# jiaxi98/cnf_ot

Hardware: NVIDIA B200
Metric: flow train-step samples/s (fwd+inv+logdet+loss+grad) (higher is better)
Workload: dtype f32

## Files before the change

cnf_ot_b200/csrc/api.cu:

```cuda
#include <cuda_runtime.h>
#include <math.h>
#include <stdarg.h>
#include <stdio.h>
#include <stdlib.h>
#include <string.h>

#include <mutex>
#include <vector>

#include "../../include/cnfot.h"
#include "device_common.cuh"
#include "dense_tc.h"
#include "dispatch.h"
#include "flow_kernels.cuh"
#include "step_host.h"
#include "wide.h"

namespace cnfot {

cudaError_t rqs_eval_dispatch(int K, bool inverse, cudaStream_t s, const float* v,
                              const float* params, int64_t rows, const SplineConsts<float>& sc,
                              float* out, float* ld, int32_t* bin, int num_sms, bool* known);
cudaError_t rqs_vjp_dispatch(int K, bool inverse, cudaStream_t s, const float* v,
                             const float* params, const float* go, const float* gl, int64_t rows,
                             const SplineConsts<float>& sc, float* gi, float* gp, int num_sms,
                             bool* known);

static thread_local char g_err[512] = "";

static int fail(int code, const char* fmt, ...) {
  va_list ap;
  va_start(ap, fmt);
  vsnprintf(g_err, sizeof(g_err), fmt, ap);
  va_end(ap);
  return code;
}

static int cuda_fail(cudaError_t e, const char* what) {
  return fail(CNFOT_ERR_CUDA, "%s: %s", what, cudaGetErrorString(e));
}

struct DeviceInfo {
  int device = -1;
  int num_sms = 0;
  int max_smem_optin = 0;
};

static int device_info(DeviceInfo* out) {
  static DeviceInfo cache[64];
  int dev = 0;
  cudaError_t e = cudaGetDevice(&dev);
  if (e != cudaSuccess) return cuda_fail(e, "cudaGetDevice (no CUDA device? libcnfot has no CPU path)");
  if (dev < 0 || dev >= 64) return fail(CNFOT_ERR_CUDA, "device id %d out of range", dev);
  if (cache[dev].device != dev) {
    DeviceInfo d;
    d.device = dev;
    e = cudaDeviceGetAttribute(&d.num_sms, cudaDevAttrMultiProcessorCount, dev);
    if (e != cudaSuccess) return cuda_fail(e, "cudaDeviceGetAttribute");
    e = cudaDeviceGetAttribute(&d.max_smem_optin, cudaDevAttrMaxSharedMemoryPerBlockOptin, dev);
    if (e != cudaSuccess) return cuda_fail(e, "cudaDeviceGetAttribute");
    cache[dev] = d;
  }
  *out = cache[dev];
  return 0;
}

constexpr int kMaxGrid = 148 * 8;
constexpr int64_t kCounterBytes = 256;

static int check_flow(const cnfot_flow_desc* f, FlowLayout* lay) {
  if (!f) return fail(CNFOT_ERR_ARG, "flow descriptor is NULL");
  if (f->dim < 1 || f->num_layers < 1 || f->mlp_layers < 1 || f->hidden < 1 || f->num_bins < 1)
    return fail(CNFOT_ERR_ARG, "flow descriptor has non-positive sizes");
  if (f->hidden % 4 != 0) return fail(CNFOT_ERR_ARG, "hidden size %d must be a multiple of 4", f->hidden);
  if (!(f->range_max > f->range_min) || f->num_bins * f->min_bin_size > f->range_max - f->range_min)
    return fail(CNFOT_ERR_ARG, "min_bin_size too large for the spline range");
  if (!(f->min_knot_slope < 1.f)) return fail(CNFOT_ERR_ARG, "min_knot_slope must be < 1");
  *lay = make_layout(f->dim, f->num_layers, f->mlp_layers, f->hidden, f->num_bins);
  return 0;
}

static bool reference_spline_consts(const cnfot_flow_desc* f) {
  const SplineConsts<float> c = make_spline_consts<float>(f->num_bins, f->range_min, f->range_max, f->min_bin_size,
                                                          f->min_knot_slope);
  return c.lo == -10.f && c.hi == 10.f && c.min_bin == 1e-4f && c.min_slope == 1e-4f &&
         fabsf(c.slope_offset - 0.5411666523385311f) <= 1e-7f;
}

static int check_fused(const cnfot_flow_desc* f, const FlowLayout& lay) {
  if (!reference_spline_consts(f))
    return fail(CNFOT_ERR_ARG, "the fused flow kernels are compiled for the reference's spline constants (range -10..10, "
                               "min_bin_size = min_knot_slope = 1e-4; cnf_ot/models/flows.py:124-132)");
  if (f->dim > kMaxDim) return fail(CNFOT_ERR_ARG, "fused kernels support dim <= %d (got %d)", kMaxDim, f->dim);
  if ((f->num_layers + 1) * f->dim > kMaxStateFloats)
    return fail(CNFOT_ERR_ARG, "fused kernels need (num_layers+1)*dim <= %d (got %d)", kMaxStateFloats,
                (f->num_layers + 1) * f->dim);
  if (!find_flow_eval_kernel(lay))
    return fail(CNFOT_ERR_ARG,
                "no fused kernel instantiated for hidden=%d num_bins=%d mlp_layers=%d "
                "(see CNFOT_NET_LIST in cnf_ot_b200/csrc/dispatch.h)",
                f->hidden, f->num_bins, f->mlp_layers);
  return 0;
}

static bool fused_ok(const cnfot_flow_desc* f, const FlowLayout& lay) {
  if (!(f->dim <= kMaxDim && (f->num_layers + 1) * f->dim <= kMaxStateFloats && find_flow_eval_kernel(lay) != nullptr))
    return false;
  if (!reference_spline_consts(f)) return false;
  if (tc_available(lay)) return true;
  DeviceInfo di;
  if (device_info(&di)) return true;
  return (int64_t)plan_smem(lay, true, false).floats * 4 <= di.max_smem_optin;
}
static bool use_wide(const cnfot_flow_desc* f, const FlowLayout& lay) {
  if (!wide_supported(lay, nullptr)) return false;
  if (!fused_ok(f, lay)) return true;
  const char* e = getenv("CNFOT_ENGINE");
  return e && !strcmp(e, "wide");
}

static SplineConsts<float> spline_consts(const cnfot_flow_desc* f) {
  return make_spline_consts<float>(f->num_bins, f->range_min, f->range_max, f->min_bin_size,
                                   f->min_knot_slope);
}

struct LaunchCfg {
  int grid;
  size_t smem;
};
static thread_local int g_last_launch[4] = {0, 0, 0, 0};

static int engine_override() {
  const char* e = getenv("CNFOT_ENGINE");
  if (!e) {
    const char* t = getenv("CNFOT_TC");
    return (t && t[0] == '1') ? kEngTc : -1;
  }
  if (!strcmp(e, "cuda")) return kEngCuda;
  if (!strcmp(e, "tc")) return kEngTc;
  if (!strcmp(e, "mma")) return kEngMma;
  return -1;
}

static int make_plan(const FlowLayout& lay, bool with_grad, SmemPlan* sp, int* engine, bool has_ws = true) {
  DeviceInfo di;
  if (int rc = device_info(&di)) return rc;
  const int want = engine_override();
  *engine = kEngCuda;
  if (want == kEngTc && tc_available(lay)) {
    SmemPlan t = plan_smem(lay, with_grad, true, true);
    if ((int64_t)t.floats * 4 * 2 <= di.max_smem_optin) {
      *sp = t;
      *engine = kEngTc;
      return 0;
    }
  }
  if ((want == kEngMma || want < 0) && tc_available(lay)) {
    SmemPlan m = plan_smem_mma(lay, with_grad);
    if ((int64_t)m.floats * 4 * 2 <= di.max_smem_optin) {
      *sp = m;
      *engine = kEngMma;
      return 0;
    }
    if (has_ws) {
      *sp = plan_smem_mma(lay, with_grad, false);
      *engine = kEngMmaStream;
      return 0;
    }
  }
  SmemPlan p = plan_smem(lay, with_grad, true);
  if ((int64_t)p.floats * 4 * 2 > di.max_smem_optin) p = plan_smem(lay, with_grad, false);
  *sp = p;
  return 0;
}

static int configure(const void* kernel, const SmemPlan& sp, int64_t tiles, LaunchCfg* cfg) {
  DeviceInfo di;
  if (int rc = device_info(&di)) return rc;
  size_t smem = (size_t)sp.floats * sizeof(float);
  if ((int64_t)smem > di.max_smem_optin)
    return fail(CNFOT_ERR_ARG, "network too large for the fused kernels: needs %zu B of shared memory, device allows %d",
                smem, di.max_smem_optin);
  cudaError_t e = cudaFuncSetAttribute(kernel, cudaFuncAttributeMaxDynamicSharedMemorySize, (int)smem);
  if (e != cudaSuccess) return cuda_fail(e, "cudaFuncSetAttribute");
  int occ = 0;
  e = cudaOccupancyMaxActiveBlocksPerMultiprocessor(&occ, kernel, kTile, smem);
  if (e != cudaSuccess) return cuda_fail(e, "cudaOccupancyMaxActiveBlocksPerMultiprocessor");
  if (sp.off_wmma >= 0) {
    cudaFuncAttributes fa;
    e = cudaFuncGetAttributes(&fa, kernel);
    if (e != cudaSuccess) return cuda_fail(e, "cudaFuncGetAttributes");
    int smem_sm = 0, regs_sm = 0;
    cudaDeviceGetAttribute(&smem_sm, cudaDevAttrMaxSharedMemoryPerMultiprocessor, di.device);
    cudaDeviceGetAttribute(&regs_sm, cudaDevAttrMaxRegistersPerMultiprocessor, di.device);
    int by_smem = (int)(smem_sm / (smem + fa.sharedSizeBytes + 1024));
    int by_regs = regs_sm / (fa.numRegs * kTile > 0 ? fa.numRegs * kTile : 1);
    int by_tmem = 512 / 32;
    occ = by_smem < by_regs ? by_smem : by_regs;
    if (occ > by_tmem) occ = by_tmem;
  }
  if (getenv("CNFOT_DEBUG")) {
    cudaFuncAttributes fa;
    cudaFuncGetAttributes(&fa, kernel);
    int o0 = 0, o1 = 0;
    cudaOccupancyMaxActiveBlocksPerMultiprocessor(&o0, kernel, kTile, 0);
    cudaOccupancyMaxActiveBlocksPerMultiprocessor(&o1, kernel, kTile, 60000);
    fprintf(stderr, "[cnfot] occ=%d (smem %zu) occ@0=%d occ@60000=%d regs=%d static_smem=%zu local=%zu maxdyn=%d carveout=%d\n",
            occ, smem, o0, o1, fa.numRegs, fa.sharedSizeBytes, fa.localSizeBytes, fa.maxDynamicSharedSizeBytes,
            fa.preferredShmemCarveout);
  }
  if (occ < 1) return fail(CNFOT_ERR_CUDA, "kernel does not fit on an SM");
  int64_t cap = (int64_t)di.num_sms * occ;
  if (cap > kMaxGrid) cap = kMaxGrid;
  int64_t g = tiles < cap ? tiles : cap;
  cfg->grid = (int)(g > 0 ? g : 1);
  cfg->smem = smem;
  g_last_launch[0] = cfg->grid;
  g_last_launch[1] = (int)smem;
  g_last_launch[2] = occ;
  g_last_launch[3] = sp.off_wmma >= 0 ? kEngTc : (sp.off_frag >= 0 ? kEngMma : kEngCuda);
  return 0;
}

static int64_t frag_bytes(const FlowLayout& lay) {
  if (!tc_available(lay)) return 0;
  return (int64_t)lay.L * (lay.D - 1) * lay.M * kFragFloats * sizeof(float);
}
static int64_t partial_bytes(const FlowLayout& lay) {
  int64_t loss = (int64_t)kMaxGrid * kNumSlots * sizeof(double);
  int64_t grad = ((int64_t)kMaxGrid * lay.total * sizeof(float) + 255) / 256 * 256;
  return kCounterBytes + loss + grad + frag_bytes(lay);
}
static int64_t stash_cta_floats(const FlowLayout& lay) {
  if (!tc_available(lay)) return 0;
  const int64_t per_cta = (int64_t)lay.L * (lay.D - 1) * (4 * lay.M + (2 * lay.K + 10 + 3) / 4) * kTile * 4;
  if (per_cta * (int64_t)sizeof(float) > 64 * 1024) return 0;
  if (const char* e = getenv("CNFOT_STEP_STASH")) {
    if (e[0] == '0') return 0;
  }
  return per_cta;
}
constexpr int kStashMaxGrid = 6 * 148;
static int64_t stash_bytes(const FlowLayout& lay) { return stash_cta_floats(lay) * (int64_t)sizeof(float) * kStashMaxGrid; }
static int64_t step_bytes(const FlowLayout& lay) { return partial_bytes(lay) + stash_bytes(lay); }
static float* carve_frags(void* ws, const FlowLayout& lay) {
  return (float*)((char*)ws + partial_bytes(lay) - frag_bytes(lay));
}
static int launch_build_frags(cudaStream_t s, const FlowLayout& lay, const float* weights, float* frags) {
  const int n_mat = lay.L * (lay.D - 1) * lay.M;
  const int blocks = (n_mat * 256 + 255) / 256;
  build_frags_kernel<<<blocks < 1184 ? blocks : 1184, 256, 0, s>>>(weights, frags, lay.D, lay.M, n_mat);
  cudaError_t e = cudaGetLastError();
  if (e != cudaSuccess) return cuda_fail(e, "build_frags_kernel launch");
  return 0;
}

static PartialBuf carve_partials(void* ws, unsigned long long** counter) {
  char* p = (char*)ws;
  *counter = (unsigned long long*)p;
  PartialBuf pb;
  pb.loss = (double*)(p + kCounterBytes);
  pb.grad = (float*)(p + kCounterBytes + (int64_t)kMaxGrid * kNumSlots * sizeof(double));
  return pb;
}

constexpr int kFinWarps = 32;
__device__ __forceinline__ double column_partial(const float* __restrict__ pgrad, int n_cta, int total, int i,
                                                 int warp) {
  double a0 = 0.0, a1 = 0.0, a2 = 0.0, a3 = 0.0;
  int c = warp;
  for (; c + 3 * kFinWarps < n_cta; c += 4 * kFinWarps) {
    const float v0 = __ldcg(pgrad + (int64_t)c * total + i);
    const float v1 = __ldcg(pgrad + (int64_t)(c + kFinWarps) * total + i);
    const float v2 = __ldcg(pgrad + (int64_t)(c + 2 * kFinWarps) * total + i);
    const float v3 = __ldcg(pgrad + (int64_t)(c + 3 * kFinWarps) * total + i);
    a0 += (double)v0; a1 += (double)v1; a2 += (double)v2; a3 += (double)v3;
  }
  for (; c < n_cta; c += kFinWarps) a0 += (double)__ldcg(pgrad + (int64_t)c * total + i);
  return (a0 + a1) + (a2 + a3);
}

__global__ void __launch_bounds__(32 * kFinWarps)
finalize_kernel(const float* __restrict__ pgrad, const double* __restrict__ ploss, int n_cta,
                int total, float* __restrict__ out_grad, float* __restrict__ out_slots,
                int accumulate) {
  __shared__ double part[kFinWarps][32];
  const int lane = threadIdx.x & 31, warp = threadIdx.x >> 5;
  const int i = blockIdx.x * 32 + lane;
  double acc = 0.0;
  if (i < total) acc = column_partial(pgrad, n_cta, total, i, warp);
  part[warp][lane] = acc;
  __syncthreads();
  if (warp == 0 && i < total) {
    double t = 0.0;
#pragma unroll
    for (int w = 0; w < kFinWarps; ++w) t += part[w][lane];
    out_grad[i] = accumulate ? out_grad[i] + (float)t : (float)t;
  }
  if (out_slots && blockIdx.x == gridDim.x - 1) {
    __syncthreads();
    const int sl = lane & 7, sub = lane >> 3;
    double v = 0.0;
    for (int c = warp * 4 + sub; c < n_cta; c += 4 * kFinWarps) v += ploss[(int64_t)c * kNumSlots + sl];
    v += __shfl_xor_sync(0xffffffffu, v, 8);
    v += __shfl_xor_sync(0xffffffffu, v, 16);
    part[warp][lane] = v;
    __syncthreads();
    if (warp == 0) {
      double t = 0.0;
      if (lane < kNumSlots)
        for (int w = 0; w < kFinWarps; ++w) t += part[w][lane];
      double tot = t;
      tot += __shfl_xor_sync(0xffffffffu, tot, 1);
      tot += __shfl_xor_sync(0xffffffffu, tot, 2);
      if (lane == 0) out_slots[0] = accumulate ? out_slots[0] + (float)tot : (float)tot;
      if (lane < 4) out_slots[1 + lane] = accumulate ? out_slots[1 + lane] + (float)t : (float)t;
      if (lane >= 5 && lane < kNumSlots) out_slots[lane] = 0.f;
    }
  }
}

static int launch_finalize(cudaStream_t s, const PartialBuf& pb, int n_cta, int total, float* out_grad,
                           float* out_slots, bool accumulate = false) {
  int blocks = (total + 31) / 32;
  finalize_kernel<<<blocks, 32 * kFinWarps, 0, s>>>(pb.grad, pb.loss, n_cta, total, out_grad, out_slots,
                                                   accumulate ? 1 : 0);
  cudaError_t e = cudaGetLastError();
  if (e != cudaSuccess) return cuda_fail(e, "finalize_kernel launch");
  return 0;
}

__global__ void energy_finalize_kernel(const double* __restrict__ ploss, int n_cta, double* __restrict__ out) {
  double v = 0.0;
  for (int c = threadIdx.x; c < n_cta; c += 32) v += ploss[(int64_t)c * kNumSlots + kSlotKinetic];
#pragma unroll
  for (int o = 16; o > 0; o >>= 1) v += __shfl_xor_sync(0xffffffffu, v, o);
  if (threadIdx.x == 0) out[0] = v;
}

__global__ void adam_kernel(float* __restrict__ p, const float* __restrict__ g, float* __restrict__ m,
                            float* __restrict__ v, int64_t n, float lr, float b1, float b2, float eps,
                            float c1, float c2) {
  for (int64_t i = blockIdx.x * (int64_t)blockDim.x + threadIdx.x; i < n; i += (int64_t)gridDim.x * blockDim.x) {
    float gi = g[i];
    float mi = b1 * m[i] + (1.f - b1) * gi;
    float vi = b2 * v[i] + (1.f - b2) * gi * gi;
    m[i] = mi;
    v[i] = vi;
    p[i] -= lr * (mi / c1) / (sqrtf(vi / c2) + eps);
  }
}

__global__ void __launch_bounds__(256)
recon_head_kernel(const float* __restrict__ x, const float* __restrict__ xr, int64_t count, float weight,
                  float* __restrict__ g_xr, double* __restrict__ loss) {
  double acc = 0.0;
  for (int64_t e = blockIdx.x * (int64_t)blockDim.x + threadIdx.x; e < count; e += (int64_t)gridDim.x * blockDim.x) {
    const float dlt = x[e] - xr[e];
    acc += (double)dlt * (double)dlt;
    g_xr[e] = -2.f * weight * dlt;
  }
#pragma unroll
  for (int o = 16; o > 0; o >>= 1) acc += __shfl_xor_sync(0xffffffffu, acc, o);
  if ((threadIdx.x & 31) == 0 && acc != 0.0) atomicAdd(loss, acc * (double)weight);
}
__global__ void __launch_bounds__(256)
mask_tail_kernel(float* __restrict__ y, int64_t rows, int dim, int sub_dim) {
  const int64_t count = rows * dim;
  for (int64_t e = blockIdx.x * (int64_t)blockDim.x + threadIdx.x; e < count; e += (int64_t)gridDim.x * blockDim.x)
    if ((int)(e % dim) >= sub_dim) y[e] = 0.f;
}

}

using namespace cnfot;

extern "C" {

int cnfot_abi_version(void) { return CNFOT_ABI_VERSION; }
static unsigned long long* g_step_timeline = nullptr;
void cnfot_debug_step_timeline(void* device_words) { g_step_timeline = (unsigned long long*)device_words; }

void cnfot_last_launch_info(int32_t* grid, int32_t* smem_bytes, int32_t* ctas_per_sm, int32_t* tensor_cores) {
  if (grid) *grid = g_last_launch[0];
  if (smem_bytes) *smem_bytes = g_last_launch[1];
  if (ctas_per_sm) *ctas_per_sm = g_last_launch[2];
  if (tensor_cores) *tensor_cores = g_last_launch[3];
}
const char* cnfot_last_error(void) { return g_err; }

int64_t cnfot_param_count(const cnfot_flow_desc* flow) {
  FlowLayout lay;
  if (check_flow(flow, &lay)) return -1;
  return lay.total;
}

int64_t cnfot_spline_param_stride(const cnfot_flow_desc* flow) {
  FlowLayout lay;
  if (check_flow(flow, &lay)) return -1;
  return lay.Pp;
}

int64_t cnfot_offset_first(const cnfot_flow_desc* flow) {
  FlowLayout lay;
  if (check_flow(flow, &lay)) return -1;
  return 0;
}

int64_t cnfot_offset_linear(const cnfot_flow_desc* flow, int32_t layer, int32_t d, int32_t m, int32_t bias) {
  FlowLayout lay;
  if (check_flow(flow, &lay)) return -1;
  if (layer < 0 || layer >= lay.L || d < 1 || d >= lay.D || m < 0 || m > lay.M) {
    fail(CNFOT_ERR_ARG, "offset_linear: index out of range");
    return -1;
  }
  const int H = lay.H;
  int64_t off = lay.Pp + (int64_t)layer * lay.layer_stride + (int64_t)(d - 1) * lay.mlp_const +
                (int64_t)H * ((d - 1) * (d + 2) / 2);
  const int n_in = d + 1;
  if (m == 0) return off + (bias ? n_in * H : 0);
  off += n_in * H + H + (int64_t)(m - 1) * (H * H + H);
  if (m < lay.M) return off + (bias ? H * H : 0);
  return off + (bias ? H * lay.Pp : 0);
}

int cnfot_flow_supported(const cnfot_flow_desc* flow) {
  FlowLayout lay;
  if (int rc = check_flow(flow, &lay)) return rc;
  if (use_wide(flow, lay)) return 0;
  return check_fused(flow, lay);
}

static int rqs_call(bool inverse, void* stream, const float* v, const float* params, int64_t rows,
                    int32_t K, float lo, float hi, float min_bin, float min_slope, float* out,
                    float* ld, int32_t* bin) {
  if (rows < 0) return fail(CNFOT_ERR_ARG, "rows < 0");
  if (rows == 0) return 0;
  if (!v || !params || !out || !ld) return fail(CNFOT_ERR_ARG, "NULL buffer");
  if (K < 1 || !(hi > lo) || K * min_bin > hi - lo || !(min_slope < 1.f))
    return fail(CNFOT_ERR_ARG, "bad spline constants");
  DeviceInfo di;
  if (int rc = device_info(&di)) return rc;
  bool known = false;
  cudaError_t e = rqs_eval_dispatch(K, inverse, (cudaStream_t)stream, v, params, rows,
                                    make_spline_consts<float>(K, lo, hi, min_bin, min_slope), out, ld,
                                    bin, di.num_sms, &known);
  if (!known) return fail(CNFOT_ERR_ARG, "num_bins=%d not instantiated (see CNFOT_BINS_LIST)", K);
  if (e != cudaSuccess) return cuda_fail(e, "rqs kernel launch");
  return 0;
}

static int rqs_vjp_call(bool inverse, void* stream, const float* v, const float* params,
                        const float* go, const float* gl, int64_t rows, int32_t K, float lo, float hi,
                        float min_bin, float min_slope, float* gi, float* gp) {
  if (rows < 0) return fail(CNFOT_ERR_ARG, "rows < 0");
  if (rows == 0) return 0;
  if (!v || !params || !go || !gl || !gi || !gp) return fail(CNFOT_ERR_ARG, "NULL buffer");
  if (K < 1 || !(hi > lo) || K * min_bin > hi - lo || !(min_slope < 1.f))
    return fail(CNFOT_ERR_ARG, "bad spline constants");
  DeviceInfo di;
  if (int rc = device_info(&di)) return rc;
  bool known = false;
  cudaError_t e = rqs_vjp_dispatch(K, inverse, (cudaStream_t)stream, v, params, go, gl, rows,
                                   make_spline_consts<float>(K, lo, hi, min_bin, min_slope), gi, gp,
                                   di.num_sms, &known);
  if (!known) return fail(CNFOT_ERR_ARG, "num_bins=%d not instantiated (see CNFOT_BINS_LIST)", K);
  if (e != cudaSuccess) return cuda_fail(e, "rqs vjp kernel launch");
  return 0;
}

int cnfot_rqs_forward(void* stream, const float* x, const float* params, int64_t rows, int32_t num_bins,
                      float range_min, float range_max, float min_bin_size, float min_knot_slope,
                      float* y, float* logdet, int32_t* bin_idx) {
  return rqs_call(false, stream, x, params, rows, num_bins, range_min, range_max, min_bin_size,
                  min_knot_slope, y, logdet, bin_idx);
}
int cnfot_rqs_inverse(void* stream, const float* y, const float* params, int64_t rows, int32_t num_bins,
                      float range_min, float range_max, float min_bin_size, float min_knot_slope,
                      float* x, float* logdet, int32_t* bin_idx) {
  return rqs_call(true, stream, y, params, rows, num_bins, range_min, range_max, min_bin_size,
                  min_knot_slope, x, logdet, bin_idx);
}
int cnfot_rqs_forward_vjp(void* stream, const float* x, const float* params, const float* g_y,
                          const float* g_logdet, int64_t rows, int32_t num_bins, float range_min,
                          float range_max, float min_bin_size, float min_knot_slope, float* g_x,
                          float* g_params) {
  return rqs_vjp_call(false, stream, x, params, g_y, g_logdet, rows, num_bins, range_min, range_max,
                      min_bin_size, min_knot_slope, g_x, g_params);
}
int cnfot_rqs_inverse_vjp(void* stream, const float* y, const float* params, const float* g_x,
                          const float* g_logdet, int64_t rows, int32_t num_bins, float range_min,
                          float range_max, float min_bin_size, float min_knot_slope, float* g_y,
                          float* g_params) {
  return rqs_vjp_call(true, stream, y, params, g_x, g_logdet, rows, num_bins, range_min, range_max,
                      min_bin_size, min_knot_slope, g_y, g_params);
}

static int flow_eval_call(int dir, void* stream, const cnfot_flow_desc* flow, const float* weights,
                          const float* in, const float* cond, int64_t cond_stride, int64_t rows,
                          float* out, float* logdet, int32_t add_base, void* workspace = nullptr,
                          int64_t workspace_bytes = 0) {
  FlowLayout lay;
  if (int rc = check_flow(flow, &lay)) return rc;
  if (use_wide(flow, lay)) {
    if (rows < 0) return fail(CNFOT_ERR_ARG, "rows < 0");
    if (cond_stride != 0 && cond_stride != 1) return fail(CNFOT_ERR_ARG, "cond_stride must be 0 or 1");
    if (rows == 0) return 0;
    if (!weights || !in || !cond || !out) return fail(CNFOT_ERR_ARG, "NULL buffer");
    const int64_t need = wide_flow_workspace_bytes(lay, rows, false);
    if (!workspace)
      return fail(CNFOT_ERR_WORKSPACE, "this flow runs on the wide-conditioner engine, which needs a workspace: "
                                       "call cnfot_flow_forward_ws / cnfot_flow_inverse_ws");
    if (workspace_bytes < need) return fail(CNFOT_ERR_WORKSPACE, "workspace too small: %lld < %lld",
                                            (long long)workspace_bytes, (long long)need);
    const char* what = "";
    cudaError_t e = wide_flow_eval((cudaStream_t)stream, lay, spline_consts(flow), weights, dir, in, cond, cond_stride,
                                   rows, out, logdet, add_base, workspace, &what);
    if (e != cudaSuccess) return cuda_fail(e, what);
    g_last_launch[0] = 0; g_last_launch[1] = 0; g_last_launch[2] = 0; g_last_launch[3] = kEngWide;
    return 0;
  }
  if (int rc = check_fused(flow, lay)) return rc;
  if (rows < 0) return fail(CNFOT_ERR_ARG, "rows < 0");
  if (cond_stride != 0 && cond_stride != 1) return fail(CNFOT_ERR_ARG, "cond_stride must be 0 or 1");
  if (rows == 0) return 0;
  if (!weights || !in || !cond || !out) return fail(CNFOT_ERR_ARG, "NULL buffer");
  SmemPlan sp;
  int engine;
  if (int rc = make_plan(lay, false, &sp, &engine, false)) return rc;
  const void* kernel = find_flow_eval_kernel(lay, engine);
  LaunchCfg cfg;
  if (int rc = configure(kernel, sp, (rows + kTile - 1) / kTile, &cfg)) return rc;
  EvalArgs a;
  a.W = weights; a.frags = nullptr; a.in = in; a.cond = cond; a.cond_stride = cond_stride; a.rows = rows;
  a.out = out; a.logdet = logdet; a.dir = dir; a.add_base = add_base;
  a.D = lay.D; a.L = lay.L; a.plan = sp;
  void* args[] = {&a};
  cudaError_t e = cudaLaunchKernel(kernel, dim3(cfg.grid), dim3(kTile), args, cfg.smem, (cudaStream_t)stream);
  if (e != cudaSuccess) return cuda_fail(e, "flow_eval_kernel launch");
  return 0;
}

int cnfot_flow_forward(void* stream, const cnfot_flow_desc* flow, const float* weights, const float* in,
                       const float* cond, int64_t cond_stride, int64_t rows, float* out, float* logdet,
                       int32_t add_base) {
  return flow_eval_call(0, stream, flow, weights, in, cond, cond_stride, rows, out, logdet, add_base);
}
int cnfot_flow_inverse(void* stream, const cnfot_flow_desc* flow, const float* weights, const float* in,
                       const float* cond, int64_t cond_stride, int64_t rows, float* out, float* logdet,
                       int32_t add_base) {
  return flow_eval_call(1, stream, flow, weights, in, cond, cond_stride, rows, out, logdet, add_base);
}

int64_t cnfot_flow_workspace_bytes(const cnfot_flow_desc* flow, int64_t rows) {
  FlowLayout lay;
  if (check_flow(flow, &lay)) return -1;
  return use_wide(flow, lay) ? wide_flow_workspace_bytes(lay, rows, false) : 0;
}
int cnfot_flow_forward_ws(void* stream, const cnfot_flow_desc* flow, const float* weights, const float* in,
                          const float* cond, int64_t cond_stride, int64_t rows, float* out, float* logdet,
                          int32_t add_base, void* workspace, int64_t workspace_bytes) {
  return flow_eval_call(0, stream, flow, weights, in, cond, cond_stride, rows, out, logdet, add_base, workspace,
                        workspace_bytes);
}
int cnfot_flow_inverse_ws(void* stream, const cnfot_flow_desc* flow, const float* weights, const float* in,
                          const float* cond, int64_t cond_stride, int64_t rows, float* out, float* logdet,
                          int32_t add_base, void* workspace, int64_t workspace_bytes) {
  return flow_eval_call(1, stream, flow, weights, in, cond, cond_stride, rows, out, logdet, add_base, workspace,
                        workspace_bytes);
}

int64_t cnfot_flow_vjp_workspace_bytes(const cnfot_flow_desc* flow, int64_t rows) {
  FlowLayout lay;
  if (check_flow(flow, &lay)) return -1;
  if (use_wide(flow, lay)) return wide_flow_workspace_bytes(lay, rows, true);
  return step_bytes(lay);
}

static int flow_vjp_call(int dir, void* stream, const cnfot_flow_desc* flow, const float* weights,
                         const float* in, const float* cond, int64_t cond_stride, int64_t rows,
                         const float* g_out, const float* g_logdet, int32_t add_base, float* g_in,
                         float* g_weights, void* workspace, int64_t workspace_bytes) {
  FlowLayout lay;
  if (int rc = check_flow(flow, &lay)) return rc;
  if (use_wide(flow, lay)) {
    if (rows < 0) return fail(CNFOT_ERR_ARG, "rows < 0");
    if (cond_stride != 0 && cond_stride != 1) return fail(CNFOT_ERR_ARG, "cond_stride must be 0 or 1");
    if (!weights || !g_weights || !workspace) return fail(CNFOT_ERR_ARG, "NULL buffer");
    if (rows > 0 && (!in || !cond || !g_out)) return fail(CNFOT_ERR_ARG, "NULL buffer");
    const int64_t need = wide_flow_workspace_bytes(lay, rows, true);
    if (workspace_bytes < need) return fail(CNFOT_ERR_WORKSPACE, "workspace too small: %lld < %lld",
                                            (long long)workspace_bytes, (long long)need);
    const char* what = "";
    cudaError_t e = wide_flow_vjp((cudaStream_t)stream, lay, spline_consts(flow), weights, dir, in, cond, cond_stride,
                                  rows, g_out, g_logdet, add_base, g_in, g_weights, workspace, &what);
    if (e != cudaSuccess) return cuda_fail(e, what);
    g_last_launch[0] = 0; g_last_launch[1] = 0; g_last_launch[2] = 0; g_last_launch[3] = kEngWide;
    return 0;
  }
  if (int rc = check_fused(flow, lay)) return rc;
  if (rows < 0) return fail(CNFOT_ERR_ARG, "rows < 0");
  if (cond_stride != 0 && cond_stride != 1) return fail(CNFOT_ERR_ARG, "cond_stride must be 0 or 1");
  if (!weights || !g_weights || !workspace) return fail(CNFOT_ERR_ARG, "NULL buffer");
  if (workspace_bytes < partial_bytes(lay)) return fail(CNFOT_ERR_WORKSPACE, "workspace too small: %lld < %lld",
                                                        (long long)workspace_bytes, (long long)partial_bytes(lay));
  cudaStream_t s = (cudaStream_t)stream;
  if (rows == 0) {
    cudaError_t e = cudaMemsetAsync(g_weights, 0, (size_t)lay.total * sizeof(float), s);
    if (e != cudaSuccess) return cuda_fail(e, "cudaMemsetAsync");
    return 0;
  }
  if (!in || !cond || !g_out) return fail(CNFOT_ERR_ARG, "NULL buffer");
  SmemPlan sp;
  int engine;
  if (int rc = make_plan(lay, true, &sp, &engine)) return rc;
  const void* kernel = find_flow_vjp_kernel(lay, engine);
  LaunchCfg cfg;
  if (int rc = configure(kernel, sp, (rows + kTile - 1) / kTile, &cfg)) return rc;
  unsigned long long* counter;
  VjpArgs a;
  a.W = weights; a.frags = nullptr; a.in = in; a.cond = cond; a.cond_stride = cond_stride; a.rows = rows;
  if (engine == kEngMmaStream) {
    float* fr = carve_frags(workspace, lay);
    if (int rc = launch_build_frags(s, lay, weights, fr)) return rc;
    a.frags = fr;
  }
  a.g_out = g_out; a.g_logdet = g_logdet; a.g_in = g_in; a.dir = dir; a.add_base = add_base;
  a.D = lay.D; a.L = lay.L; a.plan = sp;
  a.pb = carve_partials(workspace, &counter);
  a.stash = nullptr;
  a.stash_cta_floats = (engine == kEngMma || engine == kEngMmaStream) && cfg.grid <= kStashMaxGrid &&
                               workspace_bytes >= step_bytes(lay)
                           ? stash_cta_floats(lay) : 0;
  if (a.stash_cta_floats > 0) a.stash = (float*)((char*)workspace + partial_bytes(lay));
  void* args[] = {&a};
  cudaError_t e = cudaLaunchKernel(kernel, dim3(cfg.grid), dim3(kTile), args, cfg.smem, s);
  if (e != cudaSuccess) return cuda_fail(e, "flow_vjp_kernel launch");
  return launch_finalize(s, a.pb, cfg.grid, lay.total, g_weights, nullptr);
}

int cnfot_flow_forward_vjp(void* stream, const cnfot_flow_desc* flow, const float* weights,
                           const float* in, const float* cond, int64_t cond_stride, int64_t rows,
                           const float* g_out, const float* g_logdet, int32_t add_base, float* g_in,
                           float* g_weights, void* workspace, int64_t workspace_bytes) {
  return flow_vjp_call(0, stream, flow, weights, in, cond, cond_stride, rows, g_out, g_logdet, add_base,
                       g_in, g_weights, workspace, workspace_bytes);
}
int cnfot_flow_inverse_vjp(void* stream, const cnfot_flow_desc* flow, const float* weights,
                           const float* in, const float* cond, int64_t cond_stride, int64_t rows,
                           const float* g_out, const float* g_logdet, int32_t add_base, float* g_in,
                           float* g_weights, void* workspace, int64_t workspace_bytes) {
  return flow_vjp_call(1, stream, flow, weights, in, cond, cond_stride, rows, g_out, g_logdet, add_base,
                       g_in, g_weights, workspace, workspace_bytes);
}

static std::mutex g_ws_mu;
static std::vector<std::pair<void*, int64_t>> g_ws_registered;
static bool ws_registered(const void* ws) {
  std::lock_guard<std::mutex> lk(g_ws_mu);
  for (const auto& e : g_ws_registered)
    if (e.first == ws) return true;
  return false;
}
int cnfot_workspace_release(void* workspace) {
  std::lock_guard<std::mutex> lk(g_ws_mu);
  for (size_t i = 0; i < g_ws_registered.size(); ++i)
    if (g_ws_registered[i].first == workspace) {
      g_ws_registered.erase(g_ws_registered.begin() + i);
      return 0;
    }
  return 0;
}

static bool pdl_enabled() {
  static int on = -1;
  if (on < 0) {
    const char* e = getenv("CNFOT_PDL");
    on = (e && e[0] == '0') ? 0 : 1;
  }
  return on != 0;
}
static cudaError_t launch_step_kernel(const void* kernel, int grid, void** args, size_t smem, cudaStream_t s) {
  if (!pdl_enabled()) return cudaLaunchKernel(kernel, dim3(grid), dim3(kTile), args, smem, s);
  cudaLaunchConfig_t lc = {};
  lc.gridDim = dim3(grid); lc.blockDim = dim3(kTile); lc.dynamicSmemBytes = smem; lc.stream = s;
  cudaLaunchAttribute at[1];
  at[0].id = cudaLaunchAttributeProgrammaticStreamSerialization;
  at[0].val.programmaticStreamSerializationAllowed = 1;
  lc.attrs = at; lc.numAttrs = 1;
  return cudaLaunchKernelExC(&lc, kernel, args);
}

static int64_t step_ws_bytes(const cnfot_flow_desc* flow, const FlowLayout& lay, int64_t rows_B, int64_t rows_b) {
  return use_wide(flow, lay) ? wide_step_workspace_bytes(lay, rows_B, rows_b) : step_bytes(lay);
}

int64_t cnfot_mfc_step_workspace_bytes(const cnfot_flow_desc* flow, int64_t rows_B, int64_t rows_b,
                                       int32_t n_t) {
  (void)n_t;
  FlowLayout lay;
  if (check_flow(flow, &lay)) return -1;
  return step_ws_bytes(flow, lay, rows_B, rows_b);
}

static int mfc_step_wide(void* stream, const cnfot_flow_desc* flow, const FlowLayout& lay,
                         const cnfot_problem_desc* problem, const float* weights, const float* latent, const float* latent_sub,
                         const float* src, const float* tgt, const float* t_batch_host, int32_t n_t, int64_t rows_B,
                         int64_t rows_b, int64_t global_B, int64_t global_b, float lambda, float* out, void* workspace,
                         int64_t workspace_bytes, bool accumulate, const cnfot_peer_desc* peers) {
  if (!problem) return fail(CNFOT_ERR_ARG, "problem descriptor is NULL");
  if (peers)
    return fail(CNFOT_ERR_ARG, "the wide-conditioner engine has no fused all-reduce (its gradient is hundreds of MB): "
                               "call cnfot_mfc_step and all-reduce `out` with NCCL");
  if (accumulate) return fail(CNFOT_ERR_ARG, "the wide-conditioner engine does not take chunked host input");
  if (rows_B < 0 || rows_b < 0 || global_B < 1 || global_b < 1 || rows_B > global_B || rows_b > global_b)
    return fail(CNFOT_ERR_ARG, "bad row counts");
  if (n_t < 1) return fail(CNFOT_ERR_ARG, "t_batch_size must be >= 1");
  if (!weights || !out || !workspace || !t_batch_host) return fail(CNFOT_ERR_ARG, "NULL buffer");
  if (problem->type == CNFOT_OT) {
    if (rows_B > 0 && (!src || !tgt)) return fail(CNFOT_ERR_ARG, "ot needs src and tgt batches");
  } else if (rows_B > 0 && !latent) {
    return fail(CNFOT_ERR_ARG, "latent is NULL");
  }
  if (rows_b > 0 && !latent_sub) return fail(CNFOT_ERR_ARG, "latent_sub is NULL");
  const int64_t need = wide_step_workspace_bytes(lay, rows_B, rows_b);
  if (workspace_bytes < need) return fail(CNFOT_ERR_WORKSPACE, "workspace too small: %lld < %lld",
                                          (long long)workspace_bytes, (long long)need);
  StepConsts<float> pc;
  const char* err = nullptr;
  if (make_step_consts<float>(*problem, lay.D, (double)lambda, global_B, global_b, n_t, &pc, &err))
    return fail(CNFOT_ERR_ARG, "%s", err);
  const char* what = "";
  cudaError_t e = wide_mfc_step((cudaStream_t)stream, lay, spline_consts(flow), pc, weights, latent, latent_sub, src, tgt,
                                t_batch_host, n_t, rows_B, rows_b, out, workspace, &what);
  if (e != cudaSuccess) return cuda_fail(e, what);
  g_last_launch[0] = 0; g_last_launch[1] = 0; g_last_launch[2] = 0; g_last_launch[3] = kEngWide;
  return 0;
}

struct StepIo {
  const float* latent = nullptr;
  const float* latent_sub = nullptr;
  const float* src = nullptr;
  const float* tgt = nullptr;
  const float* t_batch_host = nullptr;
  bool rng = false;
  uint64_t key = 0;
  uint32_t step = 0;
  int64_t row0_B = 0, row0_b = 0;
  float* out = nullptr;
  bool accumulate = false;
  const cnfot_peer_desc* peers = nullptr;
  bool stateful = false;
  float* weights_rw = nullptr;
  float* adam_m = nullptr;
  float* adam_v = nullptr;
  float lr = 0.f, b1 = 0.9f, b2 = 0.999f, eps = 1e-8f;
  float* loss_hist = nullptr;
  int64_t loss_hist_len = 0;
};

static unsigned long long dp_timeout_ns() {
  unsigned long long ms = 20000ULL;
  if (const char* e = getenv("CNFOT_DP_TIMEOUT_MS")) {
    const long long v = atoll(e);
    if (v > 0) ms = (unsigned long long)v;
  }
  return ms * 1000000ULL;
}

static int mfc_step_impl(void* stream, const cnfot_flow_desc* flow, const cnfot_problem_desc* problem,
                         const float* weights, const StepIo& io, int32_t n_t,
                         int64_t rows_B, int64_t rows_b, int64_t global_B, int64_t global_b, float lambda,
                         void* workspace, int64_t workspace_bytes) {
  FlowLayout lay;
  if (int rc = check_flow(flow, &lay)) return rc;
  if (use_wide(flow, lay)) {
    cnfot_workspace_release(workspace);
    if (io.rng || io.stateful)
      return fail(CNFOT_ERR_ARG, "the wide-conditioner engine takes explicit row arrays: fill them with cnfot_philox_rows "
                                 "and call cnfot_mfc_step (+ cnfot_adam_update)");
    return mfc_step_wide(stream, flow, lay, problem, weights, io.latent, io.latent_sub, io.src, io.tgt, io.t_batch_host, n_t,
                         rows_B, rows_b, global_B, global_b, lambda, io.out, workspace, workspace_bytes, io.accumulate, io.peers);
  }
  if (int rc = check_fused(flow, lay)) return rc;
  if (!problem) return fail(CNFOT_ERR_ARG, "problem descriptor is NULL");
  StepArgs a;
  memset(&a.tail, 0, sizeof(a.tail));
  PeerArgs& pa = a.tail.pa;
  const cnfot_peer_desc* peers = io.peers;
  if (peers) {
    if (peers->world < 1 || peers->world > 8 || peers->rank < 0 || peers->rank >= peers->world)
      return fail(CNFOT_ERR_ARG, "peer descriptor: need 1 <= world <= 8 and 0 <= rank < world");
    if (peers->epoch == 0 && !io.stateful) return fail(CNFOT_ERR_ARG, "peer descriptor: epoch starts at 1");
    pa.rank = peers->rank; pa.world = peers->world; pa.epoch = peers->epoch;
    pa.stride = (int)cnfot_dp_exchange_stride(flow);
    pa.timeout_ns = dp_timeout_ns();
    for (int k = 0; k < peers->world; ++k) {
      if (!peers->xbuf[k] || !peers->flags[k]) return fail(CNFOT_ERR_ARG, "peer descriptor: NULL peer buffer");
      if ((uintptr_t)peers->xbuf[k] & 7) return fail(CNFOT_ERR_ARG, "peer descriptor: exchange buffers must be 8-byte aligned");
      pa.xbuf[k] = (unsigned long long*)peers->xbuf[k]; pa.flags[k] = peers->flags[k];
    }
  }
  if (rows_B < 0 || rows_b < 0 || global_B < 1 || global_b < 1 || rows_B > global_B || rows_b > global_b)
    return fail(CNFOT_ERR_ARG, "bad row counts");
  if (n_t < 1 || n_t > kMaxSegments - 4) return fail(CNFOT_ERR_ARG, "t_batch_size must be in [1, %d]", kMaxSegments - 4);
  if (!weights || !workspace) return fail(CNFOT_ERR_ARG, "NULL buffer");
  if (!io.out && !io.stateful) return fail(CNFOT_ERR_ARG, "out is NULL");
  if (!io.rng && !io.t_batch_host) return fail(CNFOT_ERR_ARG, "t_batch is NULL");
  if (workspace_bytes < step_bytes(lay)) return fail(CNFOT_ERR_WORKSPACE, "workspace too small: %lld < %lld",
                                                     (long long)workspace_bytes, (long long)step_bytes(lay));
  const char* err = nullptr;
  if (make_step_consts<float>(*problem, lay.D, (double)lambda, global_B, global_b, n_t, &a.pc, &err))
    return fail(CNFOT_ERR_ARG, "%s", err);
  if (!io.rng) {
    if (problem->type == CNFOT_OT) {
      if (rows_B > 0 && (!io.src || !io.tgt)) return fail(CNFOT_ERR_ARG, "ot needs src and tgt batches");
    } else {
      if (rows_B > 0 && !io.latent) return fail(CNFOT_ERR_ARG, "latent is NULL");
    }
    if (rows_b > 0 && !io.latent_sub) return fail(CNFOT_ERR_ARG, "latent_sub is NULL");
  } else if (io.row0_B < 0 || io.row0_b < 0 || io.row0_B + rows_B > global_B || io.row0_b + rows_b > global_b) {
    return fail(CNFOT_ERR_ARG, "shard [row0, row0 + rows) outside the global batch");
  }
  cudaStream_t s = (cudaStream_t)stream;
  if (rows_B == 0 && rows_b == 0 && !peers && !io.stateful) {
    if (io.accumulate) return 0;
    cudaError_t e = cudaMemsetAsync(io.out, 0, (size_t)(lay.total + CNFOT_NUM_LOSS_SLOTS) * sizeof(float), s);
    if (e != cudaSuccess) return cuda_fail(e, "cudaMemsetAsync");
    return 0;
  }
  SmemPlan sp;
  int engine;
  if (int rc = make_plan(lay, true, &sp, &engine)) return rc;
  const int unit = kTile;

  int ns = 0;
  int64_t tiles = 0;
  auto add = [&](int kind, int slot, int do_fit, int do_pot, float t, int t_index, const float* rows, int source,
                 int64_t row0, int64_t n, int group) {
    if (n <= 0) return;
    Segment& sg = a.seg[ns++];
    sg.kind = kind; sg.slot = slot; sg.do_fit = do_fit; sg.do_pot = do_pot; sg.t = t; sg.t_index = t_index;
    sg.rows = rows; sg.source = io.rng ? source : (int)kRowsMemory; sg.row0 = row0;
    sg.n = n; sg.first_tile = tiles; sg.group = group;
    tiles += (n * group + unit - 1) / unit;
  };
  int group = 1;
  {
    const bool with_score = problem->type != CNFOT_OT;
    const bool need_r3 = with_score || a.pc.potential == kPotObstacle;
    int g = with_score ? 4 : (need_r3 ? 4 : 2);
    while (with_score && g < 2 * lay.D) g <<= 1;
    const int64_t fit_tiles = (problem->type == CNFOT_FP ? 1 : 2) * ((rows_B + unit - 1) / unit);
    const int64_t serial_tiles = fit_tiles + (int64_t)n_t * ((rows_b + unit - 1) / unit);
    bool split = g <= 32 && serial_tiles <= kMaxGrid;
    if (const char* e = getenv("CNFOT_KINETIC_SPLIT")) split = g <= 32 && e[0] != '0';
    if (split) group = g;
  }
  bool latency = false;
  {
    const int64_t fit_tiles = (problem->type == CNFOT_FP ? 1 : 2) * ((rows_B + unit - 1) / unit);
    latency = fit_tiles + (int64_t)n_t * ((rows_b + unit - 1) / unit) < 8 * 4 * 148;
    if (const char* e = getenv("CNFOT_STEP_LATENCY")) latency = e[0] != '0';
  }
  const void* kernel = find_mfc_step_kernel(lay, engine, group > 1, latency);
  for (int i = 0; i < n_t; ++i)
    add(group > 1 ? kSegKineticSplit : kSegKinetic, kSlotKinetic, 0, 0, io.rng ? 0.f : io.t_batch_host[i], io.rng ? i : -1,
        io.latent_sub, kRowsNormal, io.row0_b, rows_b, group);
  if (problem->type == CNFOT_OT) {
    add(kSegNll, kSlotFit0, 1, 0, 0.f, -1, io.src, kRowsOtSource, io.row0_B, rows_B, 1);
    add(kSegNll, kSlotFitT, 1, 0, (float)a.pc.horizon, -1, io.tgt, kRowsNormal, io.row0_B, rows_B, 1);
  } else {
    add(kSegSample, kSlotFit0, 1, 0, 0.f, -1, io.latent, kRowsNormal, io.row0_B, rows_B, 1);
    if (problem->type == CNFOT_RWPO) add(kSegSample, kSlotFit0, 0, 1, (float)a.pc.horizon, -1, io.latent, kRowsNormal, io.row0_B, rows_B, 1);
  }
  a.n_seg = ns;
  a.n_tiles = tiles;
  a.key = io.key;
  a.step = io.step;
  a.timeline = g_step_timeline;
  a.salt_B = philox_salt(kDrawNormal, (uint64_t)global_B);
  a.salt_Bc = philox_salt(kDrawCategorical, (uint64_t)global_B);
  a.salt_b = philox_salt(kDrawNormal, (uint64_t)global_b);
  a.salt_t = philox_salt(kDrawUniform, (uint64_t)n_t);
  LaunchCfg cfg;
  if (int rc = configure(kernel, sp, (tiles * unit + kTile - 1) / kTile, &cfg)) return rc;
  a.W = weights;
  a.frags = nullptr;
  if (engine == kEngMmaStream) {
    float* fr = carve_frags(workspace, lay);
    if (int rc = launch_build_frags(s, lay, weights, fr)) return rc;
    a.frags = fr;
  }
  a.D = lay.D; a.L = lay.L; a.plan = sp;
  a.stash = nullptr;
  a.stash_cta_floats = (engine == kEngMma || engine == kEngMmaStream) && cfg.grid <= kStashMaxGrid ? stash_cta_floats(lay) : 0;
  if (a.stash_cta_floats > 0) a.stash = (float*)((char*)workspace + partial_bytes(lay));
  TailArgs& t = a.tail;
  char* wsb = (char*)workspace;
  t.sync = (uint32_t*)wsb;
  t.loss_row = (double*)(wsb) + kLossRowOffset;
  t.grad_rows = (float*)(wsb + kCounterBytes);
  const bool persistent = io.stateful || ws_registered(workspace);
  t.n_rows = cfg.grid < kStepRows ? cfg.grid : kStepRows;
  if (const char* e = getenv("CNFOT_STEP_ROWS")) {
    const int v = atoi(e);
    if (v >= 1 && v <= (persistent ? kStepRows : kMaxGrid)) t.n_rows = v < cfg.grid ? v : cfg.grid;
  }
  int n_tail = (lay.total + kNumSlots + kTile / 4 - 1) / (kTile / 4);
  if (n_tail > cfg.grid) n_tail = cfg.grid;
  if (cfg.grid > 148 && n_tail > cfg.grid / 2) n_tail = cfg.grid / 2;
  if (n_tail > 2 * 148) n_tail = 2 * 148;
  if (n_tail < 1) n_tail = 1;
  t.n_tail = n_tail;
  t.total = lay.total;
  t.n_tiles = tiles;
  t.accumulate = io.accumulate ? 1 : 0;
  t.out = io.out;
  if (io.stateful) {
    t.self_clean = 1;
    t.state = (unsigned long long*)wsb + kStateWordOffset;
    t.weights = io.weights_rw; t.adam_m = io.adam_m; t.adam_v = io.adam_v;
    t.lr = io.lr; t.b1 = io.b1; t.b2 = io.b2; t.eps = io.eps;
    t.loss_hist = io.loss_hist; t.loss_hist_len = io.loss_hist_len;
  } else if (persistent) {
    t.self_clean = 1;
  } else {
    cudaError_t e = cudaMemsetAsync(wsb, 0, (size_t)kCounterBytes + (size_t)t.n_rows * lay.total * sizeof(float), s);
    if (e != cudaSuccess) return cuda_fail(e, "cudaMemsetAsync");
  }
  void* args[] = {&a};
  cudaError_t e = launch_step_kernel(kernel, cfg.grid, args, cfg.smem, s);
  if (e != cudaSuccess) return cuda_fail(e, "mfc_step_kernel launch");
  return 0;
}

int64_t cnfot_dp_exchange_stride(const cnfot_flow_desc* flow) {
  FlowLayout lay;
  if (check_flow(flow, &lay)) return -1;
  return (lay.total + kNumSlots + 31) / 32 * 32;
}
int64_t cnfot_dp_exchange_floats(const cnfot_flow_desc* flow, int32_t world) {
  const int64_t st = cnfot_dp_exchange_stride(flow);
  return st < 0 ? -1 : 2 * 2 * (int64_t)world * st;
}
int64_t cnfot_dp_flag_count(const cnfot_flow_desc* flow, int32_t world) {
  FlowLayout lay;
  if (check_flow(flow, &lay)) return -1;
  (void)world;
  return 32;
}

int cnfot_mfc_step_dp(void* stream, const cnfot_flow_desc* flow, const cnfot_problem_desc* problem,
                      const float* weights, const float* latent, const float* latent_sub, const float* src,
                      const float* tgt, const float* t_batch_host, int32_t n_t, int64_t rows_B,
                      int64_t rows_b, int64_t global_B, int64_t global_b, float lambda, float* out,
                      void* workspace, int64_t workspace_bytes, const cnfot_peer_desc* peers) {
  if (!peers) return fail(CNFOT_ERR_ARG, "peer descriptor is NULL");
  StepIo io;
  io.latent = latent; io.latent_sub = latent_sub; io.src = src; io.tgt = tgt; io.t_batch_host = t_batch_host;
  io.out = out; io.peers = peers;
  return mfc_step_impl(stream, flow, problem, weights, io, n_t, rows_B, rows_b, global_B, global_b, lambda, workspace,
                       workspace_bytes);
}

int cnfot_workspace_register(void* stream, const cnfot_flow_desc* flow, void* workspace, int64_t workspace_bytes) {
  FlowLayout lay;
  if (int rc = check_flow(flow, &lay)) return rc;
  if (use_wide(flow, lay)) return fail(CNFOT_ERR_ARG, "persistent workspaces serve the fused per-row step kernel, not the wide-conditioner engine");
  if (!workspace) return fail(CNFOT_ERR_ARG, "NULL buffer");
  if (workspace_bytes < step_bytes(lay)) return fail(CNFOT_ERR_WORKSPACE, "workspace too small: %lld < %lld",
                                                     (long long)workspace_bytes, (long long)step_bytes(lay));
  cudaError_t e = cudaMemsetAsync(workspace, 0, (size_t)kCounterBytes + (size_t)kStepRows * lay.total * sizeof(float),
                                  (cudaStream_t)stream);
  if (e != cudaSuccess) return cuda_fail(e, "cudaMemsetAsync");
  cnfot_workspace_release(workspace);
  std::lock_guard<std::mutex> lk(g_ws_mu);
  g_ws_registered.emplace_back(workspace, workspace_bytes);
  return 0;
}

int cnfot_mfc_step(void* stream, const cnfot_flow_desc* flow, const cnfot_problem_desc* problem,
                   const float* weights, const float* latent, const float* latent_sub, const float* src,
                   const float* tgt, const float* t_batch_host, int32_t n_t, int64_t rows_B,
                   int64_t rows_b, int64_t global_B, int64_t global_b, float lambda, float* out,
                   void* workspace, int64_t workspace_bytes) {
  StepIo io;
  io.latent = latent; io.latent_sub = latent_sub; io.src = src; io.tgt = tgt; io.t_batch_host = t_batch_host;
  io.out = out;
  return mfc_step_impl(stream, flow, problem, weights, io, n_t, rows_B, rows_b, global_B, global_b, lambda, workspace,
                       workspace_bytes);
}

__global__ void __launch_bounds__(256)
philox_rows_kernel(unsigned long long key_n, unsigned long long key_c, uint32_t step, int source, int64_t row0, int64_t rows,
                   int dim, float* __restrict__ out) {
  for (int64_t r = blockIdx.x * (int64_t)blockDim.x + threadIdx.x; r < rows; r += (int64_t)gridDim.x * blockDim.x) {
    float row[kMaxDim];
    philox_row(key_n, key_c, step, source, (uint64_t)(row0 + r), dim, row);
    for (int i = 0; i < dim; ++i) out[r * dim + i] = row[i];
  }
}

int cnfot_philox_rows(void* stream, uint64_t key, uint32_t step, int32_t source, int64_t global_rows, int64_t row0,
                      int64_t rows, int32_t dim, float* out) {
  if (rows < 0 || row0 < 0 || row0 + rows > global_rows || dim < 1 || dim > kMaxDim)
    return fail(CNFOT_ERR_ARG, "philox_rows: need 0 <= row0, row0 + rows <= global_rows, 1 <= dim <= %d", kMaxDim);
  if (source != CNFOT_ROWS_NORMAL && source != CNFOT_ROWS_OT_SOURCE) return fail(CNFOT_ERR_ARG, "philox_rows: unknown row source");
  if (rows == 0) return 0;
  if (!out) return fail(CNFOT_ERR_ARG, "NULL buffer");
  int64_t blocks = (rows + 255) / 256;
  if (blocks > 148 * 8) blocks = 148 * 8;
  philox_rows_kernel<<<(int)blocks, 256, 0, (cudaStream_t)stream>>>(
      key ^ philox_salt(kDrawNormal, (uint64_t)global_rows), key ^ philox_salt(kDrawCategorical, (uint64_t)global_rows), step,
      source, row0, rows, dim, out);
  cudaError_t e = cudaGetLastError();
  if (e != cudaSuccess) return cuda_fail(e, "philox_rows_kernel launch");
  return 0;
}

int cnfot_philox_times_host(uint64_t key, uint32_t step, int32_t n_t, float horizon, float* t_host) {
  if (n_t < 0 || (n_t > 0 && !t_host)) return fail(CNFOT_ERR_ARG, "philox_times: bad arguments");
  const uint64_t kt = key ^ philox_salt(kDrawUniform, (uint64_t)n_t);
  for (int i = 0; i < n_t; ++i) t_host[i] = philox_time(kt, step, i, horizon);
  return 0;
}

int cnfot_mfc_step_rng(void* stream, const cnfot_flow_desc* flow, const cnfot_problem_desc* problem, const float* weights,
                       uint64_t key, uint32_t step, int32_t n_t, int64_t row0_B, int64_t rows_B, int64_t row0_b,
                       int64_t rows_b, int64_t global_B, int64_t global_b, float lambda, float* out, void* workspace,
                       int64_t workspace_bytes, const cnfot_peer_desc* peers) {
  StepIo io;
  io.rng = true; io.key = key; io.step = step; io.row0_B = row0_B; io.row0_b = row0_b;
  io.out = out; io.peers = peers;
  return mfc_step_impl(stream, flow, problem, weights, io, n_t, rows_B, rows_b, global_B, global_b, lambda, workspace,
                       workspace_bytes);
}

int64_t cnfot_train_state_bytes(const cnfot_flow_desc* flow) {
  FlowLayout lay;
  if (check_flow(flow, &lay)) return -1;
  if (use_wide(flow, lay)) { fail(CNFOT_ERR_ARG, "no device-resident update for the wide-conditioner engine"); return -1; }
  return step_bytes(lay);
}

int cnfot_train_state_init(void* stream, const cnfot_flow_desc* flow, void* state, int64_t state_bytes, uint64_t key,
                           uint64_t step, uint32_t epoch) {
  const int64_t need = cnfot_train_state_bytes(flow);
  if (need < 0) return CNFOT_ERR_ARG;
  if (!state) return fail(CNFOT_ERR_ARG, "NULL buffer");
  if (state_bytes < need) return fail(CNFOT_ERR_WORKSPACE, "train state too small: %lld < %lld", (long long)state_bytes, (long long)need);
  FlowLayout lay;
  check_flow(flow, &lay);
  cudaStream_t s = (cudaStream_t)stream;
  cudaError_t e = cudaMemsetAsync(state, 0, (size_t)kCounterBytes + (size_t)kStepRows * lay.total * sizeof(float), s);
  if (e != cudaSuccess) return cuda_fail(e, "cudaMemsetAsync");
  const unsigned long long words[3] = {key, step, (unsigned long long)epoch};
  e = cudaMemcpyAsync((unsigned long long*)state + kStateWordOffset, words, sizeof(words), cudaMemcpyHostToDevice, s);
  if (e != cudaSuccess) return cuda_fail(e, "H2D train state");
  e = cudaStreamSynchronize(s);
  if (e != cudaSuccess) return cuda_fail(e, "cudaStreamSynchronize");
  return 0;
}

int cnfot_mfc_update(void* stream, const cnfot_flow_desc* flow, const cnfot_problem_desc* problem, void* state,
                     int64_t state_bytes, float* weights, float* adam_m, float* adam_v, const cnfot_adam_desc* adam,
                     int32_t n_t, int64_t row0_B, int64_t rows_B, int64_t row0_b, int64_t rows_b, int64_t global_B,
                     int64_t global_b, float lambda, float* out, float* loss_hist, int64_t loss_hist_len,
                     const cnfot_peer_desc* peers) {
  if (!state || !weights || !adam_m || !adam_v || !adam) return fail(CNFOT_ERR_ARG, "NULL buffer");
  if (loss_hist_len < 0 || (loss_hist_len > 0 && !loss_hist)) return fail(CNFOT_ERR_ARG, "bad loss history buffer");
  StepIo io;
  io.rng = true; io.row0_B = row0_B; io.row0_b = row0_b;
  io.out = out; io.peers = peers;
  io.stateful = true;
  io.weights_rw = weights; io.adam_m = adam_m; io.adam_v = adam_v;
  io.lr = adam->lr; io.b1 = adam->b1; io.b2 = adam->b2; io.eps = adam->eps;
  io.loss_hist = loss_hist; io.loss_hist_len = loss_hist_len;
  return mfc_step_impl(stream, flow, problem, weights, io, n_t, rows_B, rows_b, global_B, global_b, lambda, state,
                       state_bytes);
}

static int64_t align256(int64_t v) { return (v + 255) / 256 * 256; }

struct HostPipe {
  bool ready_ = false;
  cudaStream_t copy;
  cudaEvent_t start;
  cudaEvent_t ready[4];
};
static int host_pipe(HostPipe** out) {
  static HostPipe pipes[64];
  DeviceInfo di;
  if (int rc = device_info(&di)) return rc;
  HostPipe& p = pipes[di.device];
  if (!p.ready_) {
    cudaError_t e = cudaStreamCreateWithFlags(&p.copy, cudaStreamNonBlocking);
    if (e != cudaSuccess) return cuda_fail(e, "cudaStreamCreateWithFlags");
    if ((e = cudaEventCreateWithFlags(&p.start, cudaEventDisableTiming)) != cudaSuccess) return cuda_fail(e, "cudaEventCreate");
    for (int k = 0; k < 4; ++k)
      if ((e = cudaEventCreateWithFlags(&p.ready[k], cudaEventDisableTiming)) != cudaSuccess) return cuda_fail(e, "cudaEventCreate");
    p.ready_ = true;
  }
  *out = &p;
  return 0;
}

int64_t cnfot_mfc_step_host_workspace_bytes(const cnfot_flow_desc* flow, int64_t rows_B, int64_t rows_b,
                                            int32_t n_t) {
  FlowLayout lay;
  if (check_flow(flow, &lay)) return -1;
  (void)n_t;
  int64_t rowsB = align256(rows_B * lay.D * (int64_t)sizeof(float));
  int64_t rowsb = align256(rows_b * lay.D * (int64_t)sizeof(float));
  int64_t w = align256((int64_t)lay.total * sizeof(float));
  int64_t o = align256((int64_t)(lay.total + CNFOT_NUM_LOSS_SLOTS) * sizeof(float));
  return align256(step_ws_bytes(flow, lay, rows_B, rows_b)) + w + o + 3 * rowsB + rowsb;
}

int cnfot_mfc_step_host(void* stream, const cnfot_flow_desc* flow, const cnfot_problem_desc* problem,
                        const float* weights_host, const float* latent_host,
                        const float* latent_sub_host, const float* src_host, const float* tgt_host,
                        const float* t_batch_host, int32_t n_t, int64_t rows_B, int64_t rows_b,
                        int64_t global_B, int64_t global_b, float lambda, float* out_host,
                        void* workspace, int64_t workspace_bytes) {
  FlowLayout lay;
  if (int rc = check_flow(flow, &lay)) return rc;
  if (!weights_host || !out_host || !workspace) return fail(CNFOT_ERR_ARG, "NULL buffer");
  if (rows_B < 0 || rows_b < 0) return fail(CNFOT_ERR_ARG, "bad row counts");
  int64_t need = cnfot_mfc_step_host_workspace_bytes(flow, rows_B, rows_b, n_t);
  if (workspace_bytes < need) return fail(CNFOT_ERR_WORKSPACE, "workspace too small: %lld < %lld",
                                          (long long)workspace_bytes, (long long)need);
  cudaStream_t s = (cudaStream_t)stream;
  char* p = (char*)workspace;
  const int64_t ws_bytes = align256(step_ws_bytes(flow, lay, rows_B, rows_b));
  void* ws = p; p += ws_bytes;
  float* dW = (float*)p; p += align256((int64_t)lay.total * sizeof(float));
  float* dOut = (float*)p; p += align256((int64_t)(lay.total + CNFOT_NUM_LOSS_SLOTS) * sizeof(float));
  const int64_t bytesB = rows_B * lay.D * (int64_t)sizeof(float);
  float* dLat = (float*)p; p += align256(bytesB);
  float* dSrc = (float*)p; p += align256(bytesB);
  float* dTgt = (float*)p; p += align256(bytesB);
  float* dSub = (float*)p;
  cudaError_t e;
  bool zero_copy = true;
  if (const char* ev = getenv("CNFOT_HOST_ZEROCOPY")) zero_copy = ev[0] != '0';
  const float* mapped[4] = {nullptr, nullptr, nullptr, nullptr};
  const float* hostp[4] = {latent_host, latent_sub_host, src_host, tgt_host};
  for (int k = 0; k < 4 && zero_copy; ++k) {
    if (!hostp[k]) continue;
    cudaPointerAttributes at;
    e = cudaPointerGetAttributes(&at, hostp[k]);
    if (e != cudaSuccess || at.type != cudaMemoryTypeHost || !at.devicePointer) {
      cudaGetLastError();
      zero_copy = false;
      break;
    }
    mapped[k] = (const float*)at.devicePointer;
  }
  if ((e = cudaMemcpyAsync(dW, weights_host, (size_t)lay.total * sizeof(float), cudaMemcpyHostToDevice, s)) != cudaSuccess)
    return cuda_fail(e, "H2D weights");
  if (zero_copy) {
    StepIo io;
    io.latent = mapped[0]; io.latent_sub = mapped[1]; io.src = mapped[2]; io.tgt = mapped[3]; io.t_batch_host = t_batch_host;
    io.out = dOut;
    int rc = mfc_step_impl(stream, flow, problem, dW, io, n_t, rows_B, rows_b, global_B, global_b, lambda, ws, ws_bytes);
    if (rc) return rc;
  } else {
    HostPipe* hp = nullptr;
    if (int rc = host_pipe(&hp)) return rc;
    int nchunk = 1;
    if (const char* ev = getenv("CNFOT_HOST_CHUNKS")) {
      const int v = atoi(ev);
      if (v >= 1 && v <= 4) nchunk = v;
    }
    if ((e = cudaEventRecord(hp->start, s)) != cudaSuccess) return cuda_fail(e, "cudaEventRecord");
    if ((e = cudaStreamWaitEvent(hp->copy, hp->start, 0)) != cudaSuccess) return cuda_fail(e, "cudaStreamWaitEvent");
    auto h2d = [&](cudaStream_t st, float* dst, const float* src, int64_t off_rows, int64_t n_rows) -> cudaError_t {
      if (!src || n_rows == 0) return cudaSuccess;
      return cudaMemcpyAsync(dst + off_rows * lay.D, src + off_rows * lay.D, (size_t)(n_rows * lay.D) * sizeof(float),
                             cudaMemcpyHostToDevice, st);
    };
    if ((e = h2d(s, dSub, latent_sub_host, 0, rows_b)) != cudaSuccess) return cuda_fail(e, "H2D latent_sub");
    for (int k = 0; k < nchunk; ++k) {
      const int64_t lo = rows_B * k / nchunk, hi = rows_B * (k + 1) / nchunk;
      if ((e = h2d(hp->copy, dLat, latent_host, lo, hi - lo)) != cudaSuccess) return cuda_fail(e, "H2D latent");
      if ((e = h2d(hp->copy, dSrc, src_host, lo, hi - lo)) != cudaSuccess) return cuda_fail(e, "H2D src");
      if ((e = h2d(hp->copy, dTgt, tgt_host, lo, hi - lo)) != cudaSuccess) return cuda_fail(e, "H2D tgt");
      if ((e = cudaEventRecord(hp->ready[k], hp->copy)) != cudaSuccess) return cuda_fail(e, "cudaEventRecord");
    }
    for (int k = 0; k < nchunk; ++k) {
      const int64_t lo = rows_B * k / nchunk, hi = rows_B * (k + 1) / nchunk;
      if ((e = cudaStreamWaitEvent(s, hp->ready[k], 0)) != cudaSuccess) return cuda_fail(e, "cudaStreamWaitEvent");
      StepIo io;
      io.latent = latent_host ? dLat + lo * lay.D : nullptr;
      io.latent_sub = latent_sub_host ? dSub : nullptr;
      io.src = src_host ? dSrc + lo * lay.D : nullptr;
      io.tgt = tgt_host ? dTgt + lo * lay.D : nullptr;
      io.t_batch_host = t_batch_host;
      io.out = dOut;
      io.accumulate = k > 0;
      int rc = mfc_step_impl(stream, flow, problem, dW, io, n_t, hi - lo, k == 0 ? rows_b : 0, global_B, global_b, lambda, ws,
                             ws_bytes);
      if (rc) return rc;
    }
  }
  e = cudaMemcpyAsync(out_host, dOut, (size_t)(lay.total + CNFOT_NUM_LOSS_SLOTS) * sizeof(float),
                      cudaMemcpyDeviceToHost, s);
  if (e != cudaSuccess) return cuda_fail(e, "D2H out");
  e = cudaStreamSynchronize(s);
  if (e != cudaSuccess) return cuda_fail(e, "cudaStreamSynchronize");
  return 0;
}

int64_t cnfot_mfc_step_rng_host_workspace_bytes(const cnfot_flow_desc* flow) {
  FlowLayout lay;
  if (check_flow(flow, &lay)) return -1;
  if (use_wide(flow, lay)) { fail(CNFOT_ERR_ARG, "on-chip draws are not available on the wide-conditioner engine"); return -1; }
  return align256(step_bytes(lay)) + align256((int64_t)lay.total * sizeof(float)) +
         align256((int64_t)(lay.total + CNFOT_NUM_LOSS_SLOTS) * sizeof(float));
}

int cnfot_mfc_step_rng_host(void* stream, const cnfot_flow_desc* flow, const cnfot_problem_desc* problem,
                            const float* weights_host, uint64_t key, uint32_t step, int32_t n_t, int64_t row0_B,
                            int64_t rows_B, int64_t row0_b, int64_t rows_b, int64_t global_B, int64_t global_b,
                            float lambda, float* out_host, void* workspace, int64_t workspace_bytes) {
  FlowLayout lay;
  if (int rc = check_flow(flow, &lay)) return rc;
  if (!weights_host || !out_host || !workspace) return fail(CNFOT_ERR_ARG, "NULL buffer");
  const int64_t need = cnfot_mfc_step_rng_host_workspace_bytes(flow);
  if (need < 0) return CNFOT_ERR_ARG;
  if (workspace_bytes < need) return fail(CNFOT_ERR_WORKSPACE, "workspace too small: %lld < %lld",
                                          (long long)workspace_bytes, (long long)need);
  cudaStream_t s = (cudaStream_t)stream;
  char* p = (char*)workspace;
  const int64_t ws_bytes = align256(step_bytes(lay));
  void* ws = p; p += ws_bytes;
  float* dW = (float*)p; p += align256((int64_t)lay.total * sizeof(float));
  float* dOut = (float*)p;
  cudaError_t e = cudaMemcpyAsync(dW, weights_host, (size_t)lay.total * sizeof(float), cudaMemcpyHostToDevice, s);
  if (e != cudaSuccess) return cuda_fail(e, "H2D weights");
  StepIo io;
  io.rng = true; io.key = key; io.step = step; io.row0_B = row0_B; io.row0_b = row0_b;
  float* out_mapped = nullptr;
  {
    cudaPointerAttributes at;
    if (cudaPointerGetAttributes(&at, out_host) == cudaSuccess && at.type == cudaMemoryTypeHost && at.devicePointer)
      out_mapped = (float*)at.devicePointer;
    else
      cudaGetLastError();
  }
  io.out = out_mapped ? out_mapped : dOut;
  if (int rc = mfc_step_impl(stream, flow, problem, dW, io, n_t, rows_B, rows_b, global_B, global_b, lambda, ws, ws_bytes))
    return rc;
  if (!out_mapped) {
    e = cudaMemcpyAsync(out_host, dOut, (size_t)(lay.total + CNFOT_NUM_LOSS_SLOTS) * sizeof(float), cudaMemcpyDeviceToHost, s);
    if (e != cudaSuccess) return cuda_fail(e, "D2H out");
  }
  e = cudaStreamSynchronize(s);
  if (e != cudaSuccess) return cuda_fail(e, "cudaStreamSynchronize");
  return 0;
}

int64_t cnfot_kinetic_energy_workspace_bytes(const cnfot_flow_desc* flow, int32_t n_t) {
  FlowLayout lay;
  if (check_flow(flow, &lay)) return -1;
  if (use_wide(flow, lay)) return wide_energy_workspace_bytes(lay);
  return partial_bytes(lay) + ((int64_t)(n_t > 0 ? n_t : 0) * (int64_t)sizeof(float) + 255) / 256 * 256;
}

int cnfot_kinetic_energy(void* stream, const cnfot_flow_desc* flow, const float* weights, const float* latent,
                         int64_t batch, int32_t latent_blocks, const float* t_host, int32_t n_t, float dt,
                         int32_t with_score, float kappa, float dx, double* out, void* workspace,
                         int64_t workspace_bytes) {
  FlowLayout lay;
  if (int rc = check_flow(flow, &lay)) return rc;
  if (!use_wide(flow, lay))
    if (int rc = check_fused(flow, lay)) return rc;
  if (batch < 1 || n_t < 1 || latent_blocks < 1) return fail(CNFOT_ERR_ARG, "batch, n_t and latent_blocks must be >= 1");
  if (!weights || !latent || !t_host || !out || !workspace) return fail(CNFOT_ERR_ARG, "NULL buffer");
  if (!(dt > 0.f) || (with_score && !(dx > 0.f))) return fail(CNFOT_ERR_ARG, "dt and dx must be positive");
  const int64_t need = cnfot_kinetic_energy_workspace_bytes(flow, n_t);
  if (workspace_bytes < need) return fail(CNFOT_ERR_WORKSPACE, "workspace too small: %lld < %lld",
                                          (long long)workspace_bytes, (long long)need);
  if (use_wide(flow, lay)) {
    const char* what = "";
    cudaError_t we = wide_kinetic_energy((cudaStream_t)stream, lay, spline_consts(flow), weights, latent, batch,
                                         latent_blocks, t_host, n_t, dt, with_score, kappa, dx, out, workspace, &what);
    if (we != cudaSuccess) return cuda_fail(we, what);
    g_last_launch[0] = 0; g_last_launch[1] = 0; g_last_launch[2] = 0; g_last_launch[3] = kEngWide;
    return 0;
  }
  cudaStream_t s = (cudaStream_t)stream;
  EnergyArgs a;
  float* t_dev = (float*)((char*)workspace + partial_bytes(lay));
  cudaError_t e = cudaMemcpyAsync(t_dev, t_host, (size_t)n_t * sizeof(float), cudaMemcpyHostToDevice, s);
  if (e != cudaSuccess) return cuda_fail(e, "H2D times");
  SmemPlan sp;
  int engine;
  if (int rc = make_plan(lay, false, &sp, &engine)) return rc;
  const void* kernel = find_energy_kernel(lay, engine);
  if (!kernel) return fail(CNFOT_ERR_ARG, "no energy kernel for this network shape");
  a.tiles_per_t = (batch + kTile - 1) / kTile;
  a.n_tiles = a.tiles_per_t * n_t;
  LaunchCfg cfg;
  if (int rc = configure(kernel, sp, a.n_tiles, &cfg)) return rc;
  a.W = weights;
  a.frags = nullptr;
  if (engine == kEngMmaStream) {
    float* fr = carve_frags(workspace, lay);
    if (int rc = launch_build_frags(s, lay, weights, fr)) return rc;
    a.frags = fr;
  }
  a.D = lay.D; a.L = lay.L; a.plan = sp;
  a.latent = latent; a.batch = batch; a.latent_blocks = latent_blocks;
  a.t_dev = t_dev; a.n_t = n_t; a.with_score = with_score;
  a.dt = dt; a.dx = dx; a.kappa = kappa;
  a.weight = 1.0 / (2.0 * (double)batch * (double)n_t);
  a.pb = carve_partials(workspace, &a.tile_counter);
  e = cudaMemsetAsync(a.tile_counter, 0, sizeof(unsigned long long), s);
  if (e != cudaSuccess) return cuda_fail(e, "cudaMemsetAsync");
  void* args[] = {&a};
  e = cudaLaunchKernel(kernel, dim3(cfg.grid), dim3(kTile), args, cfg.smem, s);
  if (e != cudaSuccess) return cuda_fail(e, "energy_kernel launch");
  energy_finalize_kernel<<<1, 32, 0, s>>>(a.pb.loss, cfg.grid, out);
  e = cudaGetLastError();
  if (e != cudaSuccess) return cuda_fail(e, "energy_finalize_kernel launch");
  return 0;
}

int64_t cnfot_density_workspace_bytes(const cnfot_flow_desc* flow, int32_t n_t) {
  FlowLayout lay;
  if (check_flow(flow, &lay)) return -1;
  if (use_wide(flow, lay)) { fail(CNFOT_ERR_ARG, "density evaluation runs on the fused kernels only"); return -1; }
  return partial_bytes(lay) + ((int64_t)(n_t > 0 ? n_t : 0) * (int64_t)sizeof(float) + 255) / 256 * 256 + 256;
}

static int density_call(void* stream, const cnfot_flow_desc* flow, const float* weights, DensityArgs& a, const float* t_host,
                        int32_t n_t, double* sq_err, void* workspace, int64_t workspace_bytes) {
  FlowLayout lay;
  if (int rc = check_flow(flow, &lay)) return rc;
  if (use_wide(flow, lay)) return fail(CNFOT_ERR_ARG, "density evaluation runs on the fused kernels only");
  if (int rc = check_fused(flow, lay)) return rc;
  if (!weights || !workspace) return fail(CNFOT_ERR_ARG, "NULL buffer");
  if (a.with_ref && (!sq_err || !(a.var0 > 0.f) || !(a.var1 > 0.f))) return fail(CNFOT_ERR_ARG, "reference density: need sq_err and positive variances");
  const int64_t need = cnfot_density_workspace_bytes(flow, n_t);
  if (workspace_bytes < need) return fail(CNFOT_ERR_WORKSPACE, "workspace too small: %lld < %lld", (long long)workspace_bytes, (long long)need);
  cudaStream_t s = (cudaStream_t)stream;
  if (a.n == 0) {
    if (sq_err) { cudaError_t e = cudaMemsetAsync(sq_err, 0, sizeof(double), s); if (e != cudaSuccess) return cuda_fail(e, "cudaMemsetAsync"); }
    return 0;
  }
  float* t_dev = (float*)((char*)workspace + partial_bytes(lay));
  if (n_t > 0) {
    cudaError_t e = cudaMemcpyAsync(t_dev, t_host, (size_t)n_t * sizeof(float), cudaMemcpyHostToDevice, s);
    if (e != cudaSuccess) return cuda_fail(e, "H2D times");
  }
  SmemPlan sp;
  int engine;
  if (int rc = make_plan(lay, false, &sp, &engine)) return rc;
  const void* kernel = find_density_kernel(lay, engine);
  if (!kernel) return fail(CNFOT_ERR_ARG, "no density kernel for this network shape");
  LaunchCfg cfg;
  if (int rc = configure(kernel, sp, (a.n + kTile - 1) / kTile, &cfg)) return rc;
  a.W = weights;
  a.frags = nullptr;
  if (engine == kEngMmaStream) {
    float* fr = carve_frags(workspace, lay);
    if (int rc = launch_build_frags(s, lay, weights, fr)) return rc;
    a.frags = fr;
  }
  a.D = lay.D; a.L = lay.L; a.plan = sp;
  a.t_dev = t_dev;
  unsigned long long* counter;
  a.pb = carve_partials(workspace, &counter);
  void* args[] = {&a};
  cudaError_t e = cudaLaunchKernel(kernel, dim3(cfg.grid), dim3(kTile), args, cfg.smem, s);
  if (e != cudaSuccess) return cuda_fail(e, "density_kernel launch");
  if (sq_err) {
    energy_finalize_kernel<<<1, 32, 0, s>>>(a.pb.loss, cfg.grid, sq_err);
    e = cudaGetLastError();
    if (e != cudaSuccess) return cuda_fail(e, "energy_finalize_kernel launch");
  }
  return 0;
}

int cnfot_density_grid(void* stream, const cnfot_flow_desc* flow, const float* weights, const float* t_host, int32_t n_t,
                       double x_min, double x_max, double y_min, double y_max, int32_t nx, int32_t ny, float* density,
                       int32_t with_ref, float mix, float var0, float var1, double* sq_err, void* workspace,
                       int64_t workspace_bytes) {
  if (!flow || flow->dim != 2) return fail(CNFOT_ERR_ARG, "density grids are two-dimensional (the reference's are): dim must be 2");
  if (n_t < 1 || nx < 2 || ny < 2 || !t_host) return fail(CNFOT_ERR_ARG, "density_grid: need n_t >= 1, nx, ny >= 2");
  if (!density && !with_ref) return fail(CNFOT_ERR_ARG, "density_grid: nothing to compute");
  DensityArgs a;
  memset(&a, 0, sizeof(a));
  a.mode = 0; a.nx = nx; a.ny = ny; a.n_t = n_t;
  a.x_min = x_min; a.x_step = (x_max - x_min) / (nx - 1);
  a.y_min = y_min; a.y_step = (y_max - y_min) / (ny - 1);
  a.n = (int64_t)nx * ny * n_t;
  a.density = density;
  a.with_ref = with_ref; a.mix = mix; a.var0 = var0; a.var1 = var1;
  return density_call(stream, flow, weights, a, t_host, n_t, with_ref ? sq_err : nullptr, workspace, workspace_bytes);
}

int cnfot_density_mc(void* stream, const cnfot_flow_desc* flow, const float* weights, float cond, uint64_t key, uint32_t step,
                     int64_t n, float* samples, float* density, int32_t with_ref, float mix, float var0, float var1,
                     double* sq_err, void* workspace, int64_t workspace_bytes) {
  if (n < 0) return fail(CNFOT_ERR_ARG, "density_mc: n < 0");
  if (!density && !with_ref && !samples) return fail(CNFOT_ERR_ARG, "density_mc: nothing to compute");
  DensityArgs a;
  memset(&a, 0, sizeof(a));
  a.mode = 1; a.n = n; a.cond = cond;
  a.key_n = key ^ philox_salt(kDrawNormal, (uint64_t)n);
  a.step = step;
  a.samples = samples; a.density = density;
  a.with_ref = with_ref; a.mix = mix; a.var0 = var0; a.var1 = var1;
  return density_call(stream, flow, weights, a, nullptr, 0, with_ref ? sq_err : nullptr, workspace, workspace_bytes);
}

int64_t cnfot_dense_prepared_floats(int32_t K, int32_t N) {
  if (K < 16 || N < 16 || K % 16 || N % 16) return -1;
  return 2 * (int64_t)K * N;
}

int cnfot_dense_prepare(void* stream, const float* W, int32_t K, int32_t N, int32_t ldw, int32_t transpose,
                        float* prepared) {
  if (!W || !prepared) return fail(CNFOT_ERR_ARG, "NULL buffer");
  if (cnfot_dense_prepared_floats(K, N) < 0) return fail(CNFOT_ERR_ARG, "dense layers need K and N to be multiples of 16");
  cudaError_t e = dense_prep((cudaStream_t)stream, W, K, N, ldw, transpose != 0, prepared);
  if (e != cudaSuccess) return cuda_fail(e, "dense_prep_kernel launch");
  return 0;
}

int cnfot_dense_forward(void* stream, const float* X, int64_t rows, int32_t K, int32_t ldx, const float* prepared,
                        int32_t N, const float* bias, const float* mask_src, int32_t ldm, int32_t epilogue,
                        float* Y, int32_t ldy) {
  if (rows < 0) return fail(CNFOT_ERR_ARG, "rows < 0");
  if (rows == 0) return 0;
  if (!X || !prepared || !Y) return fail(CNFOT_ERR_ARG, "NULL buffer");
  if (cnfot_dense_prepared_floats(K, N) < 0) return fail(CNFOT_ERR_ARG, "dense layers need K and N to be multiples of 16");
  if (epilogue < 0 || epilogue > 4) return fail(CNFOT_ERR_ARG, "unknown epilogue");
  if ((epilogue == 0 || epilogue == 1) && !bias) return fail(CNFOT_ERR_ARG, "bias is NULL");
  if (epilogue == 2 && !mask_src) return fail(CNFOT_ERR_ARG, "mask_src is NULL");
  if (ldx % 4 || ldy % 4 || (epilogue == 2 && ldm % 4)) return fail(CNFOT_ERR_ARG, "row strides must be multiples of 4 floats");
  bool ok = false;
  cudaError_t e = dense_forward((cudaStream_t)stream, X, rows, K, ldx, prepared, N, bias, mask_src, ldm, epilogue,
                                Y, ldy, &ok);
  if (!ok) return fail(CNFOT_ERR_ARG, "no dense kernel for N = %d", N);
  if (e != cudaSuccess) return cuda_fail(e, "dense_tc_kernel launch");
  return 0;
}

int cnfot_dense_wgrad(void* stream, const float* A, int32_t lda, const float* G, int32_t ldg, int64_t rows,
                      int32_t Ka, int32_t Nb, float* dW, int32_t ldw, float* db) {
  if (rows < 0) return fail(CNFOT_ERR_ARG, "rows < 0");
  if (rows == 0) return 0;
  if (!A || !G || !dW) return fail(CNFOT_ERR_ARG, "NULL buffer");
  if (Ka < 1 || Nb < 4 || Nb % 4 || ldw % 4 || ((uintptr_t)dW & 15))
    return fail(CNFOT_ERR_ARG, "dense_wgrad: Nb and ldw must be multiples of 4 and dW 16-byte aligned");
  cudaError_t e = dense_wgrad((cudaStream_t)stream, A, lda, G, ldg, rows, Ka, Nb, dW, ldw, db);
  if (e != cudaSuccess) return cuda_fail(e, "dense_wgrad_kernel launch");
  return 0;
}

int cnfot_recon_head(void* stream, const float* x, const float* xr, int64_t rows, int32_t dim, float weight,
                     float* g_xr, double* loss) {
  if (rows < 0 || dim < 1) return fail(CNFOT_ERR_ARG, "bad sizes");
  if (rows == 0) return 0;
  if (!x || !xr || !g_xr || !loss) return fail(CNFOT_ERR_ARG, "NULL buffer");
  const int64_t count = rows * dim;
  int64_t blocks = (count + 255) / 256;
  if (blocks > 148 * 8) blocks = 148 * 8;
  recon_head_kernel<<<(int)blocks, 256, 0, (cudaStream_t)stream>>>(x, xr, count, weight, g_xr, loss);
  cudaError_t e = cudaGetLastError();
  if (e != cudaSuccess) return cuda_fail(e, "recon_head_kernel launch");
  return 0;
}

int cnfot_mask_tail(void* stream, float* y, int64_t rows, int32_t dim, int32_t sub_dim) {
  if (rows < 0 || dim < 1 || sub_dim < 0 || sub_dim > dim) return fail(CNFOT_ERR_ARG, "bad sizes");
  if (rows == 0 || sub_dim == dim) return 0;
  if (!y) return fail(CNFOT_ERR_ARG, "NULL buffer");
  int64_t blocks = (rows * dim + 255) / 256;
  if (blocks > 148 * 8) blocks = 148 * 8;
  mask_tail_kernel<<<(int)blocks, 256, 0, (cudaStream_t)stream>>>(y, rows, dim, sub_dim);
  cudaError_t e = cudaGetLastError();
  if (e != cudaSuccess) return cuda_fail(e, "mask_tail_kernel launch");
  return 0;
}

int cnfot_adam_update(void* stream, float* params, const float* grads, float* m, float* v, int64_t count,
                      float lr, float b1, float b2, float eps, int64_t step) {
  if (count < 0 || step < 1) return fail(CNFOT_ERR_ARG, "bad count/step");
  if (count == 0) return 0;
  if (!params || !grads || !m || !v) return fail(CNFOT_ERR_ARG, "NULL buffer");
  DeviceInfo di;
  if (int rc = device_info(&di)) return rc;
  float c1 = (float)(1.0 - pow((double)b1, (double)step)), c2 = (float)(1.0 - pow((double)b2, (double)step));
  int threads = 256;
  int64_t blocks = (count + threads - 1) / threads;
  if (blocks > (int64_t)di.num_sms * 8) blocks = (int64_t)di.num_sms * 8;
  adam_kernel<<<(int)blocks, threads, 0, (cudaStream_t)stream>>>(params, grads, m, v, count, lr, b1, b2, eps, c1, c2);
  cudaError_t e = cudaGetLastError();
  if (e != cudaSuccess) return cuda_fail(e, "adam_kernel launch");
  return 0;
}

}
```

cnf_ot_b200/csrc/device_common.cuh:

```cuda
#pragma once

#include <cuda_runtime.h>
#include <stdint.h>

#include "flow_math.cuh"

namespace cnfot {

constexpr int kTile = 128;
constexpr int kWarps = kTile / 32;

__host__ __device__ inline bool tile_uses_swizzle(int n) {
  const int c = (n + 3) / 4;
  return c == 2 || c == 4 || (c >= 8 && c % 8 == 0);
}
__host__ __device__ inline int staged_stride(int n) {
  int q = (n + 3) / 4;
  if ((q & 1) == 0 && !tile_uses_swizzle(n)) q += 1;
  return q * 4;
}
__host__ __device__ inline int tile_swizzle(int n, int row) {
  if (!tile_uses_swizzle(n)) return 0;
  const int c = (n + 3) / 4;
  if (c == 2) return (row >> 2) & 1;
  if (c == 4) return (row >> 1) & 3;
  return row & 7;
}

struct SmemPlan {
  int total;
  int w_in_smem;
  int off_w;
  int w_stage;
  int off_acc;
  int off_in, ld_in;
  int off_hid, ld_h;
  int off_gh;
  int off_gth, ld_p;
  int off_lo;
  int off_wmma;
  int off_frag;
  int off_wt, wt_stride;
  int off_fk;
  int floats;
};

constexpr int kFirstKnotFloats = 128;
constexpr int kTileAlign = 128;
inline int align_up(int v, int a) { return (v + a - 1) / a * a; }

inline SmemPlan plan_smem(const FlowLayout& f, bool with_grad, bool w_in_smem = true,
                          bool tensor_cores = false) {
  SmemPlan p;
  p.total = f.total;
  p.w_in_smem = w_in_smem ? 1 : 0;
  const int tot4 = (f.total + 3) / 4 * 4;
  p.ld_in = staged_stride((f.D + 3) / 4 * 4);
  p.ld_h = staged_stride(f.H);
  p.ld_p = staged_stride(f.Pp);
  p.off_w = 0;
  p.w_stage = w_in_smem ? 0 : (f.D * f.H + f.mlp_const + 3) / 4 * 4;
  int o = w_in_smem ? tot4 : f.Pp + p.w_stage;
  p.off_acc = with_grad ? o : -1;
  if (with_grad) o += tot4;
  o = align_up(o, kTileAlign);
  p.off_in = o; o += kTile * p.ld_in;
  o = align_up(o, kTileAlign);
  p.off_hid = o; o += f.M * kTile * p.ld_h;
  p.off_gh = with_grad ? o : -1;
  if (with_grad) o += f.M * kTile * p.ld_h;
  p.off_gth = with_grad ? o : -1;
  if (with_grad) o += kTile * p.ld_p;
  p.off_lo = -1;
  p.off_wmma = -1;
  p.off_frag = -1;
  p.off_wt = -1;
  p.wt_stride = 0;
  if (tensor_cores) {
    o = align_up(o, kTileAlign);
    p.off_lo = o; o += kTile * 16;
    p.off_wmma = o; o += f.L * (f.D - 1) * f.M * 4 * 256;
  }
  o = align_up(o, 4);
  p.off_fk = o; o += kFirstKnotFloats;
  p.floats = o;
  return p;
}

__device__ inline void load_weights(float* sW, const float* __restrict__ gW, int total) {
  const int n4 = total >> 2;
  const float4* src = reinterpret_cast<const float4*>(gW);
  float4* dst = reinterpret_cast<float4*>(sW);
  for (int i = threadIdx.x; i < n4; i += blockDim.x) dst[i] = __ldg(src + i);
  for (int i = (n4 << 2) + threadIdx.x; i < total; i += blockDim.x) sW[i] = __ldg(gW + i);
}

template <int K, class SC>
__device__ __forceinline__ void first_knots_build_warp(const float* theta, const SC& c, FirstKnots<float, K>& fk) {
  static_assert(K + 1 <= 32, "one lane per knot");
  constexpr unsigned kAll = 0xffffffffu;
  const int k = threadIdx.x & 31;
  const bool bin = k < K;
  float pos[2], prob[2];
#pragma unroll
  for (int axis = 0; axis < 2; ++axis) {
    const float u = bin ? theta[axis * K + k] : -INFINITY;
    float m = u;
#pragma unroll
    for (int o = 16; o > 0; o >>= 1) m = fmaxf(m, __shfl_xor_sync(kAll, m, o));
    const float e = bin ? m_exp_shifted(u, m_exp_shift_prep(m)) : 0.f;
    float sum = e;
#pragma unroll
    for (int o = 16; o > 0; o >>= 1) sum += __shfl_xor_sync(kAll, sum, o);
    const float inv = m_rcp(sum);
    const float size = bin ? e * (inv * c.bin_scale) + c.min_bin : 0.f;
    prob[axis] = e * inv;
    float acc = size;
#pragma unroll
    for (int o = 1; o < 32; o <<= 1) {
      const float v = __shfl_up_sync(kAll, acc, o);
      if (k >= o) acc += v;
    }
    pos[axis] = c.lo + acc;
  }
  if (bin) {
    fk.pw[k] = prob[0];
    fk.ph[k] = prob[1];
    if (k + 1 <= K - 1) { fk.xp[k + 1] = pos[0]; fk.yp[k + 1] = pos[1]; }
  }
  if (k == 0) { fk.xp[0] = c.lo; fk.yp[0] = c.lo; fk.xp[K] = c.hi; fk.yp[K] = c.hi; }
  if (k <= K) {
    const float u = theta[2 * K + k] + c.slope_offset;
    fk.dk[k] = softplus(u) + c.min_slope;
    fk.sg[k] = sigmoid(u);
  }
}

template <class Net>
__device__ inline void build_first_knots(const float* first_smem, float* fk_smem) {
  static_assert(sizeof(FirstKnots<float, Net::kK>) <= kFirstKnotFloats * sizeof(float), "FirstKnots does not fit its slot");
  if (threadIdx.x < 32)
    first_knots_build_warp<Net::kK>(first_smem, FixedSplineConsts<float, Net::kK>(),
                                    *reinterpret_cast<FirstKnots<float, Net::kK>*>(fk_smem));
}

template <class Net>
__device__ inline RowTiles<float, Net> make_row_tiles(float* smem, const SmemPlan& p) {
  RowTiles<float, Net> tl;
  const int r = threadIdx.x;
  tl.in = smem + p.off_in + r * p.ld_in;
#pragma unroll
  for (int m = 0; m < Net::kM; ++m) {
    tl.hid[m] = smem + p.off_hid + (m * kTile + r) * p.ld_h;
    tl.gh[m] = p.off_gh >= 0 ? smem + p.off_gh + (m * kTile + r) * p.ld_h : nullptr;
  }
  tl.gth = p.off_gth >= 0 ? smem + p.off_gth + r * p.ld_p : nullptr;
  tl.sw_h = tile_swizzle(Net::kH, r);
  tl.sw_p = tile_swizzle(Net::kPp, r);
  return tl;
}

template <class Net>
struct DeviceCtx {
  using NetT = Net;
  static constexpr bool kWarpMlp = false;
  static constexpr bool kAccInGlobal = false;
  __device__ __forceinline__ void bind_partials(float*, bool = true) {}
  __device__ __forceinline__ void bind_frags(const float*) {}
  __device__ __forceinline__ void bind_stash(float*) {}
  __device__ __forceinline__ bool stash_on() const { return false; }
  static constexpr int H = Net::kH, M = Net::kM, Pp = Net::kPp;
  float* smem;
  const float* gW;
  SmemPlan p;

  __device__ __forceinline__ int row_in_tile() const { return threadIdx.x; }
  __device__ __forceinline__ void setup(int, int, uint64_t*, uint32_t*) { load(); }
  __device__ __forceinline__ void teardown() {}

  __device__ __forceinline__ void load() {
    if (p.w_in_smem) load_weights(smem + p.off_w, gW, p.total);
    else load_weights(smem + p.off_w, gW, Pp);
    if (p.off_acc >= 0)
      for (int i = threadIdx.x; i < p.total; i += blockDim.x) smem[p.off_acc + i] = 0.f;
    __syncthreads();
    build_first_knots<Net>(smem + p.off_w, smem + p.off_fk);
    __syncthreads();
  }

  __device__ __forceinline__ const float* first_params() const { return smem + p.off_w; }
  __device__ __forceinline__ const FirstKnots<float, Net::kK>& first_knots() const {
    return *reinterpret_cast<const FirstKnots<float, Net::kK>*>(smem + p.off_fk);
  }

  __device__ __forceinline__ const float* weights(int w_off, int count) {
    if (p.w_in_smem) return smem + p.off_w + w_off;
    __syncthreads();
    float* dst = smem + p.off_w + Pp;
    const float4* src = reinterpret_cast<const float4*>(gW + w_off);
    for (int i = threadIdx.x; i < (count >> 2); i += blockDim.x)
      reinterpret_cast<float4*>(dst)[i] = __ldg(src + i);
    __syncthreads();
    return dst;
  }

  __device__ __forceinline__ void begin() { __syncthreads(); }

  template <int K, int N>
  __device__ __forceinline__ void dense_fwd(const float* xt, int sw, const float*, const float* Wm, int, float* y) {
    dense_fwd_from_tile<float, K, N>(xt, sw, Wm, y);
  }
  template <int K, int N>
  __device__ __forceinline__ void dense_bwd(const float*, int, const float* g, const float* Wm, int, float* y) {
    dense_bwd_from_regs<float, K, N>(g, Wm, y);
  }

  __device__ __forceinline__ void block_accumulate(const float* pa, int lda, const float* pg,
                                                   int ldg, float* c) {
#pragma unroll 4
    for (int k = 0; k < kTile / 8; ++k) {
      const float4 g4 = *reinterpret_cast<const float4*>(pg + k * 8 * ldg);
      const float4 a4 = *reinterpret_cast<const float4*>(pa + k * 8 * lda);
      c[0] += a4.x * g4.x; c[1] += a4.x * g4.y; c[2] += a4.x * g4.z; c[3] += a4.x * g4.w;
      c[4] += a4.y * g4.x; c[5] += a4.y * g4.y; c[6] += a4.y * g4.z; c[7] += a4.y * g4.w;
      c[8] += a4.z * g4.x; c[9] += a4.z * g4.y; c[10] += a4.z * g4.z; c[11] += a4.z * g4.w;
      c[12] += a4.w * g4.x; c[13] += a4.w * g4.y; c[14] += a4.w * g4.z; c[15] += a4.w * g4.w;
    }
  }

  __device__ __noinline__ void reduce(int w_off, int n_in) {
    const int lane = threadIdx.x & 31, warp = threadIdx.x >> 5;
    const int rg = lane & 7, slot = lane >> 3;
    constexpr int CH = H / 4, CP = Pp / 4;
    const int nb0 = ((n_in + 3) >> 2) * CH;
    constexpr int nbm = CH * CH;
    constexpr int nbo = CH * CP;
    const int total = nb0 + (M - 1) * nbm + nbo;
    float* acc = smem + p.off_acc + w_off;
    const float* t_in = smem + p.off_in;
    const float* t_hid = smem + p.off_hid;
    const float* t_gh = smem + p.off_gh;
    const float* t_gth = smem + p.off_gth;
    const int off_hidden0 = n_in * H + H;
    for (int base = warp * 4; base < total; base += 4 * kWarps) {
      const int b = base + slot;
      const bool valid = b < total;
      const float *pa = t_in, *pg = t_gh;
      int lda = p.ld_in, ldg = p.ld_h, Na = n_in, ncol = H, rb = 0, cb = 0;
      float* dst = acc;
      if (valid) {
        if (b < nb0) {
          rb = b / CH; cb = b - rb * CH;
        } else if (b < nb0 + (M - 1) * nbm) {
          const int q = b - nb0;
          const int m = 1 + q / nbm;
          const int r = q - (m - 1) * nbm;
          rb = r / CH; cb = r - rb * CH;
          pa = t_hid + (m - 1) * kTile * p.ld_h; lda = p.ld_h; Na = H;
          pg = t_gh + m * kTile * p.ld_h;
          dst = acc + off_hidden0 + (m - 1) * (H * H + H);
        } else {
          const int r = b - nb0 - (M - 1) * nbm;
          rb = r / CP; cb = r - rb * CP;
          pa = t_hid + (M - 1) * kTile * p.ld_h; lda = p.ld_h; Na = H;
          pg = t_gth; ldg = p.ld_p; ncol = Pp;
          dst = acc + off_hidden0 + (M - 1) * (H * H + H);
        }
      }
      float c[16];
#pragma unroll
      for (int e = 0; e < 16; ++e) c[e] = 0.f;
      if (valid) {
        const int sa = pa == t_in ? 0 : tile_swizzle(H, rg);
        const int sg = ncol == H ? tile_swizzle(H, rg) : tile_swizzle(Pp, rg);
        block_accumulate(pa + rg * lda + ((rb ^ sa) << 2), lda, pg + rg * ldg + ((cb ^ sg) << 2), ldg, c);
      }
      const bool b2 = lane & 4, b1 = lane & 2, b0 = lane & 1;
      float v8[8], v4[4], v2[2];
#pragma unroll
      for (int q = 0; q < 8; ++q) {
        const float keep = b2 ? c[8 + q] : c[q], send = b2 ? c[q] : c[8 + q];
        v8[q] = keep + __shfl_xor_sync(0xffffffffu, send, 4);
      }
#pragma unroll
      for (int q = 0; q < 4; ++q) {
        const float keep = b1 ? v8[4 + q] : v8[q], send = b1 ? v8[q] : v8[4 + q];
        v4[q] = keep + __shfl_xor_sync(0xffffffffu, send, 2);
      }
#pragma unroll
      for (int q = 0; q < 2; ++q) {
        const float keep = b0 ? v4[2 + q] : v4[q], send = b0 ? v4[q] : v4[2 + q];
        v2[q] = keep + __shfl_xor_sync(0xffffffffu, send, 1);
      }
      const int row = rb * 4 + (b2 ? 2 : 0) + (b1 ? 1 : 0);
      if (valid && row < Na) {
        float2* q = reinterpret_cast<float2*>(dst + row * ncol + cb * 4 + (b0 ? 2 : 0));
        float2 cur = *q;
        cur.x += v2[0];
        cur.y += v2[1];
        *q = cur;
      }
    }
    constexpr int tasks = M * CH + CP;
    for (int task = warp; task < tasks; task += kWarps) {
      const float* pg;
      int ldg, cb;
      float* dst;
      if (task < M * CH) {
        const int m = task / CH;
        cb = task - m * CH;
        pg = t_gh + m * kTile * p.ld_h; ldg = p.ld_h;
        dst = m == 0 ? acc + n_in * H : acc + off_hidden0 + (m - 1) * (H * H + H) + H * H;
      } else {
        cb = task - M * CH;
        pg = t_gth; ldg = p.ld_p;
        dst = acc + off_hidden0 + (M - 1) * (H * H + H) + H * Pp;
      }
      float4 s = make_float4(0.f, 0.f, 0.f, 0.f);
      const int sg = task < M * CH ? tile_swizzle(H, lane) : tile_swizzle(Pp, lane);
#pragma unroll
      for (int k = 0; k < kTile / 32; ++k) {
        const float4 g4 = *reinterpret_cast<const float4*>(pg + (k * 32 + lane) * ldg + ((cb ^ sg) << 2));
        s.x += g4.x; s.y += g4.y; s.z += g4.z; s.w += g4.w;
      }
#pragma unroll
      for (int o = 16; o > 0; o >>= 1) {
        s.x += __shfl_xor_sync(0xffffffffu, s.x, o);
        s.y += __shfl_xor_sync(0xffffffffu, s.y, o);
        s.z += __shfl_xor_sync(0xffffffffu, s.z, o);
        s.w += __shfl_xor_sync(0xffffffffu, s.w, o);
      }
      if (lane == 0) {
        float4* q = reinterpret_cast<float4*>(dst + cb * 4);
        float4 cur = *q;
        cur.x += s.x; cur.y += s.y; cur.z += s.z; cur.w += s.w;
        *q = cur;
      }
    }
  }

  __device__ __forceinline__ void commit(int w_off, int n_in, const RowTiles<float, Net>&) {
    __syncthreads();
    reduce(w_off, n_in);
  }

  __device__ __forceinline__ void flush_first(const float* gfirst, const RowTiles<float, Net>& tl) {
    __syncthreads();
#pragma unroll
    for (int j = 0; j < Pp; j += 4)
      *reinterpret_cast<float4*>(tl.gth + chunk_at(j, tl.sw_p)) =
          make_float4(gfirst[j], gfirst[j + 1], gfirst[j + 2], gfirst[j + 3]);
    __syncthreads();
    const int lane = threadIdx.x & 31, warp = threadIdx.x >> 5;
    const float* pg = smem + p.off_gth;
    for (int cb = warp; cb < Pp / 4; cb += kWarps) {
      float4 s = make_float4(0.f, 0.f, 0.f, 0.f);
      const int sg = tile_swizzle(Pp, lane);
#pragma unroll
      for (int k = 0; k < kTile / 32; ++k) {
        const float4 g4 = *reinterpret_cast<const float4*>(pg + (k * 32 + lane) * p.ld_p + ((cb ^ sg) << 2));
        s.x += g4.x; s.y += g4.y; s.z += g4.z; s.w += g4.w;
      }
#pragma unroll
      for (int o = 16; o > 0; o >>= 1) {
        s.x += __shfl_xor_sync(0xffffffffu, s.x, o);
        s.y += __shfl_xor_sync(0xffffffffu, s.y, o);
        s.z += __shfl_xor_sync(0xffffffffu, s.z, o);
        s.w += __shfl_xor_sync(0xffffffffu, s.w, o);
      }
      if (lane == 0) {
        float4* q = reinterpret_cast<float4*>(smem + p.off_acc + cb * 4);
        float4 cur = *q;
        cur.x += s.x; cur.y += s.y; cur.z += s.z; cur.w += s.w;
        *q = cur;
      }
    }
    __syncthreads();
  }
};

__device__ inline double block_sum(double v, double* scratch ) {
#pragma unroll
  for (int o = 16; o > 0; o >>= 1) v += __shfl_xor_sync(0xffffffffu, v, o);
  __syncthreads();
  if ((threadIdx.x & 31) == 0) scratch[threadIdx.x >> 5] = v;
  __syncthreads();
  double t = 0.0;
  if (threadIdx.x == 0)
    for (int w = 0; w < kWarps; ++w) t += scratch[w];
  return t;
}

}
```

cnf_ot_b200/csrc/dispatch.h:

```cpp
#pragma once

#include "flow_math.cuh"

namespace cnfot {

const void* find_flow_eval_kernel(const FlowLayout& f, int engine = 0);
const void* find_flow_vjp_kernel(const FlowLayout& f, int engine = 0);
const void* find_mfc_step_kernel(const FlowLayout& f, int engine = 0, bool split = false, bool latency = false);
const void* find_energy_kernel(const FlowLayout& f, int engine = 0);
const void* find_density_kernel(const FlowLayout& f, int engine = 0);
inline bool tc_available(const FlowLayout& f) { return f.H == 16 && f.K == 5 && f.D >= 2 && f.M <= 3; }

#define CNFOT_NET_LIST(X) \
  X(16, 5, 2)             \
  X(16, 5, 1)             \
  X(16, 5, 3)             \
  X(32, 8, 2)             \
  X(32, 5, 2)             \
  X(64, 5, 2)             \
  X(8, 3, 1)

}
```

cnf_ot_b200/csrc/flow_eval.cu:

```cuda
#include "dispatch.h"
#include "flow_kernels.cuh"

namespace cnfot {

#define EVAL_CASE(H_, K_, M_)                                                            \
  if (f.H == H_ && f.K == K_ && f.M == M_)                                               \
    return (const void*)&flow_eval_kernel<NetCfg<H_, K_, M_>, Dims<0, 0>, kEngCuda>;
#define VJP_CASE(H_, K_, M_)                                                             \
  if (f.H == H_ && f.K == K_ && f.M == M_)                                               \
    return (const void*)&flow_vjp_kernel<NetCfg<H_, K_, M_>, Dims<0, 0>, kEngCuda>;
#define EVAL_ENG_CASE(M_, E_)                                                            \
  if (f.M == M_) return (const void*)&flow_eval_kernel<NetCfg<16, 5, M_>, Dims<0, 0>, E_>;
#define VJP_ENG_CASE(M_, E_)                                                             \
  if (f.M == M_) return (const void*)&flow_vjp_kernel<NetCfg<16, 5, M_>, Dims<0, 0>, E_>;

const void* find_flow_eval_kernel(const FlowLayout& f, int engine) {
  if (engine == kEngTc && tc_available(f)) {
    EVAL_ENG_CASE(1, kEngTc) EVAL_ENG_CASE(2, kEngTc) EVAL_ENG_CASE(3, kEngTc)
    return nullptr;
  }
  if (engine == kEngMma && tc_available(f)) {
    if (f.M == 2 && f.D == 2 && f.L == 2)
      return (const void*)&flow_eval_kernel<NetCfg<16, 5, 2>, Dims<2, 2>, kEngMma>;
    EVAL_ENG_CASE(1, kEngMma) EVAL_ENG_CASE(2, kEngMma) EVAL_ENG_CASE(3, kEngMma)
    return nullptr;
  }
  if (engine == kEngMmaStream && tc_available(f)) {
    EVAL_ENG_CASE(1, kEngMmaStream) EVAL_ENG_CASE(2, kEngMmaStream) EVAL_ENG_CASE(3, kEngMmaStream)
    return nullptr;
  }
  if (f.H == 16 && f.K == 5 && f.M == 2 && f.D == 2 && f.L == 2)
    return (const void*)&flow_eval_kernel<NetCfg<16, 5, 2>, Dims<2, 2>, kEngCuda>;
  CNFOT_NET_LIST(EVAL_CASE)
  return nullptr;
}

const void* find_flow_vjp_kernel(const FlowLayout& f, int engine) {
  if (engine == kEngTc && tc_available(f)) {
    VJP_ENG_CASE(1, kEngTc) VJP_ENG_CASE(2, kEngTc) VJP_ENG_CASE(3, kEngTc)
    return nullptr;
  }
  if (engine == kEngMma && tc_available(f)) {
    if (f.M == 2 && f.D == 2 && f.L == 2)
      return (const void*)&flow_vjp_kernel<NetCfg<16, 5, 2>, Dims<2, 2>, kEngMma>;
    VJP_ENG_CASE(1, kEngMma) VJP_ENG_CASE(2, kEngMma) VJP_ENG_CASE(3, kEngMma)
    return nullptr;
  }
  if (engine == kEngMmaStream && tc_available(f)) {
    VJP_ENG_CASE(1, kEngMmaStream) VJP_ENG_CASE(2, kEngMmaStream) VJP_ENG_CASE(3, kEngMmaStream)
    return nullptr;
  }
  if (f.H == 16 && f.K == 5 && f.M == 2 && f.D == 2 && f.L == 2)
    return (const void*)&flow_vjp_kernel<NetCfg<16, 5, 2>, Dims<2, 2>, kEngCuda>;
  CNFOT_NET_LIST(VJP_CASE)
  return nullptr;
}

#define ENERGY_CASE(H_, K_, M_)                                                          \
  if (f.H == H_ && f.K == K_ && f.M == M_)                                               \
    return (const void*)&energy_kernel<NetCfg<H_, K_, M_>, Dims<0, 0>, kEngCuda>;
#define ENERGY_ENG_CASE(M_, E_)                                                          \
  if (f.M == M_) return (const void*)&energy_kernel<NetCfg<16, 5, M_>, Dims<0, 0>, E_>;

const void* find_energy_kernel(const FlowLayout& f, int engine) {
  if (engine == kEngMma && tc_available(f)) {
    if (f.M == 2 && f.D == 2 && f.L == 2)
      return (const void*)&energy_kernel<NetCfg<16, 5, 2>, Dims<2, 2>, kEngMma>;
    ENERGY_ENG_CASE(1, kEngMma) ENERGY_ENG_CASE(2, kEngMma) ENERGY_ENG_CASE(3, kEngMma)
    return nullptr;
  }
  if (engine == kEngMmaStream && tc_available(f)) {
    ENERGY_ENG_CASE(1, kEngMmaStream) ENERGY_ENG_CASE(2, kEngMmaStream) ENERGY_ENG_CASE(3, kEngMmaStream)
    return nullptr;
  }
  CNFOT_NET_LIST(ENERGY_CASE)
  return nullptr;
}

#define DENSITY_CASE(H_, K_, M_)                                                         \
  if (f.H == H_ && f.K == K_ && f.M == M_)                                               \
    return (const void*)&density_kernel<NetCfg<H_, K_, M_>, Dims<0, 0>, kEngCuda>;
#define DENSITY_ENG_CASE(M_, E_)                                                         \
  if (f.M == M_) return (const void*)&density_kernel<NetCfg<16, 5, M_>, Dims<0, 0>, E_>;

const void* find_density_kernel(const FlowLayout& f, int engine) {
  if (engine == kEngMma && tc_available(f)) {
    if (f.M == 2 && f.D == 2 && f.L == 2)
      return (const void*)&density_kernel<NetCfg<16, 5, 2>, Dims<2, 2>, kEngMma>;
    DENSITY_ENG_CASE(1, kEngMma) DENSITY_ENG_CASE(2, kEngMma) DENSITY_ENG_CASE(3, kEngMma)
    return nullptr;
  }
  if (engine == kEngMmaStream && tc_available(f)) {
    DENSITY_ENG_CASE(1, kEngMmaStream) DENSITY_ENG_CASE(2, kEngMmaStream) DENSITY_ENG_CASE(3, kEngMmaStream)
    return nullptr;
  }
  CNFOT_NET_LIST(DENSITY_CASE)
  return nullptr;
}

}
```

cnf_ot_b200/csrc/flow_kernels.cuh:

```cuda
#pragma once

#include <type_traits>

#include "device_common.cuh"
#include "philox.cuh"
#include "step_math.cuh"
#include "tc_engine.cuh"
#include "warp_mlp.cuh"

namespace cnfot {

enum Engine { kEngCuda = 0, kEngTc = 1, kEngMma = 2, kEngMmaStream = 3, kEngWide = 4 };
#ifndef CNFOT_MMA_MIN_CTAS
#define CNFOT_MMA_MIN_CTAS 4
#endif
constexpr int kMmaMinCtas = CNFOT_MMA_MIN_CTAS;
#ifndef CNFOT_STEP_MIN_CTAS
#define CNFOT_STEP_MIN_CTAS 3
#endif
constexpr int kStepMinCtas = CNFOT_STEP_MIN_CTAS;
constexpr int kStepMinCtasStream = 4;
constexpr int kStepMinCtasStreamLatency = 2;
template <class Net, int ENG, int DC = 0, int LC = 0>
struct CtxSelect { using type = DeviceCtx<Net>; };
template <class Net, int DC, int LC>
struct CtxSelect<Net, kEngTc, DC, LC> { using type = DeviceCtxTC<Net>; };
template <class Net, int DC, int LC>
struct CtxSelect<Net, kEngMma, DC, LC> { using type = DeviceCtxMma<Net, true, DC, LC>; };
template <class Net, int DC, int LC>
struct CtxSelect<Net, kEngMmaStream, DC, LC> { using type = DeviceCtxMma<Net, false>; };

template <class Ctx>
__device__ __forceinline__ void ctx_setup(Ctx& ctx, int D, int L, uint64_t* mbar, uint32_t* slot) {
  ctx.setup(D, L, mbar, slot);
}
template <class Ctx>
__device__ __forceinline__ void ctx_teardown(Ctx& ctx) { ctx.teardown(); }

struct EvalArgs {
  const float* W;
  const float* frags;
  const float* in;
  const float* cond;
  int64_t cond_stride;
  int64_t rows;
  float* out;
  float* logdet;
  int dir;
  int add_base;
  int D, L;
  SmemPlan plan;
};

template <class Net, class DimsT, int ENG>
__global__ void __launch_bounds__(kTile, ENG >= kEngMma ? kMmaMinCtas : 1) flow_eval_kernel(EvalArgs a) {
  extern __shared__ __align__(1024) float smem[];
  __shared__ __align__(8) uint64_t tc_mbar;
  __shared__ uint32_t tc_slot;
  using Ctx = typename CtxSelect<Net, ENG>::type;
  Ctx ctx;
  ctx.smem = smem; ctx.gW = a.W; ctx.p = a.plan;
  ctx.bind_partials(nullptr);
  ctx.bind_frags(a.frags);
  ctx_setup(ctx, a.D, a.L, &tc_mbar, &tc_slot);
  const RowTiles<float, Net> tl = make_row_tiles<Net>(smem, a.plan);
  const DimsT dm{a.D, a.L};
  const int D = dm.D(), L = dm.L();
  for (int64_t tile = blockIdx.x; tile * kTile < a.rows; tile += gridDim.x) {
    const int64_t r = tile * kTile + ctx.row_in_tile();
    const bool live = r < a.rows;
    float st[kMaxStateFloats];
    for (int i = 0; i < D; ++i) st[i] = live ? a.in[r * D + i] : 0.f;
    const float t = live ? a.cond[r * a.cond_stride] : 0.f;
    float ld = a.dir == 0 ? flow_pass<0, float, Net, DimsT, Ctx>(dm, FixedSplineConsts<float, Net::kK>(), t, st, tl, ctx)
                          : flow_pass<1, float, Net, DimsT, Ctx>(dm, FixedSplineConsts<float, Net::kK>(), t, st, tl, ctx);
    if (!live) continue;
    for (int i = 0; i < D; ++i) a.out[r * D + i] = st[L * D + i];
    if (a.logdet) {
      if (a.add_base)
        ld = a.dir == 0 ? base_log_prob<float>(st, D) - ld
                        : base_log_prob<float>(st + L * D, D) + ld;
      a.logdet[r] = ld;
    }
  }
  ctx_teardown(ctx);
}

struct PartialBuf {
  float* grad;
  double* loss;
};

__device__ inline void flush_partials(const PartialBuf& pb, const float* sAcc, int total,
                                      const double* loss ,
                                      double* scratch) {
  __syncthreads();
  float* dst = pb.grad + (int64_t)blockIdx.x * total;
  if (sAcc)
    for (int i = threadIdx.x; i < total; i += blockDim.x) dst[i] = sAcc[i];
  for (int s = 0; s < kNumSlots; ++s) {
    double v = block_sum(loss[s], scratch);
    if (threadIdx.x == 0) pb.loss[(int64_t)blockIdx.x * kNumSlots + s] = v;
  }
}

struct VjpArgs {
  const float* W;
  const float* frags;
  const float* in;
  const float* cond;
  int64_t cond_stride;
  int64_t rows;
  const float* g_out;
  const float* g_logdet;
  float* g_in;
  int dir;
  int add_base;
  int D, L;
  SmemPlan plan;
  PartialBuf pb;
  float* stash;
  long long stash_cta_floats;
};

template <class Net, class DimsT, int ENG>
__global__ void __launch_bounds__(kTile, ENG >= kEngMma ? kMmaMinCtas : 1) flow_vjp_kernel(VjpArgs a) {
  extern __shared__ __align__(1024) float smem[];
  __shared__ double scratch[kWarps];
  __shared__ __align__(8) uint64_t tc_mbar;
  __shared__ uint32_t tc_slot;
  using Ctx = typename CtxSelect<Net, ENG>::type;
  float* sAcc = Ctx::kAccInGlobal ? nullptr : smem + a.plan.off_acc;
  Ctx ctx;
  ctx.smem = smem; ctx.gW = a.W; ctx.p = a.plan;
  ctx.bind_partials(a.pb.grad + (int64_t)blockIdx.x * a.plan.total);
  ctx.bind_frags(a.frags);
  ctx.bind_stash(a.stash ? a.stash + (size_t)blockIdx.x * a.stash_cta_floats : nullptr);
  ctx_setup(ctx, a.D, a.L, &tc_mbar, &tc_slot);
  const RowTiles<float, Net> tl = make_row_tiles<Net>(smem, a.plan);
  const DimsT dm{a.D, a.L};
  const int D = dm.D(), L = dm.L();
  FirstGrad<float, Net::kK> gfirst;
#pragma unroll
  for (int j = 0; j <= Net::kK; ++j) { gfirst.gx[j] = 0.f; gfirst.gy[j] = 0.f; gfirst.gd[j] = 0.f; }
  for (int64_t tile = blockIdx.x; tile * kTile < a.rows; tile += gridDim.x) {
    const int64_t r = tile * kTile + ctx.row_in_tile();
    const bool live = r < a.rows;
    float st[kMaxStateFloats], g[kMaxDim];
    for (int i = 0; i < D; ++i) st[i] = live ? a.in[r * D + i] : 0.f;
    const float t = live ? a.cond[r * a.cond_stride] : 0.f;
    const bool stash = ctx.stash_on();
    if (a.dir == 0) flow_pass<0, float, Net, DimsT, Ctx>(dm, FixedSplineConsts<float, Net::kK>(), t, st, tl, ctx, stash);
    else flow_pass<1, float, Net, DimsT, Ctx>(dm, FixedSplineConsts<float, Net::kK>(), t, st, tl, ctx, stash);
    const float gl = (live && a.g_logdet) ? a.g_logdet[r] : 0.f;
    for (int i = 0; i < D; ++i) g[i] = live ? a.g_out[r * D + i] : 0.f;
    float gl_pass = gl;
    if (a.add_base) {
      if (a.dir == 0) gl_pass = -gl;
      else
        for (int i = 0; i < D; ++i) g[i] -= gl * st[L * D + i];
    }
    if (a.dir == 0)
      flow_pass_bwd<0, float, Net, DimsT, Ctx>(dm, FixedSplineConsts<float, Net::kK>(), t, st, g, gl_pass, gfirst, tl, ctx, stash);
    else
      flow_pass_bwd<1, float, Net, DimsT, Ctx>(dm, FixedSplineConsts<float, Net::kK>(), t, st, g, gl_pass, gfirst, tl, ctx, stash);
    if (a.add_base && a.dir == 0)
      for (int i = 0; i < D; ++i) g[i] -= gl * st[i];
    if (live && a.g_in)
      for (int i = 0; i < D; ++i) a.g_in[r * D + i] = g[i];
  }
  {
    float graw[Net::kPp];
#pragma unroll
    for (int j = 0; j < Net::kPp; ++j) graw[j] = 0.f;
    first_grad_to_raw<float, Net::kK>(gfirst, ctx.first_knots(), FixedSplineConsts<float, Net::kK>(), graw);
    ctx.flush_first(graw, tl);
  }
  double zero[kNumSlots];
  for (int s = 0; s < kNumSlots; ++s) zero[s] = 0.0;
  flush_partials(a.pb, sAcc, a.plan.total, zero, scratch);
  ctx_teardown(ctx);
}

struct EnergyArgs {
  const float* W;
  const float* frags;
  int D, L;
  SmemPlan plan;
  const float* latent;
  int64_t batch;
  int latent_blocks;
  const float* t_dev;
  int n_t;
  int with_score;
  float dt, dx, kappa;
  double weight;
  int64_t tiles_per_t, n_tiles;
  unsigned long long* tile_counter;
  PartialBuf pb;
};

template <class Net, class DimsT, int ENG>
__global__ void __launch_bounds__(kTile, ENG >= kEngMma ? kMmaMinCtas : 1) energy_kernel(const __grid_constant__ EnergyArgs a) {
  extern __shared__ __align__(1024) float smem[];
  __shared__ double scratch[kWarps];
  __shared__ long long s_tile;
  __shared__ __align__(8) uint64_t tc_mbar;
  __shared__ uint32_t tc_slot;
  using Ctx = typename CtxSelect<Net, ENG>::type;
  Ctx ctx;
  ctx.smem = smem; ctx.gW = a.W; ctx.p = a.plan;
  ctx.bind_partials(nullptr);
  ctx.bind_frags(a.frags);
  ctx_setup(ctx, a.D, a.L, &tc_mbar, &tc_slot);
  const RowTiles<float, Net> tl = make_row_tiles<Net>(smem, a.plan);
  const DimsT dm{a.D, a.L};
  const int D = dm.D();
  double loss[kNumSlots];
#pragma unroll
  for (int s = 0; s < kNumSlots; ++s) loss[s] = 0.0;
  while (true) {
    __syncthreads();
    if (threadIdx.x == 0) s_tile = (long long)atomicAdd(a.tile_counter, 1ULL);
    __syncthreads();
    const long long tile = s_tile;
    if (tile >= a.n_tiles) break;
    const int ti = (int)(tile / a.tiles_per_t);
    const int64_t r = (tile - (long long)ti * a.tiles_per_t) * kTile + ctx.row_in_tile();
    const bool live = r < a.batch;
    const float* src = a.latent + ((int64_t)(ti % a.latent_blocks) * a.batch + r) * D;
    float row[kMaxDim];
    for (int i = 0; i < D; ++i) row[i] = live ? src[i] : 0.f;
    const float v2 = row_kinetic_value<float, Net, DimsT, Ctx>(dm, FixedSplineConsts<float, Net::kK>(), a.t_dev[ti], row, a.dt, a.with_score != 0,
                                                               a.kappa, a.dx, tl, ctx);
    if (live) loss[kSlotKinetic] += (double)v2 * a.weight;
  }
  flush_partials(a.pb, nullptr, 0, loss, scratch);
  ctx_teardown(ctx);
}

struct DensityArgs {
  const float* W;
  const float* frags;
  int D, L;
  SmemPlan plan;
  int mode;
  int nx, ny, n_t;
  double x_min, x_step, y_min, y_step;
  const float* t_dev;
  unsigned long long key_n;
  uint32_t step;
  float cond;
  int64_t n;
  float* density;
  float* samples;
  int with_ref;
  float mix, var0, var1;
  PartialBuf pb;
};

template <class Net, class DimsT, int ENG>
__global__ void __launch_bounds__(kTile, ENG >= kEngMma ? kMmaMinCtas : 1) density_kernel(const __grid_constant__ DensityArgs a) {
  extern __shared__ __align__(1024) float smem[];
  __shared__ double scratch[kWarps];
  __shared__ __align__(8) uint64_t tc_mbar;
  __shared__ uint32_t tc_slot;
  using Ctx = typename CtxSelect<Net, ENG>::type;
  Ctx ctx;
  ctx.smem = smem; ctx.gW = a.W; ctx.p = a.plan;
  ctx.bind_partials(nullptr);
  ctx.bind_frags(a.frags);
  ctx_setup(ctx, a.D, a.L, &tc_mbar, &tc_slot);
  const RowTiles<float, Net> tl = make_row_tiles<Net>(smem, a.plan);
  const DimsT dm{a.D, a.L};
  const int D = dm.D(), L = dm.L();
  const FixedSplineConsts<float, Net::kK> sc;
  double loss[kNumSlots];
#pragma unroll
  for (int s = 0; s < kNumSlots; ++s) loss[s] = 0.0;
  const float half_log_2pi = 0.91893853320467274178f;
  for (int64_t tile = blockIdx.x; tile * kTile < a.n; tile += gridDim.x) {
    const int64_t r = tile * kTile + ctx.row_in_tile();
    const bool live = r < a.n;
    float st[kMaxStateFloats];
    for (int i = 0; i < D; ++i) st[i] = 0.f;
    float t = a.cond, lp;
    const float* y;
    if (a.mode == 0) {
      const int64_t per_t = (int64_t)a.nx * a.ny;
      const int ti = live ? (int)(r / per_t) : 0;
      const int64_t q = live ? r - (int64_t)ti * per_t : 0;
      const int iy = (int)(q / a.nx), ix = (int)(q - (int64_t)iy * a.nx);
      st[0] = (float)(a.x_min + (double)ix * a.x_step);
      st[1] = (float)(a.y_min + (double)iy * a.y_step);
      t = a.t_dev[ti];
      const float ld = flow_pass<1, float, Net, DimsT, Ctx>(dm, sc, t, st, tl, ctx);
      lp = base_log_prob<float>(st + L * D, D) + ld;
      y = st;
    } else {
      if (live) philox_row(a.key_n, a.key_n, a.step, kRowsNormal, (uint64_t)r, D, st);
      const float fldj = flow_pass<0, float, Net, DimsT, Ctx>(dm, sc, t, st, tl, ctx);
      lp = base_log_prob<float>(st, D) - fldj;
      y = st + L * D;
      if (live && a.samples)
        for (int i = 0; i < D; ++i) a.samples[r * D + i] = y[i];
    }
    if (!live) continue;
    const float p = m_exp(lp);
    if (a.density) a.density[r] = p;
    if (a.with_ref) {
      float r2 = 0.f;
      for (int i = 0; i < D; ++i) r2 += y[i] * y[i];
      const float p0 = m_exp(-0.5f * r2 / a.var0 - (float)D * (half_log_2pi + 0.5f * m_log(a.var0)));
      const float p1 = m_exp(-0.5f * r2 / a.var1 - (float)D * (half_log_2pi + 0.5f * m_log(a.var1)));
      const float e = p - (p0 * (1.f - a.mix) + p1 * a.mix);
      loss[kSlotKinetic] += (double)e * (double)e;
    }
  }
  flush_partials(a.pb, nullptr, 0, loss, scratch);
  ctx_teardown(ctx);
}

enum SegmentKind { kSegNll = 0, kSegSample = 1, kSegKinetic = 2, kSegKineticSplit = 3  };

struct Segment {
  int kind;
  int slot;
  int do_fit, do_pot;
  int source;
  int t_index;
  float t;
  const float* rows;
  int64_t row0;
  int64_t n;
  int64_t first_tile;
  int group;
};

constexpr int kMaxSegments = 36;

enum SyncWord { kSyncTile = 0 , kSyncDone = 2, kSyncStatus = 4, kSyncDoneBase = 5, kSyncSeq = 6,
                kSyncTileBase = 8  };
constexpr int kStateWordOffset = 16;
constexpr int kLossRowOffset = 24;
constexpr int kStepRows = 32;

struct PeerArgs {
  int rank, world;
  uint32_t epoch;
  int stride;
  unsigned long long timeout_ns;
  unsigned long long* xbuf[8];
  uint32_t* flags[8];
};

struct TailArgs {
  int n_rows;
  int n_tail;
  int total;
  int accumulate;
  int self_clean;
  long long n_tiles;
  uint32_t* sync;
  double* loss_row;
  float* grad_rows;
  float* out;
  float* weights;
  float* adam_m;
  float* adam_v;
  float lr, b1, b2, eps;
  unsigned long long* state;
  float* loss_hist;
  long long loss_hist_len;
  PeerArgs pa;
};

struct StepArgs {
  const float* W;
  const float* frags;
  int D, L;
  SmemPlan plan;
  StepConsts<float> pc;
  int n_seg;
  int64_t n_tiles;
  float* stash;
  long long stash_cta_floats;
  unsigned long long key;
  unsigned long long salt_B, salt_Bc, salt_b, salt_t;
  uint32_t step;
  unsigned long long* timeline;
  Segment seg[kMaxSegments];
  TailArgs tail;
};

__device__ __forceinline__ uint32_t ld_acquire_gpu(const uint32_t* p) {
  uint32_t v;
  asm volatile("ld.acquire.gpu.global.u32 %0, [%1];" : "=r"(v) : "l"(p) : "memory");
  return v;
}
__device__ __forceinline__ uint32_t ld_acquire_sys(const uint32_t* p) {
  uint32_t v;
  asm volatile("ld.acquire.sys.global.u32 %0, [%1];" : "=r"(v) : "l"(p) : "memory");
  return v;
}
__device__ __forceinline__ void st_release_sys(uint32_t* p, uint32_t v) {
  asm volatile("st.release.sys.global.u32 [%0], %1;" ::"l"(p), "r"(v) : "memory");
}
__device__ __forceinline__ unsigned long long global_timer_ns() {
  unsigned long long v;
  asm volatile("mov.u64 %0, %globaltimer;" : "=l"(v));
  return v;
}

__device__ __forceinline__ void adam_one(const TailArgs& t, int i, float g, float c1, float c2, float m0, float v0, float w0) {
  const float mi = t.b1 * m0 + (1.f - t.b1) * g;
  const float vi = t.b2 * v0 + (1.f - t.b2) * g * g;
  t.adam_m[i] = mi;
  t.adam_v[i] = vi;
  t.weights[i] = w0 - t.lr * (mi / c1) / (sqrtf(vi / c2) + t.eps);
}

__device__ __forceinline__ void st_relaxed_sys_u64(unsigned long long* p, unsigned long long v) {
  asm volatile("st.relaxed.sys.global.u64 [%0], %1;" ::"l"(p), "l"(v) : "memory");
}
__device__ __forceinline__ unsigned long long ld_relaxed_sys_u64(const unsigned long long* p) {
  unsigned long long v;
  asm volatile("ld.relaxed.sys.global.u64 %0, [%1];" : "=l"(v) : "l"(p) : "memory");
  return v;
}

struct LaunchHeader {
  uint32_t done_base, seq, stepno, epoch;
  unsigned long long tile_base;
};

static __device__ __noinline__ void step_tail(const TailArgs& t, const LaunchHeader& h) {
  __shared__ unsigned s_ticket;
  __shared__ int s_bad;
  const int tid = threadIdx.x;
  __threadfence();
  __syncthreads();
  if (tid == 0) s_ticket = atomicAdd(t.sync + kSyncDone, 1u) - h.done_base;
  __syncthreads();
  const unsigned grid = gridDim.x, S = (unsigned)t.n_tail, ticket = s_ticket;
  if (ticket >= S) return;
  const int k = (int)ticket;
  const int total = t.total, n_out = total + kNumSlots;
  const bool dp = t.pa.world > 1;
  const uint32_t stepno = h.stepno, epoch = h.epoch;
  double* const loss_row = t.loss_row + 4 * (h.seq & 1u);
  float c1 = 1.f, c2 = 1.f;
  if (t.weights) {
    const float n1 = (float)stepno + 1.f;
    c1 = -expm1f(n1 * logf(t.b1));
    c2 = -expm1f(n1 * logf(t.b2));
  }
  const size_t par_off = (size_t)(epoch & 1u) * t.pa.world * t.pa.stride;
  if (tid == 0) {
    while (ld_acquire_gpu(t.sync + kSyncDone) - h.done_base < grid) __nanosleep(20);
    s_bad = (dp && ld_acquire_sys(t.pa.flags[t.pa.rank]) != 0u) ? 1 : 0;
    if (k == 0) {
      t.sync[kSyncDoneBase] = h.done_base + grid;
      t.sync[kSyncSeq] = h.seq + 1u;
      *reinterpret_cast<unsigned long long*>(t.sync + kSyncTileBase) = h.tile_base + (unsigned long long)t.n_tiles + grid;
      double* other = t.loss_row + 4 * ((h.seq & 1u) ^ 1u);
      other[0] = 0.0; other[1] = 0.0; other[2] = 0.0; other[3] = 0.0;
      if (t.state) {
        t.state[1] = (unsigned long long)h.stepno + 1ULL;
        t.state[2] = (unsigned long long)h.epoch + 1ULL;
      }
    }
  }
  __syncthreads();

  auto finish = [&](int col, float v, float m0, float v0, float w0) {
    if (col < total) {
      if (t.out) t.out[col] = t.accumulate ? t.out[col] + v : v;
      if (t.weights && v == v) adam_one(t, col, v, c1, c2, m0, v0, w0);
    } else {
      const int sl = col - total;
      if (t.out) t.out[col] = sl <= 4 ? (t.accumulate ? t.out[col] + v : v) : 0.f;
      if (sl == 0 && t.loss_hist && (long long)stepno < t.loss_hist_len) t.loss_hist[stepno] = v;
    }
  };

  const int stride_cols = (int)S * (int)(blockDim.x >> 2);
  const int rg = tid & 3;
  const bool owner = rg == 0;
  const unsigned long long* mybuf = dp ? t.pa.xbuf[t.pa.rank] + par_off : nullptr;
  const uint32_t* abort_word = dp ? t.pa.flags[t.pa.rank] : nullptr;
  const int n_cols = (n_out + 7) & ~7;
  for (int col = k * (int)(blockDim.x >> 2) + (tid >> 2); col < n_cols; col += stride_cols) {
    double acc = 0.0;
    float m0 = 0.f, v0 = 0.f, w0 = 0.f;
    if (t.weights && owner && col < total) {
      m0 = __ldcg(t.adam_m + col); v0 = __ldcg(t.adam_v + col); w0 = __ldcg(t.weights + col);
    }
    if (col < total) {
      float* p = t.grad_rows + col;
      for (int r0 = rg; r0 < t.n_rows; r0 += 32) {
        float v[8];
#pragma unroll
        for (int q = 0; q < 8; ++q) v[q] = r0 + 4 * q < t.n_rows ? __ldcg(p + (size_t)(r0 + 4 * q) * total) : 0.f;
#pragma unroll
        for (int q = 0; q < 8; ++q) acc += (double)v[q];
        if (t.self_clean) {
#pragma unroll
          for (int q = 0; q < 8; ++q)
            if (r0 + 4 * q < t.n_rows) __stcg(p + (size_t)(r0 + 4 * q) * total, 0.f);
        }
      }
    } else if (col < n_out && owner) {
      const int sl = col - total;
      if (sl == 0) acc = __ldcg(loss_row) + __ldcg(loss_row + 1) + __ldcg(loss_row + 2) + __ldcg(loss_row + 3);
      else if (sl <= 4) acc = __ldcg(loss_row + sl - 1);
    }
    acc += __shfl_xor_sync(0xffffffffu, acc, 1);
    acc += __shfl_xor_sync(0xffffffffu, acc, 2);
    if (!owner || col >= n_out) continue;
    const float mine = (float)acc;
    if (!dp) {
      finish(col, mine, m0, v0, w0);
      continue;
    }
    const unsigned long long word = ((unsigned long long)epoch << 32) | (unsigned long long)__float_as_uint(mine);
    for (int p = 0; p < t.pa.world; ++p)
      st_relaxed_sys_u64(t.pa.xbuf[p] + par_off + (size_t)t.pa.rank * t.pa.stride + col, word);
    bool bad = *(volatile int*)&s_bad != 0;
    float sum = 0.f;
    if (!bad) {
      const unsigned long long* w0 = mybuf + col;
      unsigned long long v[8];
#pragma unroll
      for (int q = 0; q < 8; ++q) v[q] = q < t.pa.world ? ld_relaxed_sys_u64(w0 + (size_t)q * t.pa.stride) : 0ULL;
#pragma unroll
      for (int q = 0; q < 8; ++q) {
        if (q >= t.pa.world || bad) continue;
        if ((uint32_t)(v[q] >> 32) != epoch) {
          const unsigned long long* w = w0 + (size_t)q * t.pa.stride;
          const unsigned long long t0 = global_timer_ns();
          unsigned spins = 0;
          while ((uint32_t)((v[q] = ld_relaxed_sys_u64(w)) >> 32) != epoch) {
            if ((++spins & 255u) == 0u &&
                (ld_acquire_sys(abort_word) != 0u || global_timer_ns() - t0 > t.pa.timeout_ns)) {
              bad = true;
              break;
            }
          }
        }
        sum += __uint_as_float((uint32_t)v[q]);
      }
    }
    if (bad) {
      for (int p = 0; p < t.pa.world; ++p) st_release_sys(t.pa.flags[p], 1u);
      s_bad = 1;
      t.sync[kSyncStatus] = 1u;
      sum = __int_as_float(0x7fc00000);
    }
    finish(col, sum, m0, v0, w0);
  }
}

template <class Net, class DimsT, int ENG, bool SPLIT = false, bool LAT = false>
__global__ void __launch_bounds__(kTile, ENG == kEngMmaStream ? (LAT || SPLIT ? kStepMinCtasStreamLatency : kStepMinCtasStream)
                                                              : (ENG >= kEngMma ? kStepMinCtas : 1))
mfc_step_kernel(const __grid_constant__ StepArgs a) {
  extern __shared__ __align__(1024) float smem[];
  __shared__ double scratch4[kWarps][4];
  __shared__ long long s_tile;
  __shared__ LaunchHeader s_hdr;
  __shared__ __align__(8) uint64_t tc_mbar;
  __shared__ uint32_t tc_slot;
  using Ctx = typename CtxSelect<Net, ENG, DimsT::kD, DimsT::kL>::type;
  asm volatile("griddepcontrol.wait;" ::: "memory");
  if (threadIdx.x == 0) {
    s_hdr.done_base = __ldcg(a.tail.sync + kSyncDoneBase);
    s_hdr.seq = __ldcg(a.tail.sync + kSyncSeq);
    s_hdr.tile_base = __ldcg(reinterpret_cast<const unsigned long long*>(a.tail.sync + kSyncTileBase));
    s_hdr.stepno = a.tail.state ? (uint32_t)__ldcg(a.tail.state + 1) : 0u;
    s_hdr.epoch = a.tail.state && a.tail.pa.world > 1 ? (uint32_t)__ldcg(a.tail.state + 2) : a.tail.pa.epoch;
  }
  unsigned long long t_start = 0;
  if (a.timeline && threadIdx.x == 0) { t_start = global_timer_ns(); atomicMin(a.timeline + 0, t_start); atomicMax(a.timeline + 7, t_start); }
  float* sAcc = Ctx::kAccInGlobal ? nullptr : smem + a.plan.off_acc;
  float* my_row = a.tail.grad_rows + (int64_t)(blockIdx.x % a.tail.n_rows) * a.plan.total;
  Ctx ctx;
  ctx.smem = smem; ctx.gW = a.W; ctx.p = a.plan;
  ctx.bind_partials(my_row, false);
  ctx.bind_frags(a.frags);
  ctx.bind_stash(a.stash ? a.stash + (size_t)blockIdx.x * a.stash_cta_floats : nullptr);
  ctx_setup(ctx, DimsT{a.D, a.L}.D(), DimsT{a.D, a.L}.L(), &tc_mbar, &tc_slot);
  if (a.timeline && threadIdx.x == 0) { const unsigned long long now = global_timer_ns(); atomicMax(a.timeline + 1, now); atomicMax(a.timeline + 6, now - t_start); }
  const RowTiles<float, Net> tl = make_row_tiles<Net>(smem, a.plan);
  const DimsT dm{a.D, a.L};
  const int D = dm.D();
  unsigned long long key = a.key;
  uint32_t step = a.step;
  if (a.tail.state) {
    key = __ldcg(a.tail.state);
    step = (uint32_t)__ldcg(a.tail.state + 1);
  }
  unsigned long long* tile_counter = reinterpret_cast<unsigned long long*>(a.tail.sync + kSyncTile);
  FirstGrad<float, Net::kK> gfirst;
#pragma unroll
  for (int j = 0; j <= Net::kK; ++j) { gfirst.gx[j] = 0.f; gfirst.gy[j] = 0.f; gfirst.gd[j] = 0.f; }
  double loss[kNumSlots];
#pragma unroll
  for (int s = 0; s < kNumSlots; ++s) loss[s] = 0.0;

  while (true) {
    __syncthreads();
    if (threadIdx.x == 0) s_tile = (long long)(atomicAdd(tile_counter, 1ULL) - s_hdr.tile_base);
    __syncthreads();
    const long long tile = s_tile;
    if (tile >= a.n_tiles) break;
    int si = 0;
    while (si + 1 < a.n_seg && tile >= a.seg[si + 1].first_tile) ++si;
    const Segment& sg = a.seg[si];
    const bool split = SPLIT && sg.kind == kSegKineticSplit;
    const int64_t r = split ? (tile - sg.first_tile) * (kTile / sg.group) + (int)threadIdx.x / sg.group
                            : (tile - sg.first_tile) * kTile + ctx.row_in_tile();
    const bool live = r < sg.n;
    float row[kMaxDim];
    if (sg.source == kRowsMemory) {
      for (int i = 0; i < D; ++i) row[i] = live ? sg.rows[r * D + i] : 0.f;
    } else {
      for (int i = 0; i < D; ++i) row[i] = 0.f;
      if (live)
        philox_row(key ^ (sg.kind >= kSegKinetic ? a.salt_b : a.salt_B), key ^ a.salt_Bc, step, sg.source,
                   (uint64_t)(sg.row0 + r), D, row);
    }
    const float tval = sg.t_index >= 0 ? philox_time(key ^ a.salt_t, step, sg.t_index, a.pc.horizon) : sg.t;
    if (sg.kind == kSegNll) {
      float v = row_nll<float, Net, DimsT, Ctx>(dm, FixedSplineConsts<float, Net::kK>(), tval, row,
                                                           live ? a.pc.w_fit : 0.f, gfirst, tl, ctx);
      loss[sg.slot] += (double)v;
    } else if (sg.kind == kSegSample) {
      StepConsts<float> pc = a.pc;
      if (!live) { pc.w_fit = 0.f; pc.w_pot = 0.f; }
      float lf = 0.f, lp = 0.f;
      row_sample_terms<float, Net, DimsT, Ctx>(dm, FixedSplineConsts<float, Net::kK>(), tval, row, sg.do_fit != 0,
                                                          sg.do_pot != 0, pc, &lf, &lp, gfirst, tl, ctx);
      loss[sg.slot] += (double)lf;
      loss[kSlotPotential] += (double)lp;
    } else {
      StepConsts<float> pc = a.pc;
      if (!live) { pc.w_kin = 0.f; pc.w_pot = 0.f; }
      float lk = 0.f, lp = 0.f;
      if constexpr (SPLIT)
        row_kinetic_split<Net, DimsT, Ctx>(dm, FixedSplineConsts<float, Net::kK>(), tval, row, pc, sg.group, &lk, &lp,
                                           gfirst, tl, ctx);
      else
        row_kinetic<float, Net, DimsT, Ctx>(dm, FixedSplineConsts<float, Net::kK>(), tval, row, pc, &lk, &lp, gfirst,
                                            tl, ctx);
      loss[kSlotKinetic] += (double)lk;
      loss[kSlotPotential] += (double)lp;
    }
  }
  asm volatile("griddepcontrol.launch_dependents;");
  if (a.timeline && threadIdx.x == 0) {
    const unsigned long long now = global_timer_ns();
    atomicMin(a.timeline + 2, now);
    atomicMax(a.timeline + 3, now);
  }
  {
    float graw[Net::kPp];
#pragma unroll
    for (int j = 0; j < Net::kPp; ++j) graw[j] = 0.f;
    first_grad_to_raw<float, Net::kK>(gfirst, ctx.first_knots(), FixedSplineConsts<float, Net::kK>(), graw);
    ctx.flush_first(graw, tl);
  }
  __syncthreads();
  if (sAcc)
    for (int i = threadIdx.x; i < a.plan.total; i += blockDim.x) {
      const float v = sAcc[i];
      if (v != 0.f) atomicAdd(my_row + i, v);
    }
  {
#pragma unroll
    for (int s = 0; s < 4; ++s) {
      double v = loss[s];
#pragma unroll
      for (int o = 16; o > 0; o >>= 1) v += __shfl_xor_sync(0xffffffffu, v, o);
      if ((threadIdx.x & 31) == 0) scratch4[threadIdx.x >> 5][s] = v;
    }
    __syncthreads();
    if (threadIdx.x < 4) {
      double v = 0.0;
#pragma unroll
      for (int w = 0; w < kWarps; ++w) v += scratch4[w][threadIdx.x];
      if (v != 0.0) atomicAdd(a.tail.loss_row + 4 * (s_hdr.seq & 1u) + threadIdx.x, v);
    }
  }
  ctx_teardown(ctx);
  if (a.timeline && threadIdx.x == 0) atomicMax(a.timeline + 4, global_timer_ns());
  step_tail(a.tail, s_hdr);
  if (a.timeline && threadIdx.x == 0) atomicMax(a.timeline + 5, global_timer_ns());
}

}
```

cnf_ot_b200/csrc/step.cu:

```cuda
#include "dispatch.h"
#include "flow_kernels.cuh"

namespace cnfot {

const void* find_mfc_step_kernel_tc(const FlowLayout& f);
const void* find_mfc_step_kernel_mma(const FlowLayout& f);
const void* find_mfc_step_kernel_mma_stream(const FlowLayout& f);
const void* find_mfc_step_kernel_cuda(const FlowLayout& f);
const void* find_mfc_step_kernel_tc_split(const FlowLayout& f);
const void* find_mfc_step_kernel_mma_split(const FlowLayout& f);
const void* find_mfc_step_kernel_mma_stream_split(const FlowLayout& f);
const void* find_mfc_step_kernel_mma_stream_lat(const FlowLayout& f);
const void* find_mfc_step_kernel_cuda_split(const FlowLayout& f);

const void* find_mfc_step_kernel(const FlowLayout& f, int engine, bool split, bool latency) {
  if (engine == kEngTc && tc_available(f)) return split ? find_mfc_step_kernel_tc_split(f) : find_mfc_step_kernel_tc(f);
  if (engine == kEngMma && tc_available(f)) return split ? find_mfc_step_kernel_mma_split(f) : find_mfc_step_kernel_mma(f);
  if (engine == kEngMmaStream && tc_available(f))
    return split ? find_mfc_step_kernel_mma_stream_split(f)
                 : (latency ? find_mfc_step_kernel_mma_stream_lat(f) : find_mfc_step_kernel_mma_stream(f));
  return split ? find_mfc_step_kernel_cuda_split(f) : find_mfc_step_kernel_cuda(f);
}

}
```

cnf_ot_b200/csrc/step_mma.cu:

```cuda
#ifndef CNFOT_STEP_SPLIT
#define CNFOT_STEP_SPLIT 0
#endif
#include "dispatch.h"
#include "flow_kernels.cuh"

namespace cnfot {

#define STEP_ENG_CASE(M_, E_) \
  if (f.M == M_) return (const void*)&mfc_step_kernel<NetCfg<16, 5, M_>, Dims<0, 0>, E_, CNFOT_STEP_SPLIT != 0>;

#if CNFOT_STEP_SPLIT
const void* find_mfc_step_kernel_mma_split(const FlowLayout& f) {
#else
const void* find_mfc_step_kernel_mma(const FlowLayout& f) {
#endif
  if (f.M == 2 && f.D == 2 && f.L == 2)
    return (const void*)&mfc_step_kernel<NetCfg<16, 5, 2>, Dims<2, 2>, kEngMma, CNFOT_STEP_SPLIT != 0>;
  STEP_ENG_CASE(1, kEngMma) STEP_ENG_CASE(2, kEngMma) STEP_ENG_CASE(3, kEngMma)
  return nullptr;
}

}
```

cnf_ot_b200/csrc/warp_mlp.cuh:

```cuda
#pragma once

#include "device_common.cuh"

namespace cnfot {

constexpr int kWtFloats = 32 * 16;
constexpr int kFragFloats = 1024;

__device__ __forceinline__ void mma_tf32(float (&d)[4], const uint32_t (&a)[4], uint32_t b0, uint32_t b1) {
  asm volatile(
      "mma.sync.aligned.m16n8k8.row.col.f32.tf32.tf32.f32 {%0,%1,%2,%3}, {%4,%5,%6,%7}, {%8,%9}, {%0,%1,%2,%3};"
      : "+f"(d[0]), "+f"(d[1]), "+f"(d[2]), "+f"(d[3])
      : "r"(a[0]), "r"(a[1]), "r"(a[2]), "r"(a[3]), "r"(b0), "r"(b1));
}

#if defined(CNFOT_TF32_TRUNC)
__device__ __forceinline__ uint32_t tf32_round(float v) { return __float_as_uint(v) & 0xFFFFE000u; }
#else
__device__ __forceinline__ uint32_t tf32_round(float v) { return (__float_as_uint(v) + 0x00001000u) & 0xFFFFE000u; }
#endif
__device__ __forceinline__ void split_tf32(float v, uint32_t& hi, uint32_t& lo) {
  hi = tf32_round(v);
  lo = __float_as_uint(v - __uint_as_float(hi));
}

__host__ __device__ inline int cw_layer_stride(int D, int M) { return 16 * ((D - 1) * (D + 2) / 2) + (D - 1) * (M + 1) * 16; }
__host__ __device__ inline int cw_offset(int D, int M, int Pp, int layer, int d) {
  return Pp + layer * cw_layer_stride(D, M) + 16 * ((d - 1) * (d + 2) / 2) + (d - 1) * (M + 1) * 16;
}
__host__ __device__ inline int cw_floats(int D, int L, int M, int Pp) { return Pp + L * cw_layer_stride(D, M); }

inline SmemPlan plan_smem_mma(const FlowLayout& f, bool with_grad, bool resident = true) {
  SmemPlan p;
  p.total = f.total;
  p.w_in_smem = resident ? 1 : 0;
  p.ld_in = p.ld_h = p.ld_p = 0;
  p.off_w = 0;
  p.w_stage = 0;
  int o = resident ? cw_floats(f.D, f.L, f.M, f.Pp) : f.Pp;
  p.off_acc = -1;
  p.off_in = p.off_hid = p.off_gh = p.off_gth = p.off_lo = p.off_wmma = -1;
  o = align_up(o, 32);
  p.off_frag = o;
  if (resident) o += f.L * (f.D - 1) * f.M * kFragFloats;
  p.off_wt = o;
  p.wt_stride = (with_grad ? f.M + 1 : 1) * kWtFloats;
  o += kWarps * p.wt_stride;
  p.off_fk = o; o += kFirstKnotFloats;
  p.floats = o;
  return p;
}

__device__ __forceinline__ float lds32(uint32_t a) {
  float v;
  asm volatile("ld.shared.f32 %0, [%1];" : "=f"(v) : "r"(a));
  return v;
}
__device__ __forceinline__ float2 lds64(uint32_t a) {
  float2 v;
  asm volatile("ld.shared.v2.f32 {%0,%1}, [%2];" : "=f"(v.x), "=f"(v.y) : "r"(a));
  return v;
}
__device__ __forceinline__ float4 lds128(uint32_t a) {
  float4 v;
  asm volatile("ld.shared.v4.f32 {%0,%1,%2,%3}, [%4];" : "=f"(v.x), "=f"(v.y), "=f"(v.z), "=f"(v.w) : "r"(a));
  return v;
}
__device__ __forceinline__ float2 ldw64(uint32_t a) {
  float2 v;
  asm("ld.shared.v2.f32 {%0,%1}, [%2];" : "=f"(v.x), "=f"(v.y) : "r"(a));
  return v;
}
__device__ __forceinline__ float4 ldw128(uint32_t a) {
  float4 v;
  asm("ld.shared.v4.f32 {%0,%1,%2,%3}, [%4];" : "=f"(v.x), "=f"(v.y), "=f"(v.z), "=f"(v.w) : "r"(a));
  return v;
}
__device__ __forceinline__ void sts32(uint32_t a, float x) {
  asm volatile("st.shared.f32 [%0], %1;" ::"r"(a), "f"(x) : "memory");
}
__device__ __forceinline__ void sts64(uint32_t a, float x, float y) {
  asm volatile("st.shared.v2.f32 [%0], {%1,%2};" ::"r"(a), "f"(x), "f"(y) : "memory");
}
__device__ __forceinline__ void sts128(uint32_t a, float x, float y, float z, float w) {
  asm volatile("st.shared.v4.f32 [%0], {%1,%2,%3,%4};" ::"r"(a), "f"(x), "f"(y), "f"(z), "f"(w) : "memory");
}
__device__ __forceinline__ void red_global(float* q, float v) {
  asm volatile("red.global.add.f32 [%0], %1;" ::"l"(q), "f"(v) : "memory");
}
__device__ __forceinline__ void red_global2(float* q, float x, float y) {
  asm volatile("red.global.add.v2.f32 [%0], {%1,%2};" ::"l"(q), "f"(x), "f"(y) : "memory");
}

template <bool RES>
struct WRef;
template <>
struct WRef<true> {
  uint32_t a;
  __device__ __forceinline__ WRef operator+(int floats) const { return WRef{a + (uint32_t)floats * 4u}; }
  __device__ __forceinline__ float2 ld2() const { return ldw64(a); }
  __device__ __forceinline__ float4 ld4() const { return ldw128(a); }
  __device__ __forceinline__ bool valid() const { return a != 0u; }
  __device__ __forceinline__ static WRef none() { return WRef{0u}; }
};
template <>
struct WRef<false> {
  const float* q;
  __device__ __forceinline__ WRef operator+(int floats) const { return WRef{q + floats}; }
  __device__ __forceinline__ float2 ld2() const { return __ldg(reinterpret_cast<const float2*>(q)); }
  __device__ __forceinline__ float4 ld4() const { return __ldg(reinterpret_cast<const float4*>(q)); }
  __device__ __forceinline__ bool valid() const { return q != nullptr; }
  __device__ __forceinline__ static WRef none() { return WRef{nullptr}; }
};

template <bool LDG = true>
__device__ __forceinline__ float4 frag_element(const float* __restrict__ blob, int D, int M, int e) {
  constexpr int H = 16, Pp = 16;
  const int ln = e & 31, ksnt = (e >> 5) & 3, dir = (e >> 7) & 1, mat = e >> 8;
  const int mlp = mat / M, slot = mat - mlp * M;
  const int layer = mlp / (D - 1), d = mlp - layer * (D - 1) + 1;
  const int mlp_const = H + (M - 1) * (H * H + H) + H * Pp + Pp;
  const int layer_stride = (D - 1) * mlp_const + H * ((D - 1) * (D + 2) / 2);
  const float* Ws = blob + Pp + layer * layer_stride + (d - 1) * mlp_const + H * ((d - 1) * (d + 2) / 2) +
                    (d + 1) * H + H + slot * (H * H + H);
  const int ks = ksnt >> 1, nt = ksnt & 1, gg = ln >> 2, tt = ln & 3;
  float b0, b1;
  const float* q0 = dir == 0 ? Ws + (8 * ks + 2 * tt) * 16 + 8 * nt + gg : Ws + (8 * nt + gg) * 16 + 8 * ks + 2 * tt;
  const float* q1 = q0 + (dir == 0 ? 16 : 1);
  if constexpr (LDG) { b0 = __ldg(q0); b1 = __ldg(q1); }
  else { b0 = *q0; b1 = *q1; }
  uint32_t h0, l0, h1, l1;
  split_tf32(b0, h0, l0);
  split_tf32(b1, h1, l1);
  return make_float4(__uint_as_float(h0), __uint_as_float(h1), __uint_as_float(l0), __uint_as_float(l1));
}

static __global__ void build_frags_kernel(const float* __restrict__ blob, float* __restrict__ frags, int D, int M,
                                   int n_mat) {
  for (int e = blockIdx.x * blockDim.x + threadIdx.x; e < n_mat * 256; e += gridDim.x * blockDim.x)
    reinterpret_cast<float4*>(frags)[e] = frag_element(blob, D, M, e);
}

struct MmaLane {
  uint32_t lane, g, t;
  uint32_t cbase;
  uint32_t cu;
  uint32_t rbase;
  uint32_t ru;
  uint32_t tbase;
  uint32_t tu;
  __device__ __forceinline__ MmaLane() {
    lane = threadIdx.x & 31;
    g = lane >> 2;
    t = lane & 3;
    const uint32_t fg = ((g >> 1) & 1) * 2 + ((g >> 2) & 1);
    cbase = (g * 16 + 2 * (t & 1)) * 4;
    cu = (t >> 1) ^ fg;
    rbase = (8 * t + g) * 64;
    ru = t ^ fg;
    tbase = (t * 16 + (g & 3)) * 4;
    tu = (g >> 2) ^ (t & 2);
  }
};

__device__ __forceinline__ uint32_t dyn_smem_base() {
  extern __shared__ __align__(1024) float cnfot_dyn_smem[];
  return (uint32_t)__cvta_generic_to_shared(cnfot_dyn_smem);
}
__device__ __forceinline__ float* dyn_smem_ptr() {
  extern __shared__ __align__(1024) float cnfot_dyn_smem[];
  return cnfot_dyn_smem;
}

template <class Net, bool RES, int DC = 0, int LC = 0>
struct DeviceCtxMma {
  using NetT = Net;
  using Ref = WRef<RES>;
  static constexpr bool kConstPlan = RES && DC > 0 && LC > 0;
  static constexpr int kcW = 0;
  static constexpr int kcCw = Net::kPp + LC * (16 * ((DC - 1) * (DC + 2) / 2) + (DC - 1) * (Net::kM + 1) * 16);
  static constexpr int kcFrag = (kcCw + 31) / 32 * 32;
  static constexpr int kcWt = kcFrag + LC * (DC - 1) * Net::kM * kFragFloats;
  static constexpr int kcWtStride = (Net::kM + 1) * kWtFloats;
  static constexpr int kcFk = kcWt + kWarps * kcWtStride;
  __device__ __forceinline__ Ref wref() const {
    if constexpr (kConstPlan) return Ref{dyn_smem_base() + (uint32_t)kcW * 4u};
    else return w_ref;
  }
  __device__ __forceinline__ Ref fref() const {
    if constexpr (kConstPlan) return Ref{dyn_smem_base() + (uint32_t)kcFrag * 4u};
    else return frag_ref;
  }
  __device__ __forceinline__ uint32_t swt() const {
    if constexpr (kConstPlan) return dyn_smem_base() + ((uint32_t)kcWt + (threadIdx.x >> 5) * (uint32_t)kcWtStride) * 4u;
    else return s_wt;
  }
  static constexpr bool kWarpMlp = true;
  static constexpr bool kAccInGlobal = true;
  static constexpr int H = Net::kH, M = Net::kM, Pp = Net::kPp;
  static_assert(H == 16 && Pp == 16, "the warp-MMA engine is written for 16-wide layers");
  float* smem;
  const float* gW;
  SmemPlan p;
  float* gacc;
  const float* gfrag;
  Ref w_ref, frag_ref;
  uint32_t s_wt;
  float* stash = nullptr;
  static constexpr int kStateFloats = 2 * Net::kK + 10;
  static constexpr int kStateChunks = (kStateFloats + 3) / 4;
  static constexpr int kStashChunks = 4 * M + kStateChunks;
  static constexpr int kStashCondFloats = kStashChunks * kTile * 4;
  __device__ __forceinline__ void bind_stash(float* q) { stash = q; }
  __device__ __forceinline__ bool stash_on() const { return stash != nullptr; }
  __device__ __forceinline__ float* stash_of(int D, int layer, int d) const {
    return stash + (size_t)(layer * (D - 1) + d - 1) * kStashCondFloats + threadIdx.x * 4;
  }
  __device__ __forceinline__ static void stash_put(float* q, int chunk0, const float (&v)[2][2][4]) {
#pragma unroll
    for (int c = 0; c < 4; ++c)
      __stcg(reinterpret_cast<float4*>(q + (chunk0 + c) * kTile * 4),
             make_float4(v[c >> 1][c & 1][0], v[c >> 1][c & 1][1], v[c >> 1][c & 1][2], v[c >> 1][c & 1][3]));
  }
  __device__ __forceinline__ void stash_state(int D, int layer, int d, const SplineState<float, Net::kK>& st) const {
    constexpr int K = Net::kK;
    float b[kStateChunks * 4];
#pragma unroll
    for (int k = 0; k < K; ++k) { b[k] = st.pw[k]; b[K + k] = st.ph[k]; }
    b[2 * K] = st.x0; b[2 * K + 1] = st.x1; b[2 * K + 2] = st.y0; b[2 * K + 3] = st.y1;
    b[2 * K + 4] = st.d0; b[2 * K + 5] = st.d1; b[2 * K + 6] = st.u0; b[2 * K + 7] = st.u1;
    b[2 * K + 8] = st.u_tail;
    b[2 * K + 9] = __int_as_float(st.idx | (st.tail << 8));
#pragma unroll
    for (int j = kStateFloats; j < kStateChunks * 4; ++j) b[j] = 0.f;
    float* q = stash_of(D, layer, d) + 4 * M * kTile * 4;
#pragma unroll
    for (int c = 0; c < kStateChunks; ++c)
      __stcg(reinterpret_cast<float4*>(q + c * kTile * 4), make_float4(b[4 * c], b[4 * c + 1], b[4 * c + 2], b[4 * c + 3]));
  }

  bool clear_acc;
  __device__ __forceinline__ void bind_partials(float* q, bool clear = true) { gacc = q; clear_acc = clear; }
  __device__ __forceinline__ void bind_frags(const float* q) { gfrag = q; }

  __device__ __forceinline__ int row_in_tile() const {
    const int lane = threadIdx.x & 31;
    return (threadIdx.x & ~31) + 8 * (lane & 3) + (lane >> 2);
  }

  __device__ __forceinline__ void setup(int D, int L, uint64_t*, uint32_t*) {
    const uint32_t s0 = (uint32_t)__cvta_generic_to_shared(smem);
    s_wt = s0 + (p.off_wt + (threadIdx.x >> 5) * p.wt_stride) * 4;
    if constexpr (kConstPlan) {
      if (D != DC || L != LC || p.off_w != kcW || p.off_frag != kcFrag || p.off_wt != kcWt || p.wt_stride != kcWtStride ||
          p.off_fk != kcFk || smem != dyn_smem_ptr())
        __trap();
    }
    if (gacc && clear_acc)
      for (int i = threadIdx.x; i < p.total; i += blockDim.x) gacc[i] = 0.f;
    if constexpr (RES) {
      w_ref = Ref{s0 + (uint32_t)p.off_w * 4u};
      frag_ref = Ref{s0 + (uint32_t)p.off_frag * 4u};
      float* stage = smem + p.off_wt;
      const bool staged = p.total <= kWarps * p.wt_stride;
      if (staged) {
        load_weights(stage, gW, p.total);
        __syncthreads();
      }
      const float* blob = staged ? stage : gW;
      for (int i = threadIdx.x; i < Pp; i += blockDim.x) smem[p.off_w + i] = blob[i];
      for (int mlp = 0; mlp < L * (D - 1); ++mlp) {
        const int layer = mlp / (D - 1), d = mlp - layer * (D - 1) + 1;
        const float* src = blob + mlp_offset<Net>(D, layer, d);
        float* dst = smem + p.off_w + cw_offset(D, M, Pp, layer, d);
        const int n0 = (d + 2) * 16;
        for (int i = threadIdx.x; i < n0 + M * 16; i += blockDim.x) {
          int so = i;
          if (i >= n0) {
            const int m = (i - n0) >> 4, j = i & 15;
            so = n0 + m * (H * H + H) + H * H + j;
          }
          dst[i] = src[so];
        }
      }
      const int n_mat = L * (D - 1) * M;
      const int nb = (int)blockDim.x - 32;
      if (staged) {
        if ((int)threadIdx.x >= nb) {
          first_knots_build_warp<Net::kK>(stage, FixedSplineConsts<float, Net::kK>(),
                                          *reinterpret_cast<FirstKnots<float, Net::kK>*>(smem + p.off_fk));
        } else {
          for (int e = threadIdx.x; e < n_mat * 256; e += nb)
            reinterpret_cast<float4*>(smem + p.off_frag)[e] = frag_element<false>(stage, D, M, e);
        }
        __syncthreads();
        return;
      }
      for (int e = threadIdx.x; e < n_mat * 256; e += blockDim.x)
        reinterpret_cast<float4*>(smem + p.off_frag)[e] = frag_element<true>(gW, D, M, e);
    } else {
      load_weights(smem + p.off_w, gW, Pp);
      w_ref = Ref{gW};
      frag_ref = Ref{gfrag};
    }
    __syncthreads();
    build_first_knots<Net>(smem + p.off_w, smem + p.off_fk);
    __syncthreads();
  }
  __device__ __forceinline__ void teardown() {}

  __device__ __forceinline__ const float* first_params() const { return smem + p.off_w; }
  __device__ __forceinline__ const FirstKnots<float, Net::kK>& first_knots() const {
    if constexpr (kConstPlan) return *reinterpret_cast<const FirstKnots<float, Net::kK>*>(dyn_smem_ptr() + kcFk);
    else return *reinterpret_cast<const FirstKnots<float, Net::kK>*>(smem + p.off_fk);
  }

  __device__ __forceinline__ static void store_c(uint32_t tile, const MmaLane& ln, const float (&x)[2][2][4]) {
#pragma unroll
    for (int q = 0; q < 4; ++q)
#pragma unroll
      for (int nt = 0; nt < 2; ++nt)
        sts64(tile + ln.cbase + q * 512 + 16 * (ln.cu ^ (2 * nt ^ q)), x[q >> 1][nt][2 * (q & 1)],
              x[q >> 1][nt][2 * (q & 1) + 1]);
  }
  __device__ __forceinline__ static void store_a(uint32_t tile, const MmaLane& ln, const float (&a)[2][2][4]) {
#pragma unroll
    for (int q = 0; q < 4; ++q)
#pragma unroll
      for (int nt = 0; nt < 2; ++nt) {
        const uint32_t ad = tile + ln.cbase + q * 512 + 16 * (ln.cu ^ (2 * nt ^ q));
        sts32(ad, a[q >> 1][nt][q & 1]);
        sts32(ad + 4, a[q >> 1][nt][(q & 1) + 2]);
      }
  }
  __device__ __forceinline__ static void load_c(uint32_t tile, const MmaLane& ln, float (&x)[2][2][4]) {
#pragma unroll
    for (int q = 0; q < 4; ++q)
#pragma unroll
      for (int nt = 0; nt < 2; ++nt) {
        const float2 v = lds64(tile + ln.cbase + q * 512 + 16 * (ln.cu ^ (2 * nt ^ q)));
        x[q >> 1][nt][2 * (q & 1)] = v.x;
        x[q >> 1][nt][2 * (q & 1) + 1] = v.y;
      }
  }
  __device__ __forceinline__ static void store_row(uint32_t tile, const MmaLane& ln, const float* v) {
#pragma unroll
    for (int c = 0; c < 4; ++c)
      sts128(tile + ln.rbase + 16 * (ln.ru ^ c), v[4 * c], v[4 * c + 1], v[4 * c + 2], v[4 * c + 3]);
  }
  __device__ __forceinline__ static void load_row(uint32_t tile, const MmaLane& ln, float* v) {
#pragma unroll
    for (int c = 0; c < 4; ++c) {
      const float4 q = lds128(tile + ln.rbase + 16 * (ln.ru ^ c));
      v[4 * c] = q.x; v[4 * c + 1] = q.y; v[4 * c + 2] = q.z; v[4 * c + 3] = q.w;
    }
  }

  __device__ __forceinline__ static void dense16(const float (&a)[2][2][4], Ref frag, Ref bias,
                                                 const MmaLane& ln, float (&o)[2][2][4]) {
    float2 c0 = make_float2(0.f, 0.f), c1 = c0;
    if (bias.valid()) {
      c0 = (bias + 2 * ln.t).ld2();
      c1 = (bias + 8 + 2 * ln.t).ld2();
    }
#pragma unroll
    for (int mt = 0; mt < 2; ++mt) {
      o[mt][0][0] = c0.x; o[mt][0][1] = c0.y; o[mt][0][2] = c0.x; o[mt][0][3] = c0.y;
      o[mt][1][0] = c1.x; o[mt][1][1] = c1.y; o[mt][1][2] = c1.x; o[mt][1][3] = c1.y;
    }
    const Ref fr = frag + ln.lane * 4;
#pragma unroll
    for (int ks = 0; ks < 2; ++ks) {
      uint32_t ahi[2][4], alo[2][4];
#pragma unroll
      for (int mt = 0; mt < 2; ++mt)
#pragma unroll
        for (int e = 0; e < 4; ++e) split_tf32(a[mt][ks][e], ahi[mt][e], alo[mt][e]);
#pragma unroll
      for (int nt = 0; nt < 2; ++nt) {
        const float4 f = (fr + (ks * 2 + nt) * 128).ld4();
        const uint32_t bh0 = __float_as_uint(f.x), bh1 = __float_as_uint(f.y);
        const uint32_t bl0 = __float_as_uint(f.z), bl1 = __float_as_uint(f.w);
#pragma unroll
        for (int mt = 0; mt < 2; ++mt) {
          mma_tf32(o[mt][nt], alo[mt], bh0, bh1);
          mma_tf32(o[mt][nt], ahi[mt], bl0, bl1);
          mma_tf32(o[mt][nt], ahi[mt], bh0, bh1);
        }
      }
    }
  }

  __device__ __forceinline__ static void relu_to_a(const float (&c)[2][2][4], float (&a)[2][2][4]) {
#pragma unroll
    for (int mt = 0; mt < 2; ++mt)
#pragma unroll
      for (int nt = 0; nt < 2; ++nt) {
        a[mt][nt][0] = fmaxf(c[mt][nt][0], 0.f);
        a[mt][nt][1] = fmaxf(c[mt][nt][2], 0.f);
        a[mt][nt][2] = fmaxf(c[mt][nt][1], 0.f);
        a[mt][nt][3] = fmaxf(c[mt][nt][3], 0.f);
      }
  }

  __device__ __forceinline__ void cond_forward(int D, int layer, int d, float tval, const float* cvec,
                                               float* theta, bool keep, bool put = false) const {
    float* sq = put ? stash_of(D, layer, d) : nullptr;
    const MmaLane ln;
    const uint32_t wt = swt();
    const int n_in = d + 1, mlp = layer * (D - 1) + d - 1;
    const Ref W = wref() + (RES ? cw_offset(D, M, Pp, layer, d) : mlp_offset<Net>(D, layer, d));
    const Ref b0 = W + n_in * H;
    const Ref frag = fref() + mlp * M * kFragFloats;
    float x[2][2][4], a[2][2][4];
    {
      const float2 c0 = (b0 + 2 * ln.t).ld2();
      const float2 c1 = (b0 + 8 + 2 * ln.t).ld2();
#pragma unroll
      for (int mt = 0; mt < 2; ++mt) {
        x[mt][0][0] = c0.x; x[mt][0][1] = c0.y; x[mt][0][2] = c0.x; x[mt][0][3] = c0.y;
        x[mt][1][0] = c1.x; x[mt][1][1] = c1.y; x[mt][1][2] = c1.x; x[mt][1][3] = c1.y;
      }
    }
#pragma unroll 1
    for (int i = 0; i < n_in; ++i) {
      const float xi = i == 0 ? tval : cvec[perm_at(layer, i - 1, D)];
      const float2 w0 = (W + i * 16 + 2 * ln.t).ld2();
      const float2 w1 = (W + i * 16 + 8 + 2 * ln.t).ld2();
#pragma unroll
      for (int q = 0; q < 4; ++q) {
        const float xq = __shfl_sync(0xffffffffu, xi, (ln.lane & ~3u) | q);
        float* a0 = x[q >> 1][0] + 2 * (q & 1);
        float* a1 = x[q >> 1][1] + 2 * (q & 1);
        a0[0] = fmaf(xq, w0.x, a0[0]); a0[1] = fmaf(xq, w0.y, a0[1]);
        a1[0] = fmaf(xq, w1.x, a1[0]); a1[1] = fmaf(xq, w1.y, a1[1]);
      }
    }
    relu_to_a(x, a);
    if (keep) {
      __syncwarp();
      store_a(wt, ln, a);
    }
    if (put) stash_put(sq, 0, a);
    Ref bm = RES ? b0 + H : b0 + (H + H * H);
#pragma unroll
    for (int m = 1; m < M; ++m) {
      dense16(a, frag + (m - 1) * kFragFloats, bm, ln, x);
      relu_to_a(x, a);
      if (keep) store_a(wt + m * kWtFloats * 4, ln, a);
      if (put) stash_put(sq, 4 * m, a);
      bm = bm + (RES ? H : H * H + H);
    }
    dense16(a, frag + (M - 1) * kFragFloats, bm, ln, x);
    const uint32_t scratch = wt + (keep ? M : 0) * kWtFloats * 4;
    __syncwarp();
    store_c(scratch, ln, x);
    __syncwarp();
    load_row(scratch, ln, theta);
  }

  __device__ __forceinline__ void cond_restore(int D, int layer, int d, SplineState<float, Net::kK>& st, float min_slope) const {
    constexpr int K = Net::kK;
    const MmaLane ln;
    const uint32_t wt = swt();
    const float* sq = stash_of(D, layer, d);
    float4 f[kStashChunks];
#pragma unroll
    for (int c = 0; c < kStashChunks; ++c) f[c] = __ldcg(reinterpret_cast<const float4*>(sq + c * kTile * 4));
    __syncwarp();
#pragma unroll
    for (int m = 0; m < M; ++m) {
      float a[2][2][4];
#pragma unroll
      for (int c = 0; c < 4; ++c) {
        const float4 v = f[4 * m + c];
        a[c >> 1][c & 1][0] = v.x; a[c >> 1][c & 1][1] = v.y; a[c >> 1][c & 1][2] = v.z; a[c >> 1][c & 1][3] = v.w;
      }
      store_a(wt + m * kWtFloats * 4, ln, a);
    }
    float b[kStateChunks * 4];
#pragma unroll
    for (int c = 0; c < kStateChunks; ++c) {
      const float4 v = f[4 * M + c];
      b[4 * c] = v.x; b[4 * c + 1] = v.y; b[4 * c + 2] = v.z; b[4 * c + 3] = v.w;
    }
#pragma unroll
    for (int k = 0; k < K; ++k) { st.pw[k] = b[k]; st.ph[k] = b[K + k]; }
    st.x0 = b[2 * K]; st.x1 = b[2 * K + 1]; st.y0 = b[2 * K + 2]; st.y1 = b[2 * K + 3];
    st.d0 = b[2 * K + 4]; st.d1 = b[2 * K + 5]; st.u0 = b[2 * K + 6]; st.u1 = b[2 * K + 7];
    st.u_tail = b[2 * K + 8];
    const int it = __float_as_int(b[2 * K + 9]);
    st.idx = it & 0xff;
    st.tail = it >> 8;
    st.s_tail = st.d0;
    if (st.tail == 2) st.s_tail = softplus(st.u_tail) + min_slope;
  }

  __device__ __forceinline__ static void colsum_add(const float (&v)[4], float* dst, const MmaLane& ln) {
    const bool hi = ln.lane & 16, b8 = ln.lane & 8;
    float k0 = hi ? v[2] : v[0], k1 = hi ? v[3] : v[1];
    const float s0 = hi ? v[0] : v[2], s1 = hi ? v[1] : v[3];
    k0 += __shfl_xor_sync(0xffffffffu, s0, 16);
    k1 += __shfl_xor_sync(0xffffffffu, s1, 16);
    float kk = b8 ? k1 : k0;
    const float ss = b8 ? k0 : k1;
    kk += __shfl_xor_sync(0xffffffffu, ss, 8);
    kk += __shfl_xor_sync(0xffffffffu, kk, 4);
    if (!(ln.lane & 4)) red_global(dst + (hi ? 8 : 0) + 2 * ln.t + (b8 ? 1 : 0), kk);
  }
  __device__ __forceinline__ static void colsum_a(const float (&a)[2][2][4], float* dst, const MmaLane& ln) {
    float s[4];
#pragma unroll
    for (int nt = 0; nt < 2; ++nt) {
      s[2 * nt] = (a[0][nt][0] + a[0][nt][1]) + (a[1][nt][0] + a[1][nt][1]);
      s[2 * nt + 1] = (a[0][nt][2] + a[0][nt][3]) + (a[1][nt][2] + a[1][nt][3]);
    }
    colsum_add(s, dst, ln);
  }

  __device__ __forceinline__ static void wgrad16(uint32_t TA, uint32_t TG, float* dst, const MmaLane& ln) {
    float dw[2][4];
#pragma unroll
    for (int nt = 0; nt < 2; ++nt)
#pragma unroll
      for (int e = 0; e < 4; ++e) dw[nt][e] = 0.f;
    const uint32_t ta = TA + ln.tbase, tg = TG + ln.tbase;
#pragma unroll
    for (int ks = 0; ks < 4; ++ks) {
      float av[4];
      av[0] = lds32(ta + ks * 512 + 16 * (ln.tu ^ ks));
      av[1] = lds32(ta + ks * 512 + 16 * (ln.tu ^ ks ^ 2));
      av[2] = lds32(ta + ks * 512 + 256 + 16 * (ln.tu ^ ks ^ 1));
      av[3] = lds32(ta + ks * 512 + 256 + 16 * (ln.tu ^ ks ^ 3));
      uint32_t ahi[4], alo[4];
#pragma unroll
      for (int e = 0; e < 4; ++e) split_tf32(av[e], ahi[e], alo[e]);
#pragma unroll
      for (int nt = 0; nt < 2; ++nt) {
        const float b0 = lds32(tg + ks * 512 + 16 * (ln.tu ^ ks ^ (2 * nt)));
        const float b1 = lds32(tg + ks * 512 + 256 + 16 * (ln.tu ^ ks ^ (2 * nt) ^ 1));
        uint32_t bh0, bh1, bl0, bl1;
        split_tf32(b0, bh0, bl0);
        split_tf32(b1, bh1, bl1);
        mma_tf32(dw[nt], alo, bh0, bh1);
        mma_tf32(dw[nt], ahi, bl0, bl1);
        mma_tf32(dw[nt], ahi, bh0, bh1);
      }
    }
#pragma unroll
    for (int nt = 0; nt < 2; ++nt) {
      float* q0 = dst + ln.g * 16 + 8 * nt + 2 * ln.t;
      red_global2(q0, dw[nt][0], dw[nt][1]);
      red_global2(q0 + 128, dw[nt][2], dw[nt][3]);
    }
  }

  __device__ __forceinline__ void cond_backward(int D, int layer, int d, float tval, const float* cvec,
                                                const float* gtheta, float* gvec) const {
    const MmaLane ln;
    const uint32_t wt = swt();
    const int n_in = d + 1, mlp = layer * (D - 1) + d - 1;
    const int w_off = mlp_offset<Net>(D, layer, d);
    const Ref W = wref() + (RES ? cw_offset(D, M, Pp, layer, d) : w_off);
    float* A = gacc + w_off;
    const Ref frag = fref() + (mlp * M * kFragFloats + 512);
    const uint32_t tg = wt + M * kWtFloats * 4;
    __syncwarp();
    store_row(tg, ln, gtheta);
    __syncwarp();
    float G[2][2][4];
    {
      float c[2][2][4];
      load_c(tg, ln, c);
#pragma unroll
      for (int mt = 0; mt < 2; ++mt)
#pragma unroll
        for (int nt = 0; nt < 2; ++nt) {
          G[mt][nt][0] = c[mt][nt][0]; G[mt][nt][1] = c[mt][nt][2];
          G[mt][nt][2] = c[mt][nt][1]; G[mt][nt][3] = c[mt][nt][3];
        }
    }
#pragma unroll
    for (int slot = M - 1; slot >= 0; --slot) {
      const int moff = n_in * H + H + slot * (H * H + H);
      wgrad16(wt + slot * kWtFloats * 4, tg, A + moff, ln);
      colsum_a(G, A + moff + H * 16, ln);
      float dh[2][2][4], hm[2][2][4];
      dense16(G, frag + slot * kFragFloats, Ref::none(), ln, dh);
      load_c(wt + slot * kWtFloats * 4, ln, hm);
#pragma unroll
      for (int mt = 0; mt < 2; ++mt)
#pragma unroll
        for (int nt = 0; nt < 2; ++nt) {
          G[mt][nt][0] = hm[mt][nt][0] > 0.f ? dh[mt][nt][0] : 0.f;
          G[mt][nt][1] = hm[mt][nt][2] > 0.f ? dh[mt][nt][2] : 0.f;
          G[mt][nt][2] = hm[mt][nt][1] > 0.f ? dh[mt][nt][1] : 0.f;
          G[mt][nt][3] = hm[mt][nt][3] > 0.f ? dh[mt][nt][3] : 0.f;
        }
      if (slot > 0) {
        __syncwarp();
        store_a(tg, ln, G);
        __syncwarp();
      }
    }
    colsum_a(G, A + n_in * H, ln);
#pragma unroll 1
    for (int i = 0; i < n_in; ++i) {
      const float xi = i == 0 ? tval : cvec[perm_at(layer, i - 1, D)];
      const float2 w0 = (W + i * 16 + 2 * ln.t).ld2();
      const float2 w1 = (W + i * 16 + 8 + 2 * ln.t).ld2();
      float pw[4] = {0.f, 0.f, 0.f, 0.f}, pin[4];
#pragma unroll
      for (int q = 0; q < 4; ++q) {
        const float xq = __shfl_sync(0xffffffffu, xi, (ln.lane & ~3u) | q);
        const float g00 = G[q >> 1][0][q & 1], g01 = G[q >> 1][0][(q & 1) + 2];
        const float g10 = G[q >> 1][1][q & 1], g11 = G[q >> 1][1][(q & 1) + 2];
        pw[0] = fmaf(xq, g00, pw[0]); pw[1] = fmaf(xq, g01, pw[1]);
        pw[2] = fmaf(xq, g10, pw[2]); pw[3] = fmaf(xq, g11, pw[3]);
        pin[q] = g00 * w0.x + g01 * w0.y + g10 * w1.x + g11 * w1.y;
      }
      colsum_add(pw, A + i * 16, ln);
      if (i >= 1) {
        const bool t2 = ln.lane & 2, t1 = ln.lane & 1;
        float k0 = t2 ? pin[2] : pin[0], k1 = t2 ? pin[3] : pin[1];
        const float s0 = t2 ? pin[0] : pin[2], s1 = t2 ? pin[1] : pin[3];
        k0 += __shfl_xor_sync(0xffffffffu, s0, 2);
        k1 += __shfl_xor_sync(0xffffffffu, s1, 2);
        float kk = t1 ? k1 : k0;
        const float ss = t1 ? k0 : k1;
        kk += __shfl_xor_sync(0xffffffffu, ss, 1);
        gvec[perm_at(layer, i - 1, D)] += kk;
      }
    }
  }

  __device__ __forceinline__ void flush_first(const float* gfirst, const RowTiles<float, Net>&) const {
    const uint32_t lane = threadIdx.x & 31;
#pragma unroll
    for (int j = 0; j < Pp; ++j) {
      float v = gfirst[j];
#pragma unroll
      for (int o = 16; o > 0; o >>= 1) v += __shfl_xor_sync(0xffffffffu, v, o);
      if (lane == 0) red_global(gacc + j, v);
    }
    __syncthreads();
  }
};

}
```

Baseline: 1.809 billion.

## Move forward-pass activation stash from global memory into Blackwell tensor memory

Replaces the per-CTA global-memory stash of hidden activations and spline state (written with __stcg, reread with __ldcg in the backward pass) with a per-CTA tcgen05 tensor-memory allocation. New kernel variants (kEngMmaStash) allocate TMEM columns at kernel start and free them at the end. Occupancy is now also capped by the TMEM columns each CTA needs. This removes L2/HBM traffic and the workspace region for the stash, but adds alloc/dealloc synchronisation and can lower the number of resident CTAs when a layout needs many columns.

```diff
diff --git a/cnf_ot_b200/csrc/api.cu b/cnf_ot_b200/csrc/api.cu
--- a/cnf_ot_b200/csrc/api.cu
+++ b/cnf_ot_b200/csrc/api.cu
@@ -174,7 +174,7 @@
   return 0;
 }
 
-static int configure(const void* kernel, const SmemPlan& sp, int64_t tiles, LaunchCfg* cfg) {
+static int configure(const void* kernel, const SmemPlan& sp, int64_t tiles, LaunchCfg* cfg, int tmem_cols = 0) {
   DeviceInfo di;
   if (int rc = device_info(&di)) return rc;
   size_t smem = (size_t)sp.floats * sizeof(float);
@@ -186,7 +186,8 @@
   int occ = 0;
   e = cudaOccupancyMaxActiveBlocksPerMultiprocessor(&occ, kernel, kTile, smem);
   if (e != cudaSuccess) return cuda_fail(e, "cudaOccupancyMaxActiveBlocksPerMultiprocessor");
-  if (sp.off_wmma >= 0) {
+  if (sp.off_wmma >= 0) tmem_cols = kTcTmemCols;
+  if (tmem_cols > 0) {
     cudaFuncAttributes fa;
     e = cudaFuncGetAttributes(&fa, kernel);
     if (e != cudaSuccess) return cuda_fail(e, "cudaFuncGetAttributes");
@@ -195,7 +196,7 @@
     cudaDeviceGetAttribute(&regs_sm, cudaDevAttrMaxRegistersPerMultiprocessor, di.device);
     int by_smem = (int)(smem_sm / (smem + fa.sharedSizeBytes + 1024));
     int by_regs = regs_sm / (fa.numRegs * kTile > 0 ? fa.numRegs * kTile : 1);
-    int by_tmem = 512 / 32;
+    int by_tmem = 512 / tmem_cols;
     occ = by_smem < by_regs ? by_smem : by_regs;
     if (occ > by_tmem) occ = by_tmem;
   }
@@ -231,18 +232,17 @@
   int64_t grad = ((int64_t)kMaxGrid * lay.total * sizeof(float) + 255) / 256 * 256;
   return kCounterBytes + loss + grad + frag_bytes(lay);
 }
-static int64_t stash_cta_floats(const FlowLayout& lay) {
-  if (!tc_available(lay)) return 0;
-  const int64_t per_cta = (int64_t)lay.L * (lay.D - 1) * (4 * lay.M + (2 * lay.K + 10 + 3) / 4) * kTile * 4;
-  if (per_cta * (int64_t)sizeof(float) > 64 * 1024) return 0;
+static int stash_tmem_cols(const FlowLayout& lay, int engine) {
+  if (engine != kEngMma) return 0;
+  const int per_thread = lay.L * (lay.D - 1) * (16 * lay.M + 2 * lay.K + 10);
+  if (per_thread > 128) return 0;
   if (const char* e = getenv("CNFOT_STEP_STASH")) {
     if (e[0] == '0') return 0;
   }
-  return per_cta;
-}
-constexpr int kStashMaxGrid = 6 * 148;
-static int64_t stash_bytes(const FlowLayout& lay) { return stash_cta_floats(lay) * (int64_t)sizeof(float) * kStashMaxGrid; }
-static int64_t step_bytes(const FlowLayout& lay) { return partial_bytes(lay) + stash_bytes(lay); }
+  int cols = 32;
+  while (cols < per_thread) cols <<= 1;
+  return cols;
+}
 static float* carve_frags(void* ws, const FlowLayout& lay) {
   return (float*)((char*)ws + partial_bytes(lay) - frag_bytes(lay));
 }
@@ -574,7 +574,7 @@
   FlowLayout lay;
   if (check_flow(flow, &lay)) return -1;
   if (use_wide(flow, lay)) return wide_flow_workspace_bytes(lay, rows, true);
-  return step_bytes(lay);
+  return partial_bytes(lay);
 }
 
 static int flow_vjp_call(int dir, void* stream, const cnfot_flow_desc* flow, const float* weights,
@@ -614,9 +614,10 @@
   SmemPlan sp;
   int engine;
   if (int rc = make_plan(lay, true, &sp, &engine)) return rc;
-  const void* kernel = find_flow_vjp_kernel(lay, engine);
+  const int stash_cols = stash_tmem_cols(lay, engine);
+  const void* kernel = find_flow_vjp_kernel(lay, engine, stash_cols > 0);
   LaunchCfg cfg;
-  if (int rc = configure(kernel, sp, (rows + kTile - 1) / kTile, &cfg)) return rc;
+  if (int rc = configure(kernel, sp, (rows + kTile - 1) / kTile, &cfg, stash_cols)) return rc;
   unsigned long long* counter;
   VjpArgs a;
   a.W = weights; a.frags = nullptr; a.in = in; a.cond = cond; a.cond_stride = cond_stride; a.rows = rows;
@@ -628,11 +629,7 @@
   a.g_out = g_out; a.g_logdet = g_logdet; a.g_in = g_in; a.dir = dir; a.add_base = add_base;
   a.D = lay.D; a.L = lay.L; a.plan = sp;
   a.pb = carve_partials(workspace, &counter);
-  a.stash = nullptr;
-  a.stash_cta_floats = (engine == kEngMma || engine == kEngMmaStream) && cfg.grid <= kStashMaxGrid &&
-                               workspace_bytes >= step_bytes(lay)
-                           ? stash_cta_floats(lay) : 0;
-  if (a.stash_cta_floats > 0) a.stash = (float*)((char*)workspace + partial_bytes(lay));
+  a.stash_cols = stash_cols;
   void* args[] = {&a};
   cudaError_t e = cudaLaunchKernel(kernel, dim3(cfg.grid), dim3(kTile), args, cfg.smem, s);
   if (e != cudaSuccess) return cuda_fail(e, "flow_vjp_kernel launch");
@@ -692,7 +689,7 @@
 }
 
 static int64_t step_ws_bytes(const cnfot_flow_desc* flow, const FlowLayout& lay, int64_t rows_B, int64_t rows_b) {
-  return use_wide(flow, lay) ? wide_step_workspace_bytes(lay, rows_B, rows_b) : step_bytes(lay);
+  return use_wide(flow, lay) ? wide_step_workspace_bytes(lay, rows_B, rows_b) : partial_bytes(lay);
 }
 
 int64_t cnfot_mfc_step_workspace_bytes(const cnfot_flow_desc* flow, int64_t rows_B, int64_t rows_b,
@@ -808,8 +805,8 @@
   if (!weights || !workspace) return fail(CNFOT_ERR_ARG, "NULL buffer");
   if (!io.out && !io.stateful) return fail(CNFOT_ERR_ARG, "out is NULL");
   if (!io.rng && !io.t_batch_host) return fail(CNFOT_ERR_ARG, "t_batch is NULL");
-  if (workspace_bytes < step_bytes(lay)) return fail(CNFOT_ERR_WORKSPACE, "workspace too small: %lld < %lld",
-                                                     (long long)workspace_bytes, (long long)step_bytes(lay));
+  if (workspace_bytes < partial_bytes(lay)) return fail(CNFOT_ERR_WORKSPACE, "workspace too small: %lld < %lld",
+                                                        (long long)workspace_bytes, (long long)partial_bytes(lay));
   const char* err = nullptr;
   if (make_step_consts<float>(*problem, lay.D, (double)lambda, global_B, global_b, n_t, &a.pc, &err))
     return fail(CNFOT_ERR_ARG, "%s", err);
@@ -864,7 +861,8 @@
     latency = fit_tiles + (int64_t)n_t * ((rows_b + unit - 1) / unit) < 8 * 4 * 148;
     if (const char* e = getenv("CNFOT_STEP_LATENCY")) latency = e[0] != '0';
   }
-  const void* kernel = find_mfc_step_kernel(lay, engine, group > 1, latency);
+  const int stash_cols = stash_tmem_cols(lay, engine);
+  const void* kernel = find_mfc_step_kernel(lay, engine, group > 1, latency, stash_cols > 0);
   for (int i = 0; i < n_t; ++i)
     add(group > 1 ? kSegKineticSplit : kSegKinetic, kSlotKinetic, 0, 0, io.rng ? 0.f : io.t_batch_host[i], io.rng ? i : -1,
         io.latent_sub, kRowsNormal, io.row0_b, rows_b, group);
@@ -885,7 +883,7 @@
   a.salt_b = philox_salt(kDrawNormal, (uint64_t)global_b);
   a.salt_t = philox_salt(kDrawUniform, (uint64_t)n_t);
   LaunchCfg cfg;
-  if (int rc = configure(kernel, sp, (tiles * unit + kTile - 1) / kTile, &cfg)) return rc;
+  if (int rc = configure(kernel, sp, (tiles * unit + kTile - 1) / kTile, &cfg, stash_cols)) return rc;
   a.W = weights;
   a.frags = nullptr;
   if (engine == kEngMmaStream) {
@@ -894,9 +892,7 @@
     a.frags = fr;
   }
   a.D = lay.D; a.L = lay.L; a.plan = sp;
-  a.stash = nullptr;
-  a.stash_cta_floats = (engine == kEngMma || engine == kEngMmaStream) && cfg.grid <= kStashMaxGrid ? stash_cta_floats(lay) : 0;
-  if (a.stash_cta_floats > 0) a.stash = (float*)((char*)workspace + partial_bytes(lay));
+  a.stash_cols = stash_cols;
   TailArgs& t = a.tail;
   char* wsb = (char*)workspace;
   t.sync = (uint32_t*)wsb;
@@ -970,8 +966,8 @@
   if (int rc = check_flow(flow, &lay)) return rc;
   if (use_wide(flow, lay)) return fail(CNFOT_ERR_ARG, "persistent workspaces serve the fused per-row step kernel, not the wide-conditioner engine");
   if (!workspace) return fail(CNFOT_ERR_ARG, "NULL buffer");
-  if (workspace_bytes < step_bytes(lay)) return fail(CNFOT_ERR_WORKSPACE, "workspace too small: %lld < %lld",
-                                                     (long long)workspace_bytes, (long long)step_bytes(lay));
+  if (workspace_bytes < partial_bytes(lay)) return fail(CNFOT_ERR_WORKSPACE, "workspace too small: %lld < %lld",
+                                                        (long long)workspace_bytes, (long long)partial_bytes(lay));
   cudaError_t e = cudaMemsetAsync(workspace, 0, (size_t)kCounterBytes + (size_t)kStepRows * lay.total * sizeof(float),
                                   (cudaStream_t)stream);
   if (e != cudaSuccess) return cuda_fail(e, "cudaMemsetAsync");
@@ -1042,7 +1038,7 @@
   FlowLayout lay;
   if (check_flow(flow, &lay)) return -1;
   if (use_wide(flow, lay)) { fail(CNFOT_ERR_ARG, "no device-resident update for the wide-conditioner engine"); return -1; }
-  return step_bytes(lay);
+  return partial_bytes(lay);
 }
 
 int cnfot_train_state_init(void* stream, const cnfot_flow_desc* flow, void* state, int64_t state_bytes, uint64_t key,
@@ -1218,7 +1214,7 @@
   FlowLayout lay;
   if (check_flow(flow, &lay)) return -1;
   if (use_wide(flow, lay)) { fail(CNFOT_ERR_ARG, "on-chip draws are not available on the wide-conditioner engine"); return -1; }
-  return align256(step_bytes(lay)) + align256((int64_t)lay.total * sizeof(float)) +
+  return align256(partial_bytes(lay)) + align256((int64_t)lay.total * sizeof(float)) +
          align256((int64_t)(lay.total + CNFOT_NUM_LOSS_SLOTS) * sizeof(float));
 }
 
@@ -1235,7 +1231,7 @@
                                           (long long)workspace_bytes, (long long)need);
   cudaStream_t s = (cudaStream_t)stream;
   char* p = (char*)workspace;
-  const int64_t ws_bytes = align256(step_bytes(lay));
+  const int64_t ws_bytes = align256(partial_bytes(lay));
   void* ws = p; p += ws_bytes;
   float* dW = (float*)p; p += align256((int64_t)lay.total * sizeof(float));
   float* dOut = (float*)p;
diff --git a/cnf_ot_b200/csrc/device_common.cuh b/cnf_ot_b200/csrc/device_common.cuh
--- a/cnf_ot_b200/csrc/device_common.cuh
+++ b/cnf_ot_b200/csrc/device_common.cuh
@@ -167,7 +167,8 @@
   static constexpr bool kAccInGlobal = false;
   __device__ __forceinline__ void bind_partials(float*, bool = true) {}
   __device__ __forceinline__ void bind_frags(const float*) {}
-  __device__ __forceinline__ void bind_stash(float*) {}
+  __device__ __forceinline__ void stash_acquire(int, int, uint32_t*) {}
+  __device__ __forceinline__ void stash_release() {}
   __device__ __forceinline__ bool stash_on() const { return false; }
   static constexpr int H = Net::kH, M = Net::kM, Pp = Net::kPp;
   float* smem;
diff --git a/cnf_ot_b200/csrc/dispatch.h b/cnf_ot_b200/csrc/dispatch.h
--- a/cnf_ot_b200/csrc/dispatch.h
+++ b/cnf_ot_b200/csrc/dispatch.h
@@ -5,8 +5,9 @@
 namespace cnfot {
 
 const void* find_flow_eval_kernel(const FlowLayout& f, int engine = 0);
-const void* find_flow_vjp_kernel(const FlowLayout& f, int engine = 0);
-const void* find_mfc_step_kernel(const FlowLayout& f, int engine = 0, bool split = false, bool latency = false);
+const void* find_flow_vjp_kernel(const FlowLayout& f, int engine = 0, bool stash = false);
+const void* find_mfc_step_kernel(const FlowLayout& f, int engine = 0, bool split = false, bool latency = false,
+                                 bool stash = false);
 const void* find_energy_kernel(const FlowLayout& f, int engine = 0);
 const void* find_density_kernel(const FlowLayout& f, int engine = 0);
 inline bool tc_available(const FlowLayout& f) { return f.H == 16 && f.K == 5 && f.D >= 2 && f.M <= 3; }
diff --git a/cnf_ot_b200/csrc/flow_eval.cu b/cnf_ot_b200/csrc/flow_eval.cu
--- a/cnf_ot_b200/csrc/flow_eval.cu
+++ b/cnf_ot_b200/csrc/flow_eval.cu
@@ -35,9 +35,15 @@
   return nullptr;
 }
 
-const void* find_flow_vjp_kernel(const FlowLayout& f, int engine) {
+const void* find_flow_vjp_kernel(const FlowLayout& f, int engine, bool stash) {
   if (engine == kEngTc && tc_available(f)) {
     VJP_ENG_CASE(1, kEngTc) VJP_ENG_CASE(2, kEngTc) VJP_ENG_CASE(3, kEngTc)
+    return nullptr;
+  }
+  if (engine == kEngMma && tc_available(f) && stash) {
+    if (f.M == 2 && f.D == 2 && f.L == 2)
+      return (const void*)&flow_vjp_kernel<NetCfg<16, 5, 2>, Dims<2, 2>, kEngMmaStash>;
+    VJP_ENG_CASE(1, kEngMmaStash) VJP_ENG_CASE(2, kEngMmaStash) VJP_ENG_CASE(3, kEngMmaStash)
     return nullptr;
   }
   if (engine == kEngMma && tc_available(f)) {
diff --git a/cnf_ot_b200/csrc/flow_kernels.cuh b/cnf_ot_b200/csrc/flow_kernels.cuh
--- a/cnf_ot_b200/csrc/flow_kernels.cuh
+++ b/cnf_ot_b200/csrc/flow_kernels.cuh
@@ -10,7 +10,7 @@
 
 namespace cnfot {
 
-enum Engine { kEngCuda = 0, kEngTc = 1, kEngMma = 2, kEngMmaStream = 3, kEngWide = 4 };
+enum Engine { kEngCuda = 0, kEngTc = 1, kEngMma = 2, kEngMmaStream = 3, kEngWide = 4, kEngMmaStash = 5 };
 #ifndef CNFOT_MMA_MIN_CTAS
 #define CNFOT_MMA_MIN_CTAS 4
 #endif
@@ -29,6 +29,8 @@
 struct CtxSelect<Net, kEngMma, DC, LC> { using type = DeviceCtxMma<Net, true, DC, LC>; };
 template <class Net, int DC, int LC>
 struct CtxSelect<Net, kEngMmaStream, DC, LC> { using type = DeviceCtxMma<Net, false>; };
+template <class Net, int DC, int LC>
+struct CtxSelect<Net, kEngMmaStash, DC, LC> { using type = DeviceCtxMma<Net, true, DC, LC, true>; };
 
 template <class Ctx>
 __device__ __forceinline__ void ctx_setup(Ctx& ctx, int D, int L, uint64_t* mbar, uint32_t* slot) {
@@ -119,8 +121,7 @@
   int D, L;
   SmemPlan plan;
   PartialBuf pb;
-  float* stash;
-  long long stash_cta_floats;
+  int stash_cols;
 };
 
 template <class Net, class DimsT, int ENG>
@@ -135,7 +136,7 @@
   ctx.smem = smem; ctx.gW = a.W; ctx.p = a.plan;
   ctx.bind_partials(a.pb.grad + (int64_t)blockIdx.x * a.plan.total);
   ctx.bind_frags(a.frags);
-  ctx.bind_stash(a.stash ? a.stash + (size_t)blockIdx.x * a.stash_cta_floats : nullptr);
+  ctx.stash_acquire(a.stash_cols, a.L * (a.D - 1), &tc_slot);
   ctx_setup(ctx, a.D, a.L, &tc_mbar, &tc_slot);
   const RowTiles<float, Net> tl = make_row_tiles<Net>(smem, a.plan);
   const DimsT dm{a.D, a.L};
@@ -169,6 +170,7 @@
     if (live && a.g_in)
       for (int i = 0; i < D; ++i) a.g_in[r * D + i] = g[i];
   }
+  ctx.stash_release();
   {
     float graw[Net::kPp];
 #pragma unroll
@@ -383,8 +385,7 @@
   StepConsts<float> pc;
   int n_seg;
   int64_t n_tiles;
-  float* stash;
-  long long stash_cta_floats;
+  int stash_cols;
   unsigned long long key;
   unsigned long long salt_B, salt_Bc, salt_b, salt_t;
   uint32_t step;
@@ -588,7 +589,7 @@
   ctx.smem = smem; ctx.gW = a.W; ctx.p = a.plan;
   ctx.bind_partials(my_row, false);
   ctx.bind_frags(a.frags);
-  ctx.bind_stash(a.stash ? a.stash + (size_t)blockIdx.x * a.stash_cta_floats : nullptr);
+  ctx.stash_acquire(a.stash_cols, DimsT{a.D, a.L}.L() * (DimsT{a.D, a.L}.D() - 1), &tc_slot);
   ctx_setup(ctx, DimsT{a.D, a.L}.D(), DimsT{a.D, a.L}.L(), &tc_mbar, &tc_slot);
   if (a.timeline && threadIdx.x == 0) { const unsigned long long now = global_timer_ns(); atomicMax(a.timeline + 1, now); atomicMax(a.timeline + 6, now - t_start); }
   const RowTiles<float, Net> tl = make_row_tiles<Net>(smem, a.plan);
@@ -657,6 +658,7 @@
       loss[kSlotPotential] += (double)lp;
     }
   }
+  ctx.stash_release();
   asm volatile("griddepcontrol.launch_dependents;");
   if (a.timeline && threadIdx.x == 0) {
     const unsigned long long now = global_timer_ns();
diff --git a/cnf_ot_b200/csrc/step.cu b/cnf_ot_b200/csrc/step.cu
--- a/cnf_ot_b200/csrc/step.cu
+++ b/cnf_ot_b200/csrc/step.cu
@@ -4,18 +4,19 @@
 namespace cnfot {
 
 const void* find_mfc_step_kernel_tc(const FlowLayout& f);
-const void* find_mfc_step_kernel_mma(const FlowLayout& f);
+const void* find_mfc_step_kernel_mma(const FlowLayout& f, bool stash);
 const void* find_mfc_step_kernel_mma_stream(const FlowLayout& f);
 const void* find_mfc_step_kernel_cuda(const FlowLayout& f);
 const void* find_mfc_step_kernel_tc_split(const FlowLayout& f);
-const void* find_mfc_step_kernel_mma_split(const FlowLayout& f);
+const void* find_mfc_step_kernel_mma_split(const FlowLayout& f, bool stash);
 const void* find_mfc_step_kernel_mma_stream_split(const FlowLayout& f);
 const void* find_mfc_step_kernel_mma_stream_lat(const FlowLayout& f);
 const void* find_mfc_step_kernel_cuda_split(const FlowLayout& f);
 
-const void* find_mfc_step_kernel(const FlowLayout& f, int engine, bool split, bool latency) {
+const void* find_mfc_step_kernel(const FlowLayout& f, int engine, bool split, bool latency, bool stash) {
   if (engine == kEngTc && tc_available(f)) return split ? find_mfc_step_kernel_tc_split(f) : find_mfc_step_kernel_tc(f);
-  if (engine == kEngMma && tc_available(f)) return split ? find_mfc_step_kernel_mma_split(f) : find_mfc_step_kernel_mma(f);
+  if (engine == kEngMma && tc_available(f))
+    return split ? find_mfc_step_kernel_mma_split(f, stash) : find_mfc_step_kernel_mma(f, stash);
   if (engine == kEngMmaStream && tc_available(f))
     return split ? find_mfc_step_kernel_mma_stream_split(f)
                  : (latency ? find_mfc_step_kernel_mma_stream_lat(f) : find_mfc_step_kernel_mma_stream(f));
diff --git a/cnf_ot_b200/csrc/step_mma.cu b/cnf_ot_b200/csrc/step_mma.cu
--- a/cnf_ot_b200/csrc/step_mma.cu
+++ b/cnf_ot_b200/csrc/step_mma.cu
@@ -10,10 +10,16 @@
   if (f.M == M_) return (const void*)&mfc_step_kernel<NetCfg<16, 5, M_>, Dims<0, 0>, E_, CNFOT_STEP_SPLIT != 0>;
 
 #if CNFOT_STEP_SPLIT
-const void* find_mfc_step_kernel_mma_split(const FlowLayout& f) {
+const void* find_mfc_step_kernel_mma_split(const FlowLayout& f, bool stash) {
 #else
-const void* find_mfc_step_kernel_mma(const FlowLayout& f) {
+const void* find_mfc_step_kernel_mma(const FlowLayout& f, bool stash) {
 #endif
+  if (stash) {
+    if (f.M == 2 && f.D == 2 && f.L == 2)
+      return (const void*)&mfc_step_kernel<NetCfg<16, 5, 2>, Dims<2, 2>, kEngMmaStash, CNFOT_STEP_SPLIT != 0>;
+    STEP_ENG_CASE(1, kEngMmaStash) STEP_ENG_CASE(2, kEngMmaStash) STEP_ENG_CASE(3, kEngMmaStash)
+    return nullptr;
+  }
   if (f.M == 2 && f.D == 2 && f.L == 2)
     return (const void*)&mfc_step_kernel<NetCfg<16, 5, 2>, Dims<2, 2>, kEngMma, CNFOT_STEP_SPLIT != 0>;
   STEP_ENG_CASE(1, kEngMma) STEP_ENG_CASE(2, kEngMma) STEP_ENG_CASE(3, kEngMma)
diff --git a/cnf_ot_b200/csrc/warp_mlp.cuh b/cnf_ot_b200/csrc/warp_mlp.cuh
--- a/cnf_ot_b200/csrc/warp_mlp.cuh
+++ b/cnf_ot_b200/csrc/warp_mlp.cuh
@@ -172,7 +172,7 @@
   return cnfot_dyn_smem;
 }
 
-template <class Net, bool RES, int DC = 0, int LC = 0>
+template <class Net, bool RES, int DC = 0, int LC = 0, bool STASH = false>
 struct DeviceCtxMma {
   using NetT = Net;
   using Ref = WRef<RES>;
@@ -206,37 +206,89 @@
   const float* gfrag;
   Ref w_ref, frag_ref;
   uint32_t s_wt;
-  float* stash = nullptr;
   static constexpr int kStateFloats = 2 * Net::kK + 10;
-  static constexpr int kStateChunks = (kStateFloats + 3) / 4;
-  static constexpr int kStashChunks = 4 * M + kStateChunks;
-  static constexpr int kStashCondFloats = kStashChunks * kTile * 4;
-  __device__ __forceinline__ void bind_stash(float* q) { stash = q; }
-  __device__ __forceinline__ bool stash_on() const { return stash != nullptr; }
-  __device__ __forceinline__ float* stash_of(int D, int layer, int d) const {
-    return stash + (size_t)(layer * (D - 1) + d - 1) * kStashCondFloats + threadIdx.x * 4;
-  }
-  __device__ __forceinline__ static void stash_put(float* q, int chunk0, const float (&v)[2][2][4]) {
-#pragma unroll
-    for (int c = 0; c < 4; ++c)
-      __stcg(reinterpret_cast<float4*>(q + (chunk0 + c) * kTile * 4),
-             make_float4(v[c >> 1][c & 1][0], v[c >> 1][c & 1][1], v[c >> 1][c & 1][2], v[c >> 1][c & 1][3]));
-  }
+  static_assert(kStateFloats == 20, "the stash layout holds a located spline of 5 bins");
+  uint32_t stash_t = 0;
+  int stash_nc = 0;
+  int stash_cols = 0;
+  __device__ __forceinline__ bool stash_on() const { return STASH && stash_nc != 0; }
+  __device__ __forceinline__ int stash_ncond() const {
+    if constexpr (kConstPlan) return LC * (DC - 1);
+    else return stash_nc;
+  }
+  __device__ __forceinline__ static int stash_cond(int D, int layer, int d) { return layer * (D - 1) + d - 1; }
+  __device__ __forceinline__ void stash_acquire(int cols, int n_cond, uint32_t* slot) {
+    if constexpr (STASH) {
+      if (threadIdx.x < 32) {
+        asm volatile("tcgen05.alloc.cta_group::1.sync.aligned.shared::cta.b32 [%0], %1;"
+                     ::"r"((uint32_t)__cvta_generic_to_shared(slot)), "r"(cols) : "memory");
+        asm volatile("tcgen05.relinquish_alloc_permit.cta_group::1.sync.aligned;" ::: "memory");
+      }
+      asm volatile("tcgen05.fence::before_thread_sync;" ::: "memory");
+      __syncthreads();
+      asm volatile("tcgen05.fence::after_thread_sync;" ::: "memory");
+      stash_t = *slot + ((threadIdx.x & ~31u) << 16);
+      stash_nc = n_cond;
+      stash_cols = cols;
+    }
+  }
+  __device__ __forceinline__ void stash_release() {
+    if constexpr (STASH) {
+      asm volatile("tcgen05.fence::before_thread_sync;" ::: "memory");
+      __syncthreads();
+      if (threadIdx.x < 32) {
+        asm volatile("tcgen05.fence::after_thread_sync;" ::: "memory");
+        asm volatile("tcgen05.dealloc.cta_group::1.sync.aligned.b32 %0, %1;" ::"r"(stash_t), "r"(stash_cols) : "memory");
+      }
+      stash_nc = 0;
+      stash_cols = 0;
+    }
+  }
+  __device__ __forceinline__ static void tmem_st16(uint32_t ta, const float* v) {
+    asm volatile(
+        "tcgen05.st.sync.aligned.32x32b.x16.b32 [%0], {%1,%2,%3,%4,%5,%6,%7,%8,%9,%10,%11,%12,%13,%14,%15,%16};"
+        ::"r"(ta), "f"(v[0]), "f"(v[1]), "f"(v[2]), "f"(v[3]), "f"(v[4]), "f"(v[5]), "f"(v[6]), "f"(v[7]), "f"(v[8]),
+          "f"(v[9]), "f"(v[10]), "f"(v[11]), "f"(v[12]), "f"(v[13]), "f"(v[14]), "f"(v[15])
+        : "memory");
+  }
+  __device__ __forceinline__ static void tmem_st4(uint32_t ta, const float* v) {
+    asm volatile("tcgen05.st.sync.aligned.32x32b.x4.b32 [%0], {%1,%2,%3,%4};"
+                 ::"r"(ta), "f"(v[0]), "f"(v[1]), "f"(v[2]), "f"(v[3]) : "memory");
+  }
+  __device__ __forceinline__ static void tmem_ld16(uint32_t ta, float* v) {
+    asm volatile(
+        "tcgen05.ld.sync.aligned.32x32b.x16.b32 {%0,%1,%2,%3,%4,%5,%6,%7,%8,%9,%10,%11,%12,%13,%14,%15}, [%16];\n\t"
+        "tcgen05.wait::ld.sync.aligned;"
+        : "=f"(v[0]), "=f"(v[1]), "=f"(v[2]), "=f"(v[3]), "=f"(v[4]), "=f"(v[5]), "=f"(v[6]), "=f"(v[7]), "=f"(v[8]),
+          "=f"(v[9]), "=f"(v[10]), "=f"(v[11]), "=f"(v[12]), "=f"(v[13]), "=f"(v[14]), "=f"(v[15])
+        : "r"(ta) : "memory");
+  }
+  __device__ __forceinline__ static void tmem_ld16_4(uint32_t ta16, uint32_t ta4, float* v) {
+    asm volatile(
+        "tcgen05.ld.sync.aligned.32x32b.x16.b32 {%0,%1,%2,%3,%4,%5,%6,%7,%8,%9,%10,%11,%12,%13,%14,%15}, [%20];\n\t"
+        "tcgen05.ld.sync.aligned.32x32b.x4.b32 {%16,%17,%18,%19}, [%21];\n\t"
+        "tcgen05.wait::ld.sync.aligned;"
+        : "=f"(v[0]), "=f"(v[1]), "=f"(v[2]), "=f"(v[3]), "=f"(v[4]), "=f"(v[5]), "=f"(v[6]), "=f"(v[7]), "=f"(v[8]),
+          "=f"(v[9]), "=f"(v[10]), "=f"(v[11]), "=f"(v[12]), "=f"(v[13]), "=f"(v[14]), "=f"(v[15]), "=f"(v[16]),
+          "=f"(v[17]), "=f"(v[18]), "=f"(v[19])
+        : "r"(ta16), "r"(ta4) : "memory");
+  }
+  __device__ __forceinline__ uint32_t stash_hidden(int c, int m) const { return stash_t + 16 * (c * M + m); }
   __device__ __forceinline__ void stash_state(int D, int layer, int d, const SplineState<float, Net::kK>& st) const {
-    constexpr int K = Net::kK;
-    float b[kStateChunks * 4];
-#pragma unroll
-    for (int k = 0; k < K; ++k) { b[k] = st.pw[k]; b[K + k] = st.ph[k]; }
-    b[2 * K] = st.x0; b[2 * K + 1] = st.x1; b[2 * K + 2] = st.y0; b[2 * K + 3] = st.y1;
-    b[2 * K + 4] = st.d0; b[2 * K + 5] = st.d1; b[2 * K + 6] = st.u0; b[2 * K + 7] = st.u1;
-    b[2 * K + 8] = st.u_tail;
-    b[2 * K + 9] = __int_as_float(st.idx | (st.tail << 8));
-#pragma unroll
-    for (int j = kStateFloats; j < kStateChunks * 4; ++j) b[j] = 0.f;
-    float* q = stash_of(D, layer, d) + 4 * M * kTile * 4;
-#pragma unroll
-    for (int c = 0; c < kStateChunks; ++c)
-      __stcg(reinterpret_cast<float4*>(q + c * kTile * 4), make_float4(b[4 * c], b[4 * c + 1], b[4 * c + 2], b[4 * c + 3]));
+    if constexpr (STASH) {
+      constexpr int K = Net::kK;
+      float b[kStateFloats];
+  #pragma unroll
+      for (int k = 0; k < K; ++k) { b[k] = st.pw[k]; b[K + k] = st.ph[k]; }
+      b[2 * K] = st.x0; b[2 * K + 1] = st.x1; b[2 * K + 2] = st.y0; b[2 * K + 3] = st.y1;
+      b[2 * K + 4] = st.d0; b[2 * K + 5] = st.d1; b[2 * K + 6] = st.u0; b[2 * K + 7] = st.u1;
+      b[2 * K + 8] = st.u_tail;
+      b[2 * K + 9] = __int_as_float(st.idx | (st.tail << 8));
+      const int c = stash_cond(D, layer, d), nc = stash_ncond();
+      __syncwarp();
+      tmem_st16(stash_t + 16 * (nc * M + c), b);
+      tmem_st4(stash_t + 16 * nc * (M + 1) + 4 * c, b + 16);
+    }
   }
 
   bool clear_acc;
@@ -405,7 +457,7 @@
 
   __device__ __forceinline__ void cond_forward(int D, int layer, int d, float tval, const float* cvec,
                                                float* theta, bool keep, bool put = false) const {
-    float* sq = put ? stash_of(D, layer, d) : nullptr;
+    const int sc = stash_cond(D, layer, d);
     const MmaLane ln;
     const uint32_t wt = swt();
     const int n_in = d + 1, mlp = layer * (D - 1) + d - 1;
@@ -441,14 +493,14 @@
       __syncwarp();
       store_a(wt, ln, a);
     }
-    if (put) stash_put(sq, 0, a);
+    if (STASH && put) tmem_st16(stash_hidden(sc, 0), &a[0][0][0]);
     Ref bm = RES ? b0 + H : b0 + (H + H * H);
 #pragma unroll
     for (int m = 1; m < M; ++m) {
       dense16(a, frag + (m - 1) * kFragFloats, bm, ln, x);
       relu_to_a(x, a);
       if (keep) store_a(wt + m * kWtFloats * 4, ln, a);
-      if (put) stash_put(sq, 4 * m, a);
+      if (STASH && put) tmem_st16(stash_hidden(sc, m), &a[0][0][0]);
       bm = bm + (RES ? H : H * H + H);
     }
     dense16(a, frag + (M - 1) * kFragFloats, bm, ln, x);
@@ -460,40 +512,32 @@
   }
 
   __device__ __forceinline__ void cond_restore(int D, int layer, int d, SplineState<float, Net::kK>& st, float min_slope) const {
-    constexpr int K = Net::kK;
-    const MmaLane ln;
-    const uint32_t wt = swt();
-    const float* sq = stash_of(D, layer, d);
-    float4 f[kStashChunks];
-#pragma unroll
-    for (int c = 0; c < kStashChunks; ++c) f[c] = __ldcg(reinterpret_cast<const float4*>(sq + c * kTile * 4));
-    __syncwarp();
-#pragma unroll
-    for (int m = 0; m < M; ++m) {
-      float a[2][2][4];
-#pragma unroll
-      for (int c = 0; c < 4; ++c) {
-        const float4 v = f[4 * m + c];
-        a[c >> 1][c & 1][0] = v.x; a[c >> 1][c & 1][1] = v.y; a[c >> 1][c & 1][2] = v.z; a[c >> 1][c & 1][3] = v.w;
-      }
-      store_a(wt + m * kWtFloats * 4, ln, a);
-    }
-    float b[kStateChunks * 4];
-#pragma unroll
-    for (int c = 0; c < kStateChunks; ++c) {
-      const float4 v = f[4 * M + c];
-      b[4 * c] = v.x; b[4 * c + 1] = v.y; b[4 * c + 2] = v.z; b[4 * c + 3] = v.w;
-    }
-#pragma unroll
-    for (int k = 0; k < K; ++k) { st.pw[k] = b[k]; st.ph[k] = b[K + k]; }
-    st.x0 = b[2 * K]; st.x1 = b[2 * K + 1]; st.y0 = b[2 * K + 2]; st.y1 = b[2 * K + 3];
-    st.d0 = b[2 * K + 4]; st.d1 = b[2 * K + 5]; st.u0 = b[2 * K + 6]; st.u1 = b[2 * K + 7];
-    st.u_tail = b[2 * K + 8];
-    const int it = __float_as_int(b[2 * K + 9]);
-    st.idx = it & 0xff;
-    st.tail = it >> 8;
-    st.s_tail = st.d0;
-    if (st.tail == 2) st.s_tail = softplus(st.u_tail) + min_slope;
+    if constexpr (STASH) {
+      constexpr int K = Net::kK;
+      const MmaLane ln;
+      const uint32_t wt = swt();
+      const int c = stash_cond(D, layer, d), nc = stash_ncond();
+      __syncwarp();
+      asm volatile("tcgen05.wait::st.sync.aligned;" ::: "memory");
+  #pragma unroll
+      for (int m = 0; m < M; ++m) {
+        float a[2][2][4];
+        tmem_ld16(stash_hidden(c, m), &a[0][0][0]);
+        store_a(wt + m * kWtFloats * 4, ln, a);
+      }
+      float b[kStateFloats];
+      tmem_ld16_4(stash_t + 16 * (nc * M + c), stash_t + 16 * nc * (M + 1) + 4 * c, b);
+  #pragma unroll
+      for (int k = 0; k < K; ++k) { st.pw[k] = b[k]; st.ph[k] = b[K + k]; }
+      st.x0 = b[2 * K]; st.x1 = b[2 * K + 1]; st.y0 = b[2 * K + 2]; st.y1 = b[2 * K + 3];
+      st.d0 = b[2 * K + 4]; st.d1 = b[2 * K + 5]; st.u0 = b[2 * K + 6]; st.u1 = b[2 * K + 7];
+      st.u_tail = b[2 * K + 8];
+      const int it = __float_as_int(b[2 * K + 9]);
+      st.idx = it & 0xff;
+      st.tail = it >> 8;
+      st.s_tail = st.d0;
+      if (st.tail == 2) st.s_tail = softplus(st.u_tail) + min_slope;
+    }
   }
 
   __device__ __forceinline__ static void colsum_add(const float (&v)[4], float* dst, const MmaLane& ln) {
```

New measurement: 1.925 billion, median of 6. 6.4% higher.
